# adolfogonzalez3/maddpg

Measured on AMD Instinct MI355X. Metric: env-steps/sec (end-to-end at the reference update cadence), simple_spread N=3, batch 1024, higher is better.
Workload: dtype fp32

## Files before the change

include/maddpg_hip.h:

```cpp
#ifndef MADDPG_HIP_H
#define MADDPG_HIP_H

#include <stddef.h>
#include <stdint.h>

#ifdef __cplusplus
extern "C" {
#endif

#define MDP_MAX_AGENTS 8
#define MDP_ACT_DIM 5
#define MDP_MAX_UNITS 256
#define MDP_ABI_VERSION 5

enum mdp_scenario {
    MDP_SCN_NONE = 0,
    MDP_SCN_SIMPLE = 1,
    MDP_SCN_SPREAD = 2,
    MDP_SCN_ADVERSARY = 3,
    MDP_SCN_TAG = 4,
    MDP_SCN_SPEAKER_LISTENER = 5
};

enum mdp_which {
    MDP_ACTOR = 0, MDP_CRITIC = 1, MDP_TGT_ACTOR = 2, MDP_TGT_CRITIC = 3,
    MDP_M_ACTOR = 4, MDP_V_ACTOR = 5, MDP_M_CRITIC = 6, MDP_V_CRITIC = 7,
    MDP_G_ACTOR = 8, MDP_G_CRITIC = 9
};

enum mdp_region_id {
    MDP_R_THETA = 0, MDP_R_TARGET = 1, MDP_R_ADAM_M = 2, MDP_R_ADAM_V = 3,
    MDP_R_GRAD = 4, MDP_R_REPLAY = 5, MDP_R_INDEX = 6, MDP_R_STATS = 7,
    MDP_R_ENV = 8, MDP_R_EPLOG = 9, MDP_R_BETA = 10, MDP_R_SLAB = 11,
    MDP_R_CTL = 12, MDP_R_COUNT = 13
};

typedef struct mdp_config {
    int32_t n_agents;
    int32_t obs_dim[MDP_MAX_AGENTS];
    int32_t local_q[MDP_MAX_AGENTS];
    int32_t act_dim;
    int32_t num_units;
    int32_t batch_size;
    int32_t max_episode_len;
    int64_t capacity;
    int32_t num_envs;
    int32_t scenario;
    int32_t num_adversaries;
    int32_t world_size, rank;
    float lr;
    float tau;
    float grad_clip;
    float actor_reg;
    float adam_b1, adam_b2, adam_eps;
    double gamma;
    uint64_t seed;
    int32_t episode_log_rows;
    int32_t reserved;
} mdp_config;

typedef struct mdp_tensor_info {
    int64_t offset;
    int32_t rows, cols;
    int32_t dev_rows, dev_cols;
} mdp_tensor_info;

typedef struct mdp_handle mdp_handle;

int32_t mdp_abi_version(void);
int64_t mdp_arena_bytes(const mdp_config* cfg, int64_t* param_floats);
int mdp_create(const mdp_config* cfg, void* arena_dev, int64_t arena_bytes,
               void* hip_stream, mdp_handle** out);
int mdp_destroy(mdp_handle* h);
const char* mdp_last_error(const mdp_handle* h);
void* mdp_stream(mdp_handle* h);
int mdp_synchronize(mdp_handle* h);
int mdp_region(const mdp_handle* h, int32_t region, int64_t* offset, int64_t* bytes);
int mdp_tensor(const mdp_handle* h, int32_t agent, int32_t net, int32_t t, mdp_tensor_info* out);
int mdp_row_layout(const mdp_handle* h, int32_t agent, int32_t out6[6]);
int mdp_set_act_dims(mdp_handle* h, const int32_t dims[MDP_MAX_AGENTS]);
int mdp_get_act_dims(const mdp_handle* h, int32_t dims[MDP_MAX_AGENTS]);

int mdp_set_params(mdp_handle* h, int32_t agent, int32_t which, const float* src_host, int64_t n);
int mdp_get_params(mdp_handle* h, int32_t agent, int32_t which, float* dst_host, int64_t n);
int mdp_get_beta_powers(mdp_handle* h, int32_t agent, int32_t net, float out2[2]);
int mdp_set_beta_powers(mdp_handle* h, int32_t agent, int32_t net, const float in2[2]);

int64_t mdp_buffer_len(mdp_handle* h);
int mdp_buffer_add_rows(mdp_handle* h, const float* rows_dev, int64_t rows);
int mdp_buffer_put_agent(mdp_handle* h, int32_t agent, const int64_t* pos_dev,
                         const float* cols_dev, int64_t rows);
int mdp_buffer_set_len(mdp_handle* h, int64_t len, int64_t next_idx);
int mdp_buffer_set_ring(mdp_handle* h, int64_t len, int64_t next_idx, int64_t rows_total);
int mdp_seed_py_random(mdp_handle* h, uint64_t seed);
int mdp_set_rng_state(mdp_handle* h, const uint32_t* state625_host);
int mdp_get_rng_state(mdp_handle* h, uint32_t* state625_host);
int mdp_make_index(mdp_handle* h, int32_t count, int32_t* idx_dev);
int mdp_sample_rows(mdp_handle* h, const int32_t* idx_dev, int32_t count, float* out_dev);

int mdp_act(mdp_handle* h, int32_t agent, int32_t target, const float* obs_dev,
            float* act_dev, int32_t rows, const float* u_dev);
int mdp_actor_logits(mdp_handle* h, int32_t agent, int32_t target, const float* obs_dev,
                     float* logits_dev, int32_t rows);
int mdp_q_values(mdp_handle* h, int32_t agent, int32_t target, const float* x_dev,
                 float* q_dev, int32_t rows);

int mdp_update(mdp_handle* h, int32_t agent, const int32_t* idx_dev,
               const float* u_tgt_dev, const float* u_act_dev);
int mdp_update_gate(mdp_handle* h, int64_t t);
int mdp_agent_update(mdp_handle* h, int32_t agent, int64_t t, const int32_t* idx_dev, const float* u_dev,
                     double stats_out[6]);
int mdp_update_round(mdp_handle* h);
int mdp_set_graphs(mdp_handle* h, int32_t on);
int mdp_train_step(mdp_handle* h, int32_t rounds);
int mdp_train_steps(mdp_handle* h, int32_t n, const int32_t* rounds, int32_t launch);

int mdp_dp_unique_id(uint8_t* out128);
int mdp_dp_init(mdp_handle* h, const uint8_t* id128, int32_t world, int32_t rank);

#define MDP_XGMI_HANDLE_BYTES 64
int mdp_dp_xgmi_open(mdp_handle* h, int32_t world, int32_t rank, uint8_t* handle_out);
int mdp_dp_xgmi_connect(mdp_handle* h, const uint8_t* handles);
int mdp_dp_xgmi_probe(mdp_handle* h, int32_t* mismatches);
int mdp_dp_xgmi_enable(mdp_handle* h);
int mdp_dp_xgmi_close(mdp_handle* h);
int mdp_dp_info(mdp_handle* h, int32_t out4[4]);
int mdp_dp_exchange_stats(mdp_handle* h, double out4[4], int32_t reset);
int mdp_dp_exchange_stats_enable(mdp_handle* h, int32_t on);
int mdp_ra_plan(const mdp_config* cfg, int32_t cus, int32_t per_cu, int32_t* out);
int mdp_critic_grad(mdp_handle* h, int32_t agent, const int32_t* idx_dev, const float* u_tgt_dev);
int mdp_actor_grad(mdp_handle* h, int32_t agent, const int32_t* idx_dev, const float* u_act_dev);
int mdp_reduce_grad(mdp_handle* h, int32_t agent, int32_t net);
int mdp_apply_grad(mdp_handle* h, int32_t agent, int32_t net, float scale);
int mdp_get_stats(mdp_handle* h, int32_t agent, double out6[6]);
int mdp_check_finite(mdp_handle* h, int64_t* nonfinite_out);

int mdp_set_update_mode(mdp_handle* h, int32_t mode);
int mdp_update_all(mdp_handle* h, const int32_t* idx_dev, const float* u_tgt_dev, const float* u_act_dev);

int mdp_env_reset(mdp_handle* h);
int mdp_env_step(mdp_handle* h, const float* act_in_dev, const float* u_dev);
int mdp_env_get_state(mdp_handle* h, float* pos_host, float* vel_host, int32_t* goal_host, int32_t* ep_step_host);
int mdp_env_set_state(mdp_handle* h, const float* pos_host, const float* vel_host, const int32_t* goal_host, const int32_t* ep_step_host);
int mdp_env_get_comm(mdp_handle* h, float* comm_host);
int mdp_env_set_comm(mdp_handle* h, const float* comm_host);
int mdp_env_obs(mdp_handle* h, float* obs_dev);
#define MDP_BENCH_W 8
int mdp_env_step_bench(mdp_handle* h, float* info_dev);
int mdp_env_step_bench_u(mdp_handle* h, float* info_dev, const float* u_dev);

enum { MDP_EVAL_SAMPLE = 0, MDP_EVAL_MEAN = 1 };
int mdp_evaluate(mdp_handle* h, int64_t first_episode, int32_t episodes, int32_t mode,
                 const float* u_dev, float* ret_dev, float* bench_dev);
int mdp_eval_initial_state(mdp_handle* h, int64_t first_episode, int32_t episodes,
                           float* pos_host, float* vel_host, int32_t* goal_host);

int64_t mdp_actor_set_floats(const mdp_handle* h);
int mdp_actor_set_write(mdp_handle* h, float* set_dev, int32_t agent, const float* src_host, int64_t n);
int mdp_actor_set_snapshot(mdp_handle* h, float* set_dev);
int mdp_evaluate_matchups(mdp_handle* h, const float* bank_dev, int32_t n_sets,
                          const int32_t* table_host, int32_t matchups,
                          int64_t first_episode, int32_t episodes, int32_t mode,
                          const float* u_dev, float* ret_dev, float* bench_dev);
int64_t mdp_episode_count(mdp_handle* h);
int mdp_episode_log(mdp_handle* h, int64_t first, int64_t n, float* out_host);

int64_t mdp_per_bytes(const mdp_config* cfg);
int mdp_per_enable(mdp_handle* h, void* buf_dev, int64_t bytes, float alpha, float beta0, float beta_inc,
                   float eps, float abs_err_upper);
int mdp_per_sample(mdp_handle* h, int32_t agent, int32_t count, const float* u_dev, int32_t* idx_out_dev,
                   float* w_out_dev);
int mdp_per_set_priorities(mdp_handle* h, int32_t agent, const int32_t* pos_dev, const float* p_dev, int32_t count);
int mdp_per_update_errors(mdp_handle* h, int32_t agent, const int32_t* pos_dev, const float* abs_err_dev,
                          int32_t count);
int mdp_per_slots(mdp_handle* h, int32_t agent, int64_t out3[3]);
int64_t mdp_per_tree_nodes(const mdp_handle* h);
int mdp_per_get_tree(mdp_handle* h, int32_t agent, float* nodes_host);
int mdp_per_info(mdp_handle* h, int32_t agent, double out5[5]);

enum mdp_kernel_kind {
    MDP_K_INDEX = 0, MDP_K_GATHER = 1, MDP_K_CRITIC_GRAD = 2, MDP_K_ACTOR_GRAD = 3,
    MDP_K_APPLY = 4, MDP_K_ROLLOUT = 5, MDP_K_REDUCE = 6, MDP_K_REDUCE_APPLY = 7,
    MDP_K_ALLREDUCE = 8,
    MDP_K_PER_SYNC = 9, MDP_K_PER_SAMPLE = 10, MDP_K_PER_UPDATE = 11,
    MDP_K_EVAL = 12,
    MDP_K_COUNT = 13
};
int mdp_prof_enable(mdp_handle* h, int32_t kind, int32_t on);
int mdp_grad_variant(mdp_handle* h, int32_t agent);
int mdp_prof_read(mdp_handle* h, int32_t kind, double* total_ms, int64_t* launches);

#ifdef __cplusplus
}
#endif
#endif
```

maddpg_amd/_lib.py:

```python
import ctypes
import os
import re

import torch

HERE = os.path.dirname(os.path.abspath(__file__))
LIB_PATH = os.environ.get("MDP_LIB") or os.path.join(HERE, "libmaddpg_hip.so")
HEADER = os.path.join(os.path.dirname(HERE), "include", "maddpg_hip.h")

MAX_AGENTS = 8
ACT_DIM = 5
BENCH_W = 8
MAX_UNITS = 256
ABI_VERSION = 5

SCN = {"none": 0, "simple": 1, "simple_spread": 2, "simple_adversary": 3, "simple_tag": 4,
       "simple_speaker_listener": 5}
WHICH = {"actor": 0, "critic": 1, "tgt_actor": 2, "tgt_critic": 3, "m_actor": 4, "v_actor": 5,
         "m_critic": 6, "v_critic": 7, "g_actor": 8, "g_critic": 9}
REGION = {"theta": 0, "target": 1, "adam_m": 2, "adam_v": 3, "grad": 4, "replay": 5, "index": 6,
          "stats": 7, "env": 8, "eplog": 9, "beta": 10, "slab": 11, "ctl": 12}
KERNEL = {"index": 0, "gather": 1, "critic_grad": 2, "actor_grad": 3, "apply": 4, "rollout": 5,
          "reduce": 6, "reduce_apply": 7, "allreduce": 8}
KERNEL_PER = {"per_sync": 9, "per_sample": 10, "per_update": 11}
KERNEL_EVAL = {"eval": 12}
EVAL_MODE = {"sample": 0, "mean": 1}
EVAL_MAX_EPISODES = 1 << 20
EVAL_MAX_SETS = 4096
EVAL_MAX_MATCHUP_EPISODES = 1 << 22


class MdpConfig(ctypes.Structure):
    _fields_ = [
        ("n_agents", ctypes.c_int32),
        ("obs_dim", ctypes.c_int32 * MAX_AGENTS),
        ("local_q", ctypes.c_int32 * MAX_AGENTS),
        ("act_dim", ctypes.c_int32),
        ("num_units", ctypes.c_int32),
        ("batch_size", ctypes.c_int32),
        ("max_episode_len", ctypes.c_int32),
        ("capacity", ctypes.c_int64),
        ("num_envs", ctypes.c_int32),
        ("scenario", ctypes.c_int32),
        ("num_adversaries", ctypes.c_int32),
        ("world_size", ctypes.c_int32),
        ("rank", ctypes.c_int32),
        ("lr", ctypes.c_float),
        ("tau", ctypes.c_float),
        ("grad_clip", ctypes.c_float),
        ("actor_reg", ctypes.c_float),
        ("adam_b1", ctypes.c_float),
        ("adam_b2", ctypes.c_float),
        ("adam_eps", ctypes.c_float),
        ("gamma", ctypes.c_double),
        ("seed", ctypes.c_uint64),
        ("episode_log_rows", ctypes.c_int32),
        ("reserved", ctypes.c_int32),
    ]


class MdpTensorInfo(ctypes.Structure):
    _fields_ = [("offset", ctypes.c_int64), ("rows", ctypes.c_int32), ("cols", ctypes.c_int32),
                ("dev_rows", ctypes.c_int32), ("dev_cols", ctypes.c_int32)]


_P = ctypes.c_void_p
_I32 = ctypes.c_int32
_I64 = ctypes.c_int64
_F32P = ctypes.POINTER(ctypes.c_float)
_F64P = ctypes.POINTER(ctypes.c_double)
_U32P = ctypes.POINTER(ctypes.c_uint32)
_I32P = ctypes.POINTER(ctypes.c_int32)

SIGNATURES = {
    "mdp_abi_version": (_I32, []),
    "mdp_arena_bytes": (_I64, [ctypes.POINTER(MdpConfig), ctypes.POINTER(_I64)]),
    "mdp_create": (ctypes.c_int, [ctypes.POINTER(MdpConfig), _P, _I64, _P, ctypes.POINTER(_P)]),
    "mdp_destroy": (ctypes.c_int, [_P]),
    "mdp_last_error": (ctypes.c_char_p, [_P]),
    "mdp_stream": (_P, [_P]),
    "mdp_synchronize": (ctypes.c_int, [_P]),
    "mdp_region": (ctypes.c_int, [_P, _I32, ctypes.POINTER(_I64), ctypes.POINTER(_I64)]),
    "mdp_tensor": (ctypes.c_int, [_P, _I32, _I32, _I32, ctypes.POINTER(MdpTensorInfo)]),
    "mdp_row_layout": (ctypes.c_int, [_P, _I32, _I32P]),
    "mdp_set_act_dims": (ctypes.c_int, [_P, _I32P]),
    "mdp_get_act_dims": (ctypes.c_int, [_P, _I32P]),
    "mdp_set_params": (ctypes.c_int, [_P, _I32, _I32, _F32P, _I64]),
    "mdp_get_params": (ctypes.c_int, [_P, _I32, _I32, _F32P, _I64]),
    "mdp_get_beta_powers": (ctypes.c_int, [_P, _I32, _I32, _F32P]),
    "mdp_set_beta_powers": (ctypes.c_int, [_P, _I32, _I32, _F32P]),
    "mdp_buffer_len": (_I64, [_P]),
    "mdp_buffer_add_rows": (ctypes.c_int, [_P, _P, _I64]),
    "mdp_buffer_put_agent": (ctypes.c_int, [_P, _I32, _P, _P, _I64]),
    "mdp_buffer_set_len": (ctypes.c_int, [_P, _I64, _I64]),
    "mdp_buffer_set_ring": (ctypes.c_int, [_P, _I64, _I64, _I64]),
    "mdp_seed_py_random": (ctypes.c_int, [_P, ctypes.c_uint64]),
    "mdp_set_rng_state": (ctypes.c_int, [_P, _U32P]),
    "mdp_get_rng_state": (ctypes.c_int, [_P, _U32P]),
    "mdp_make_index": (ctypes.c_int, [_P, _I32, _P]),
    "mdp_sample_rows": (ctypes.c_int, [_P, _P, _I32, _P]),
    "mdp_act": (ctypes.c_int, [_P, _I32, _I32, _P, _P, _I32, _P]),
    "mdp_actor_logits": (ctypes.c_int, [_P, _I32, _I32, _P, _P, _I32]),
    "mdp_q_values": (ctypes.c_int, [_P, _I32, _I32, _P, _P, _I32]),
    "mdp_update": (ctypes.c_int, [_P, _I32, _P, _P, _P]),
    "mdp_update_gate": (ctypes.c_int, [_P, _I64]),
    "mdp_update_round": (ctypes.c_int, [_P]),
    "mdp_set_graphs": (ctypes.c_int, [_P, _I32]),
    "mdp_train_step": (ctypes.c_int, [_P, _I32]),
    "mdp_dp_unique_id": (ctypes.c_int, [ctypes.c_char_p]),
    "mdp_grad_variant": (ctypes.c_int, [_P, _I32]),
    "mdp_dp_init": (ctypes.c_int, [_P, ctypes.c_char_p, _I32, _I32]),
    "mdp_dp_xgmi_open": (ctypes.c_int, [_P, _I32, _I32, ctypes.c_char_p]),
    "mdp_dp_xgmi_connect": (ctypes.c_int, [_P, ctypes.c_char_p]),
    "mdp_dp_xgmi_probe": (ctypes.c_int, [_P, _I32P]),
    "mdp_dp_xgmi_enable": (ctypes.c_int, [_P]),
    "mdp_dp_xgmi_close": (ctypes.c_int, [_P]),
    "mdp_dp_info": (ctypes.c_int, [_P, _I32P]),
    "mdp_dp_exchange_stats": (ctypes.c_int, [_P, ctypes.POINTER(ctypes.c_double), _I32]),
    "mdp_dp_exchange_stats_enable": (ctypes.c_int, [_P, _I32]),
    "mdp_train_steps": (ctypes.c_int, [_P, _I32, ctypes.POINTER(ctypes.c_int32), _I32]),
    "mdp_agent_update": (ctypes.c_int, [_P, _I32, ctypes.c_int64, _P, _P, ctypes.POINTER(ctypes.c_double)]),
    "mdp_ra_plan": (ctypes.c_int, [ctypes.POINTER(MdpConfig), _I32, _I32, _I32P]),
    "mdp_critic_grad": (ctypes.c_int, [_P, _I32, _P, _P]),
    "mdp_actor_grad": (ctypes.c_int, [_P, _I32, _P, _P]),
    "mdp_reduce_grad": (ctypes.c_int, [_P, _I32, _I32]),
    "mdp_apply_grad": (ctypes.c_int, [_P, _I32, _I32, ctypes.c_float]),
    "mdp_get_stats": (ctypes.c_int, [_P, _I32, _F64P]),
    "mdp_check_finite": (ctypes.c_int, [_P, ctypes.POINTER(_I64)]),
    "mdp_env_reset": (ctypes.c_int, [_P]),
    "mdp_env_step": (ctypes.c_int, [_P, _P, _P]),
    "mdp_env_get_state": (ctypes.c_int, [_P, _F32P, _F32P, _I32P, _I32P]),
    "mdp_env_set_state": (ctypes.c_int, [_P, _F32P, _F32P, _I32P, _I32P]),
    "mdp_env_get_comm": (ctypes.c_int, [_P, _F32P]),
    "mdp_env_set_comm": (ctypes.c_int, [_P, _F32P]),
    "mdp_env_obs": (ctypes.c_int, [_P, _P]),
    "mdp_env_step_bench": (ctypes.c_int, [_P, _P]),
    "mdp_env_step_bench_u": (ctypes.c_int, [_P, _P, _P]),
    "mdp_evaluate": (ctypes.c_int, [_P, _I64, _I32, _I32, _P, _P, _P]),
    "mdp_eval_initial_state": (ctypes.c_int, [_P, _I64, _I32, _F32P, _F32P, _I32P]),
    "mdp_actor_set_floats": (_I64, [_P]),
    "mdp_actor_set_write": (ctypes.c_int, [_P, _P, _I32, _F32P, _I64]),
    "mdp_actor_set_snapshot": (ctypes.c_int, [_P, _P]),
    "mdp_evaluate_matchups": (ctypes.c_int, [_P, _P, _I32, _I32P, _I32, _I64, _I32, _I32, _P, _P, _P]),
    "mdp_set_update_mode": (ctypes.c_int, [_P, _I32]),
    "mdp_update_all": (ctypes.c_int, [_P, _P, _P, _P]),
    "mdp_episode_count": (_I64, [_P]),
    "mdp_episode_log": (ctypes.c_int, [_P, _I64, _I64, _F32P]),
    "mdp_per_bytes": (_I64, [ctypes.POINTER(MdpConfig)]),
    "mdp_per_enable": (ctypes.c_int, [_P, _P, _I64, ctypes.c_float, ctypes.c_float, ctypes.c_float,
                                      ctypes.c_float, ctypes.c_float]),
    "mdp_per_sample": (ctypes.c_int, [_P, _I32, _I32, _P, _P, _P]),
    "mdp_per_set_priorities": (ctypes.c_int, [_P, _I32, _P, _P, _I32]),
    "mdp_per_update_errors": (ctypes.c_int, [_P, _I32, _P, _P, _I32]),
    "mdp_per_slots": (ctypes.c_int, [_P, _I32, ctypes.POINTER(_I64)]),
    "mdp_per_tree_nodes": (_I64, [_P]),
    "mdp_per_get_tree": (ctypes.c_int, [_P, _I32, _F32P]),
    "mdp_per_info": (ctypes.c_int, [_P, _I32, _F64P]),
    "mdp_prof_enable": (ctypes.c_int, [_P, _I32, _I32]),
    "mdp_prof_read": (ctypes.c_int, [_P, _I32, _F64P, ctypes.POINTER(_I64)]),
}


def header_symbols(path=HEADER):
    text = open(path).read()
    return sorted(set(re.findall(r"\b(mdp_[a-z0-9_]+)\s*\(", text)))


_lib = None


def load():
    global _lib
    if _lib is not None:
        return _lib
    if not os.path.exists(LIB_PATH):
        raise ImportError(
            f"{LIB_PATH} is missing: build it with `make -C maddpg_amd/csrc` "
            "(or __graft_entry__.build()); maddpg_amd has no CPU fallback")
    lib = ctypes.CDLL(LIB_PATH)
    for name, (res, args) in SIGNATURES.items():
        if os.environ.get("MDP_LIB") and not hasattr(lib, name):
            continue
        fn = getattr(lib, name)
        fn.restype = res
        fn.argtypes = args
    if lib.mdp_abi_version() != ABI_VERSION:
        raise ImportError("libmaddpg_hip.so ABI version mismatch")
    _lib = lib
    return lib


class MdpError(RuntimeError):
    pass


def check(lib, handle, rc, what=""):
    if rc < 0:
        msg = lib.mdp_last_error(handle)
        raise MdpError(f"{what}: {msg.decode() if msg else 'error'}")
    return rc


def fptr(a):
    return a.ctypes.data_as(_F32P)
```

maddpg_amd/csrc/mdp_api.cpp:

```cpp
#include <hip/hip_runtime.h>

#include <algorithm>
#include <cmath>
#include <cstdio>
#include <cstdlib>
#include <cstring>
#include <string>
#include <dlfcn.h>
#include <rccl/rccl.h>

#include <map>
#include <vector>

#include "mdp_kernels.h"

namespace {

inline int64_t r4(int64_t n) { return (n + 3) & ~int64_t(3); }
inline int64_t a256(int64_t n) { return (n + 255) & ~int64_t(255); }

NDesc make_net(int64_t& off, int in, int H, int out) {
  NDesc d;
  d.off = (int)off;
  d.in = in;
// ... 155 lines not shown
  }
  const int E = c->num_envs;
  std::vector<int> dims, widths;
  if (c->scenario != MDP_SCN_NONE) {
    if (!make_env(*c, L.env, dims, widths, err)) return false;
    for (int i = 0; i < n; ++i) topo_set_act_w(T, i, widths[i]);
    for (int i = 0; i < n; ++i)
      if (dims[i] != c->obs_dim[i]) {
        char b[160];
        std::snprintf(b, sizeof(b), "obs_dim[%d]=%d does not match scenario (%d)", i, c->obs_dim[i], dims[i]);
        err = b;
        return false;
      }
    if ((int64_t)E > c->capacity) { err = "num_envs exceeds replay capacity"; return false; }
  } else {
    std::memset(&L.env, 0, sizeof(L.env));
  }
  L.n_ent = n + L.env.n_landmarks;
  {
    int need = std::max(lds_critic_bytes(T, 1), lds_actor_bytes(T));
    need = std::max(need, lds_eval_bytes(std::max(cin_max, obs_max), H));
    if (c->scenario != MDP_SCN_NONE) need = std::max(need, lds_rollout_bytes(T));
    if (need > MDP_LDS_BUDGET) {
      char b[200];
      std::snprintf(b, sizeof(b),
                    "configuration outside the kernels' LDS envelope: a 16-row tile needs %d bytes, a CU has %d "
                    "(sum of obs dims %d, %d units)", need, MDP_LDS_BUDGET, sum_obs, c->num_units);
      err = b;
      return false;
    }
  }
  if (c->episode_log_rows < 0) { err = "episode_log_rows < 0"; return false; }
  if (c->episode_log_rows > 0 && (int64_t)c->episode_log_rows < 2 * (int64_t)E) {
    err = "episode_log_rows must be 0 (default) or at least 2 * num_envs";
    return false;
  }
  L.eplog_rows = c->episode_log_rows > 0 ? c->episode_log_rows : std::max(4096, 4 * E);
  int64_t sz[MDP_R_COUNT];
  sz[MDP_R_THETA] = sz[MDP_R_TARGET] = sz[MDP_R_ADAM_M] = sz[MDP_R_ADAM_V] = sz[MDP_R_GRAD] = 4 * L.PT;
  sz[MDP_R_REPLAY] = 4 * c->capacity * T.row_stride;
  sz[MDP_R_INDEX] = 2 * 4 * (int64_t)n * c->batch_size;
  sz[MDP_R_STATS] = 8 * 8 * (int64_t)n;
  sz[MDP_R_ENV] = (int64_t)E * (4 * 4 * L.n_ent + 4 + 4 + 4 * n) + 64 +
                  (env_dim_c(c->scenario) > 0 ? 4 * (int64_t)E * n * MDP_ACT_DIM : 0);
  sz[MDP_R_EPLOG] = 4 * (int64_t)L.eplog_rows * (1 + n);
  sz[MDP_R_BETA] = 4 * 8 * (int64_t)n;
  sz[MDP_R_SLAB] = (int64_t)n * (4 * (int64_t)L.nwg * (L.slab_c + L.slab_a) + 2 * 8 * 8 * (int64_t)L.nwg +
                                  8 * (int64_t)c->batch_size) + 256 + 256 + mdp_ra_sync_bytes() +
                   4 * (int64_t)L.nwg * 16 * (MDP_APRE_W + MDP_CPRE_W + 2 * T.row_stride) +
                   512;
  sz[MDP_R_CTL] = sizeof(Ctl);
  int64_t o = 0;
  for (int r = 0; r < MDP_R_COUNT; ++r) {
    L.off[r] = o;
    L.bytes[r] = sz[r];
    o += a256(sz[r]);
  }
  L.total = o;
  return true;
}

void py_seed_state(uint64_t seed, uint32_t* mt, int32_t* pos) {
  std::vector<uint32_t> key;
  uint64_t s = seed;
  while (s) {
    key.push_back((uint32_t)(s & 0xffffffffu));
    s >>= 32;
  }
  if (key.empty()) key.push_back(0);
  mt[0] = 19650218u;
  for (int i = 1; i < 624; ++i) mt[i] = 1812433253u * (mt[i - 1] ^ (mt[i - 1] >> 30)) + (uint32_t)i;
  int i = 1, j = 0;
  const int kl = (int)key.size();
  for (int k = std::max(624, kl); k; --k) {
    mt[i] = (mt[i] ^ ((mt[i - 1] ^ (mt[i - 1] >> 30)) * 1664525u)) + key[j] + (uint32_t)j;
    ++i;
    ++j;
    if (i >= 624) {
      mt[0] = mt[623];
      i = 1;
    }
    if (j >= kl) j = 0;
  }
  for (int k = 623; k; --k) {
    mt[i] = (mt[i] ^ ((mt[i - 1] ^ (mt[i - 1] >> 30)) * 1566083941u)) - (uint32_t)i;
    ++i;
    if (i >= 624) {
      mt[0] = mt[623];
      i = 1;
    }
  }
  mt[0] = 0x80000000u;
  *pos = 624;
}

}

struct mdp_handle {
  mdp_config cfg;
  Layout L;
  int device = 0;
  hipStream_t stream = nullptr;
  bool own_stream = false;
  char* arena = nullptr;
  float *theta, *target, *m, *v, *grad, *replay, *beta, *slab_c, *slab_a, *eplog;
  float *pos, *vel, *ep_rew;
  float* env_comm = nullptr;
  int32_t *index, *goal, *ep_step;
  double *stats, *stat_c, *stat_a, *y;
  Ctl* ctl;
  int64_t len = 0, next = 0;
  uint32_t act_ctr = 0, reset_ctr = 0;
  bool env_lockstep = true;
  std::string err;
  bool ready = false;
  bool prof_on[MDP_K_COUNT] = {};
  std::vector<hipEvent_t> ev[MDP_K_COUNT];
  size_t ev_used[MDP_K_COUNT] = {};
  double prof_ms[MDP_K_COUNT] = {};
  int64_t prof_n[MDP_K_COUNT] = {};
  bool graphs = true;
  bool capturing = false;
  int eager_rounds = 0;
  bool general_grads = false;
  bool fused_apply = true;
  uint32_t* ra_ctr = nullptr;
  uint64_t* ra_part = nullptr;
  float* apre = nullptr;
  bool actor_pre = true;
  float* cpre = nullptr;
  bool critic_pre = true;
  float* apre_rows = nullptr;
  float* cpre_rows = nullptr;
  hipGraph_t round_graph = nullptr;
  hipGraphExec_t round_exec = nullptr;
  std::map<int, hipGraphExec_t> step_exec;
  std::map<std::vector<int>, hipGraphExec_t> multi_exec;
  int eager_steps = 0;
  ncclComm_t comm = nullptr;
  int dp_world = 1;
  bool dp_graphs = false;
  int update_mode = 0;
  FusedApplyArgs* tp_list = nullptr;
  RaBatch tp_batch;
  RaBatch tp_reduce, tp_step;
  int ra_cap = 0, ra_batch_cap = 0;
  bool tp_fits[4] = {true, true, true, true};
  std::vector<FusedApplyArgs> tp_host[4];
  RaBatch tp_xchg;
  RaBatch tp_pair[3][MDP_MAX_AGENTS];
  bool tp_pair_fits[3][MDP_MAX_AGENTS] = {};
  FusedApplyArgs tp_pair_host[3][MDP_MAX_AGENTS][2];
  bool rollout_draw = true;
  bool draw_ahead = true;
  bool grad_pair = true;
  uint64_t* xbuf = nullptr;
  int x_world = 0, x_rank = 0;
  std::vector<void*> x_opened;
  XchgDesc* xd_dev = nullptr;
  uint32_t* x_probe = nullptr;
  uint32_t x_probe_ep = 0;
  bool p2p = false;
  bool xw_stats = false;
  bool per = false;
  bool trained = false;
  bool started = false;
  PerHdr* per_hdr = nullptr;
  PerState* per_st = nullptr;
  int32_t* per_idx = nullptr;
  float *per_w = nullptr, *per_td = nullptr;
  PerNode* per_trees = nullptr;
  int64_t per_P = 0;
  float per_alpha = 0.6f, per_beta0 = 0.4f, per_beta_inc = 0.001f, per_eps = 0.01f, per_upper = 1.0f;
  int64_t per_host_total = 0;
};

namespace {

int fail(mdp_handle* h, const char* what, hipError_t e = hipSuccess) {
  if (h) {
    h->err = what;
    if (e != hipSuccess) {
      h->err += ": ";
      h->err += hipGetErrorString(e);
    }
  }
  return -1;
}

#define HIPCHK(h, call)                        \
  do {                                         \
    hipError_t e__ = (call);                   \
    if (e__ != hipSuccess) return fail(h, #call, e__); \
  } while (0)

bool unusable(const mdp_handle* h) { return !h || !h->ready; }
#define MDP_NEED(h)               \
  do {                            \
    if (unusable(h)) return -1;   \
  } while (0)

int need_dev(mdp_handle* h, const void* p, int64_t bytes, const char* fn, const char* arg, bool null_ok = true) {
  auto refuse = [&](const char* why) {
    std::string m = std::string(fn) + ": " + arg + " " + why;
    return fail(h, m.c_str());
  };
  if (!p) return null_ok ? 0 : refuse("is null");
  hipPointerAttribute_t a;
  std::memset(&a, 0, sizeof(a));
  const hipError_t e = hipPointerGetAttributes(&a, p);
  if (e != hipSuccess) (void)hipGetLastError();
  const bool managed = a.isManaged || a.type == hipMemoryTypeManaged;
  if (e != hipSuccess || !(a.type == hipMemoryTypeDevice || managed)) {
    (void)hipGetLastError();
    return refuse("is not device memory (a host address would fault the GPU); pass a buffer of the handle's device");
  }
  if (!managed && a.device != h->device) return refuse("is memory of another device than the handle's");
  if (!managed && bytes > 0) {
    hipDeviceptr_t base = nullptr;
    size_t size = 0;
    if (hipMemGetAddressRange(&base, &size, (hipDeviceptr_t)p) == hipSuccess) {
      if ((const char*)p + bytes > (const char*)base + size)
        return refuse("ends before the bytes this call reads or writes (allocation too small)");
    } else {
      (void)hipGetLastError();
    }
  }
  return 0;
}
#define MDP_DEV(h, p, bytes, fn, null_ok)                                   \
  do {                                                                     \
    if (need_dev(h, p, (int64_t)(bytes), fn, #p, null_ok)) return -1;     \
  } while (0)

}

MdpLaunchEv& mdp_launch_ev() {
  static thread_local MdpLaunchEv e;
  return e;
}

namespace {

struct ProfScope {
  mdp_handle* h;
  int kind;
  bool packet;
  hipEvent_t stop = nullptr;
  ProfScope(mdp_handle* hh, int k, bool pk = true) : h(hh), kind(k), packet(pk) {
    if (!h->prof_on[kind] || h->capturing) return;
    auto& pool = h->ev[kind];
    size_t u = h->ev_used[kind];
    if (u + 2 > pool.size()) {
      for (int q = 0; q < 64; ++q) {
        hipEvent_t e;
        if (hipEventCreate(&e) != hipSuccess) return;
        pool.push_back(e);
      }
    }
    h->ev_used[kind] = u + 2;
    stop = pool[u + 1];
    if (packet) {
      mdp_launch_ev() = MdpLaunchEv{pool[u], pool[u + 1]};
    } else {
      (void)hipEventRecord(pool[u], h->stream);
    }
  }
  ~ProfScope() {
    if (!stop) return;
    if (!packet) {
      (void)hipEventRecord(stop, h->stream);
      return;
    }
    MdpLaunchEv& e = mdp_launch_ev();
    if (e.start) {
      e.start = e.stop = nullptr;
      h->ev_used[kind] -= 2;
    }
  }
};

void flush_prof(mdp_handle* h, int kind) {
  auto& pool = h->ev[kind];
  const size_t u = h->ev_used[kind];
  if (!u) return;
  (void)hipEventSynchronize(pool[u - 1]);
  for (size_t q = 0; q + 1 < u; q += 2) {
    float ms = 0.f;
    if (hipEventElapsedTime(&ms, pool[q], pool[q + 1]) == hipSuccess) {
      h->prof_ms[kind] += ms;
      h->prof_n[kind] += 1;
    }
  }
  h->ev_used[kind] = 0;
}

bool bad_agent(mdp_handle* h, int agent) {
  if (unusable(h)) return true;
  if (agent < 0 || agent >= h->cfg.n_agents) {
    fail(h, "agent index out of range");
    return true;
  }
  return false;
}

int region_for(int which, int* region, int* net) {
// ... 705 lines not shown
      const int rc = launch_tp_batch(h, 1);
      if (rc) return rc;
    }
    const int rc = dp_allreduce_all(h);
    if (rc) return rc;
    ProfScope p(h, MDP_K_APPLY, h->tp_fits[2]);
    return launch_tp_batch(h, 2);
  }
  ProfScope p(h, MDP_K_REDUCE_APPLY, h->tp_fits[0]);
  return launch_tp_batch(h, 0);
}

int set_ring(mdp_handle* h, int64_t len, int64_t next) {
  h->len = len;
  h->next = next;
  HIPCHK(h, mdp_launch_set_ring(h->ctl, len, next, h->stream));
  return 0;
}

struct PerLayout {
  int64_t P = 1, hdr = 0, st = 0, idx = 0, w = 0, td = 0, trees = 0, total = 0;
};
PerLayout per_layout(const mdp_config& c) {
  PerLayout p;
  while (p.P < c.capacity) p.P <<= 1;
  const int64_t nb = 4 * (int64_t)c.n_agents * c.batch_size;
  int64_t o = 0;
  p.hdr = o;
  o += a256(sizeof(PerHdr));
  p.st = o;
  o += a256(sizeof(PerState) * MDP_MAX_AGENTS);
  p.idx = o;
  o += a256(nb);
  p.w = o;
  o += a256(nb);
  p.td = o;
  o += a256(nb);
  p.trees = o;
  o += (int64_t)c.n_agents * 2 * p.P * (int64_t)sizeof(PerNode);
  p.total = o;
  return p;
}

int per_sync(mdp_handle* h, int64_t host_rows, bool reset) {
  PerSyncArgs a;
  a.ctl = h->ctl;
  a.hdr = h->per_hdr;
  a.trees = h->per_trees;
  a.tree_stride = 2 * h->per_P;
  a.P = h->per_P;
  a.cap = h->cfg.capacity;
  a.E = h->cfg.num_envs;
  a.host_rows = host_rows;
  a.reset = reset ? 1 : 0;
  a.upper = h->per_upper;
  a.alpha = h->per_alpha;
  ProfScope p(h, MDP_K_PER_SYNC);
  HIPCHK(h, mdp_launch_per_sync(a, h->cfg.n_agents, h->stream));
  return 0;
}

int per_sample(mdp_handle* h, int agent0, int agents, int count, const float* u, const int32_t* idx_in,
               int32_t* idx_out, float* w_out, int64_t stride) {
  PerSampleArgs a;
  a.trees = h->per_trees + (int64_t)agent0 * 2 * h->per_P;
  a.tree_stride = 2 * h->per_P;
  a.P = h->per_P;
  a.cap = h->cfg.capacity;
  a.st = h->per_st + agent0;
  a.agent0 = agent0;
  a.count = count;
  a.u = u;
  a.idx_in = idx_in;
  a.idx_out = idx_out;
  a.w_out = w_out;
  a.stride = stride;
  a.seed = h->cfg.seed;
  a.beta_inc = h->per_beta_inc;
  ProfScope p(h, MDP_K_PER_SAMPLE);
  HIPCHK(h, mdp_launch_per_sample(a, agents, h->stream));
  return 0;
}

int per_update(mdp_handle* h, int agent0, int agents, int count, const int32_t* pos, const float* val,
               int64_t stride, bool from_err) {
  PerUpdateArgs a;
  a.trees = h->per_trees + (int64_t)agent0 * 2 * h->per_P;
  a.tree_stride = 2 * h->per_P;
  a.P = h->per_P;
  a.cap = h->cfg.capacity;
  a.count = count;
  a.ctl = h->ctl;
  a.pos = pos;
  a.val = val;
  a.stride = stride;
  a.from_err = from_err ? 1 : 0;
  a.eps = h->per_eps;
  a.upper = h->per_upper;
  a.alpha = h->per_alpha;
  ProfScope p(h, MDP_K_PER_UPDATE);
  HIPCHK(h, mdp_launch_per_update(a, agents, h->stream));
  return 0;
}

const char* kPerNoDp = "prioritized replay runs on one GPU in strict mode: no data-parallel exchange";

}

extern "C" {

int32_t mdp_abi_version(void) { return MDP_ABI_VERSION; }

int64_t mdp_arena_bytes(const mdp_config* cfg, int64_t* param_floats) {
  Layout L;
  std::string err;
  if (!build_layout(cfg, L, err)) return -1;
  if (param_floats) *param_floats = L.PT;
  return L.total;
}

int mdp_ra_plan(const mdp_config* cfg, int32_t cus, int32_t per_cu, int32_t* out) {
  Layout L;
  std::string err;
  if (!build_layout(cfg, L, err) || cus < 0 || per_cu < 0) return -1;
  int fallback = 0;
  for (int i = 0; i < cfg->n_agents; ++i)
    for (int net = 0; net < 2; ++net) {
      const int g = mdp_ra_grid_of(L.topo, i, net);
      const bool ok = mdp_ra_fits(L.topo, i, net, cus * per_cu);
      if (out) out[2 * i + net] = ok ? g : -g;
      fallback += ok ? 0 : 1;
    }
  return fallback;
}

int mdp_create(const mdp_config* cfg, void* arena_dev, int64_t arena_bytes, void* hip_stream, mdp_handle** out) {
  if (!out) return -1;
  *out = nullptr;
  mdp_handle* h = new mdp_handle();
  std::string err;
  if (!build_layout(cfg, h->L, err)) {
    h->err = err;
    *out = h;
    return -1;
  }
  h->cfg = *cfg;
  {
    const char* g = getenv("MDP_GENERAL_GRADS");
    h->general_grads = g && g[0] == '1';
    const char* u = getenv("MDP_UNFUSED_APPLY");
    h->fused_apply = !(u && u[0] == '1');
    const char* rd = getenv("MDP_ROLLOUT_DRAW");
    h->rollout_draw = !(rd && rd[0] == '0');
    const char* da = getenv("MDP_DRAW_AHEAD");
    h->draw_ahead = !(da && da[0] == '0');
    const char* gp = getenv("MDP_GRAD_PAIR");
    h->grad_pair = !(gp && gp[0] == '0');
    const char* ap = getenv("MDP_ACTOR_PRE");
    h->actor_pre = !(ap && ap[0] == '0');
    const char* cp = getenv("MDP_CRITIC_PRE");
    h->critic_pre = !(cp && cp[0] == '0');
  }
  if (!arena_dev || arena_bytes < h->L.total) {
    h->err = "arena missing or too small";
    *out = h;
    return -1;
  }
  *out = h;
  HIPCHK(h, hipGetDevice(&h->device));
  if (need_dev(h, arena_dev, h->L.total, "mdp_create", "arena_dev", false)) return -1;
  {
    int cus = 0, per = 0, per_b = 0;
    HIPCHK(h, hipDeviceGetAttribute(&cus, hipDeviceAttributeMultiprocessorCount, h->device));
    HIPCHK(h, mdp_ra_occupancy(&per));
    HIPCHK(h, mdp_ra_batch_occupancy(&per_b));
    h->ra_cap = cus * per;
    h->ra_batch_cap = cus * per_b;
    int scratch = 0;
    HIPCHK(h, mdp_spin_kernels_scratch(&scratch));
    if (scratch > 0) h->ra_cap = h->ra_batch_cap = 0;
  }
  if (hip_stream) {
    h->stream = (hipStream_t)hip_stream;
  } else {
    HIPCHK(h, hipStreamCreateWithFlags(&h->stream, hipStreamNonBlocking));
    h->own_stream = true;
  }
  h->arena = (char*)arena_dev;
  auto R = [&](int r) { return (void*)(h->arena + h->L.off[r]); };
  h->theta = (float*)R(MDP_R_THETA);
  h->target = (float*)R(MDP_R_TARGET);
  h->m = (float*)R(MDP_R_ADAM_M);
  h->v = (float*)R(MDP_R_ADAM_V);
  h->grad = (float*)R(MDP_R_GRAD);
  h->replay = (float*)R(MDP_R_REPLAY);
  h->index = (int32_t*)R(MDP_R_INDEX);
  h->stats = (double*)R(MDP_R_STATS);
  h->eplog = (float*)R(MDP_R_EPLOG);
  h->beta = (float*)R(MDP_R_BETA);
  h->ctl = (Ctl*)R(MDP_R_CTL);
  {
    const int E = cfg->num_envs, ne = h->L.n_ent, n = cfg->n_agents;
    char* p = (char*)R(MDP_R_ENV);
    h->pos = (float*)p;
    p += 4 * (int64_t)E * ne * 2;
    h->vel = (float*)p;
    p += 4 * (int64_t)E * ne * 2;
    h->goal = (int32_t*)p;
    p += 4 * (int64_t)E;
    h->ep_step = (int32_t*)p;
    p += 4 * (int64_t)E;
    h->ep_rew = (float*)p;
    p += 4 * (int64_t)E * n;
    if (env_dim_c(cfg->scenario) > 0) h->env_comm = (float*)(p + 64);
  }
  {
    char* p = (char*)R(MDP_R_SLAB);
    const int64_t nwg = h->L.nwg, na = cfg->n_agents;
    h->slab_c = (float*)p;
    p += 4 * na * nwg * h->L.slab_c;
    h->slab_a = (float*)p;
    p += 4 * na * nwg * h->L.slab_a;
    p = (char*)(((uintptr_t)p + 7) & ~uintptr_t(7));
    h->stat_c = (double*)p;
    p += 8 * 8 * na * nwg;
    h->stat_a = (double*)p;
    p += 8 * 8 * na * nwg;
    h->y = (double*)p;
    p += 8 * na * (int64_t)cfg->batch_size + 256;
    p = (char*)(((uintptr_t)p + 255) & ~uintptr_t(255));
    h->ra_ctr = (uint32_t*)p;
    h->ra_part = (uint64_t*)(p + (int64_t)MDP_MAX_AGENTS * 2 * 8 * 128);
    h->apre = (float*)(p + mdp_ra_sync_bytes());
    h->cpre = h->apre + (int64_t)nwg * 16 * MDP_APRE_W;
    h->apre_rows = h->cpre + (int64_t)nwg * 16 * MDP_CPRE_W;
    h->cpre_rows = h->apre_rows + (int64_t)nwg * 16 * h->L.topo.row_stride;
  }
  HIPCHK(h, hipMemsetAsync(h->arena, 0, h->L.total, h->stream));
  std::vector<float> beta(8 * cfg->n_agents);
  for (int i = 0; i < cfg->n_agents * 2; ++i) {
    beta[4 * i] = beta[4 * i + 2] = cfg->adam_b1;
    beta[4 * i + 1] = beta[4 * i + 3] = cfg->adam_b2;
  }
  HIPCHK(h, hipMemcpyAsync(h->beta, beta.data(), 4 * beta.size(), hipMemcpyHostToDevice, h->stream));
  Ctl c;
  std::memset(&c, 0, sizeof(c));
  py_seed_state(0, c.mt, &c.mt_pos);
  HIPCHK(h, hipMemcpyAsync(h->ctl, &c, sizeof(c), hipMemcpyHostToDevice, h->stream));
  HIPCHK(h, hipStreamSynchronize(h->stream));
  h->err.clear();
  h->ready = true;
  return 0;
}

int mdp_destroy(mdp_handle* h) {
  if (!h) return 0;
  if (h->stream) (void)hipStreamSynchronize(h->stream);
  if (h->tp_list) (void)hipFree(h->tp_list);
  for (int k = 0; k < MDP_K_COUNT; ++k)
    for (auto e : h->ev[k]) (void)hipEventDestroy(e);
  if (h->round_exec) (void)hipGraphExecDestroy(h->round_exec);
  if (h->comm) (void)rccl().destroy(h->comm);
  xgmi_release(h);
  for (auto& kv : h->step_exec) (void)hipGraphExecDestroy(kv.second);
  for (auto& kv : h->multi_exec) (void)hipGraphExecDestroy(kv.second);
  if (h->round_graph) (void)hipGraphDestroy(h->round_graph);
  if (h->own_stream && h->stream) (void)hipStreamDestroy(h->stream);
  delete h;
  return 0;
}

const char* mdp_last_error(const mdp_handle* h) { return h ? h->err.c_str() : "null handle"; }
void* mdp_stream(mdp_handle* h) { return h ? (void*)h->stream : nullptr; }

int mdp_synchronize(mdp_handle* h) {
  MDP_NEED(h);
  HIPCHK(h, hipStreamSynchronize(h->stream));
  uint32_t fault = 0;
  HIPCHK(h, hipMemcpy(&fault, &h->ctl->fault, sizeof(fault), hipMemcpyDeviceToHost));
  if (fault == 1) return fail(h, "device fault: a tensor-norm handshake timed out (k_reduce_apply)");
  if (fault == 2) return fail(h, "device fault: a data-parallel peer did not reach the xGMI exchange within 30 s");
  if (fault) return fail(h, "device fault");
  return 0;
}

int mdp_region(const mdp_handle* h, int32_t region, int64_t* offset, int64_t* bytes) {
  if (unusable(h) || region < 0 || region >= MDP_R_COUNT) return -1;
  if (offset) *offset = h->L.off[region];
  if (bytes) *bytes = h->L.bytes[region];
  return 0;
}

int mdp_tensor(const mdp_handle* h, int32_t agent, int32_t net, int32_t t, mdp_tensor_info* out) {
  if (unusable(h) || agent < 0 || agent >= h->cfg.n_agents || t < 0 || t > 5 || !out) return -1;
  const NDesc& d = net ? h->L.topo.ag[agent].critic : h->L.topo.ag[agent].actor;
  out->offset = d.t[t].off;
  logical_shape(h, agent, net ? 1 : 0, t, &out->rows, &out->cols);
  out->dev_rows = d.t[t].rows;
  out->dev_cols = d.t[t].cols;
  return 0;
}

int mdp_set_act_dims(mdp_handle* h, const int32_t dims[MDP_MAX_AGENTS]) {
  MDP_NEED(h);
  if (!dims) return fail(h, "mdp_set_act_dims: dims is null");
  if (h->started || h->trained)
// ... 399 lines not shown
    if (e != hipSuccess) return fail(h, "hipStreamEndCapture", e);
    h->round_graph = g;
    HIPCHK(h, hipGraphInstantiate(&h->round_exec, g, nullptr, nullptr, 0));
  }
  HIPCHK(h, hipGraphLaunch(h->round_exec, h->stream));
  return 0;
}

int mdp_grad_variant(mdp_handle* h, int32_t agent) {
  if (unusable(h) || agent < 0 || agent >= h->cfg.n_agents) return -1;
  return (!h->general_grads && grads_r_ok(h->L.topo, agent)) ? 1 : 0;
}

int mdp_dp_unique_id(uint8_t* out128) {
  if (!out128 || !rccl().ok) return -1;
  ncclUniqueId id;
  if (rccl().get_id(&id) != ncclSuccess) return -1;
  std::memcpy(out128, &id, sizeof(id));
  return 0;
}

int mdp_dp_init(mdp_handle* h, const uint8_t* id128, int32_t world, int32_t rank) {
  if (unusable(h) || !id128) return -1;
  if (h->per) return fail(h, kPerNoDp);
  if (h->update_mode != 0) return fail(h, "join data parallelism before choosing the throughput mode");
  if (h->p2p || h->xbuf) return fail(h, "mdp_dp_init: the xGMI exchange is already set up");
  if (!rccl().ok) return fail(h, "librccl.so.1 could not be loaded");
  if (world < 1 || rank < 0 || rank >= world) return fail(h, "mdp_dp_init: bad world/rank");
  if (h->comm) return fail(h, "mdp_dp_init: already initialised");
  ncclUniqueId id;
  std::memcpy(&id, id128, sizeof(id));
  HIPCHK(h, hipSetDevice(h->device));
  const ncclResult_t r = rccl().init_rank(&h->comm, world, id, rank);
  if (r != ncclSuccess) {
    h->comm = nullptr;
    h->err = std::string("ncclCommInitRank: ") + rccl().err(r);
    return -1;
  }
  h->dp_world = world;
  const char* g = getenv("MDP_DP_GRAPHS");
  h->dp_graphs = g && g[0] == '1';
  for (auto& kv : h->step_exec) (void)hipGraphExecDestroy(kv.second);
  for (auto& kv : h->multi_exec) (void)hipGraphExecDestroy(kv.second);
  h->step_exec.clear();
  h->multi_exec.clear();
  if (h->round_exec) {
    (void)hipGraphExecDestroy(h->round_exec);
    h->round_exec = nullptr;
  }
  if (h->round_graph) {
    (void)hipGraphDestroy(h->round_graph);
    h->round_graph = nullptr;
  }
  return 0;
}

static void drop_graphs(mdp_handle* h);

int mdp_dp_xgmi_open(mdp_handle* h, int32_t world, int32_t rank, uint8_t* handle_out) {
  if (unusable(h) || !handle_out) return -1;
  if (h->per) return fail(h, kPerNoDp);
  if (h->update_mode != 0) return fail(h, "join data parallelism before choosing the throughput mode");
  if (h->comm) return fail(h, "mdp_dp_xgmi_open: an RCCL communicator is already set up");
  if (h->xbuf) return fail(h, "mdp_dp_xgmi_open: already open");
  if (world < 2 || world > MDP_XCH_MAXW || rank < 0 || rank >= world)
    return fail(h, "mdp_dp_xgmi_open: world must be 2..8 and 0 <= rank < world");
  if (h->general_grads || !h->fused_apply) return fail(h, "the xGMI exchange needs the fused optimizer kernel");
  for (int i = 0; i < h->cfg.n_agents; ++i)
    for (int net = 0; net < 2; ++net) {
      if (!reduce_apply_ok(h, i, net)) return fail(h, "the xGMI exchange needs the fused optimizer kernel");
    }
  HIPCHK(h, hipSetDevice(h->device));
  const int64_t bytes = mdp_xch_bytes(world, h->L.PT);
  void* p = nullptr;
  HIPCHK(h, hipExtMallocWithFlags(&p, (size_t)bytes, hipDeviceMallocUncached));
  h->xbuf = (uint64_t*)p;
  HIPCHK(h, hipMemset(p, 0, (size_t)bytes));
  HIPCHK(h, hipMalloc((void**)&h->x_probe, 2 * sizeof(uint32_t)));
  HIPCHK(h, hipDeviceSynchronize());
  hipIpcMemHandle_t mh;
  HIPCHK(h, hipIpcGetMemHandle(&mh, p));
  static_assert(sizeof(mh) == MDP_XGMI_HANDLE_BYTES, "IPC handle size");
  std::memcpy(handle_out, &mh, sizeof(mh));
  h->x_world = world;
  h->x_rank = rank;
  return 0;
}

int mdp_dp_xgmi_connect(mdp_handle* h, const uint8_t* handles) {
  if (unusable(h) || !handles) return -1;
  if (!h->xbuf) return fail(h, "mdp_dp_xgmi_connect: call mdp_dp_xgmi_open first");
  if (!h->x_opened.empty()) return fail(h, "mdp_dp_xgmi_connect: already connected");
  const int W = h->x_world, r = h->x_rank;
  XchgDesc xd;
  std::memset(&xd, 0, sizeof(xd));
  xd.world = W;
  xd.rank = r;
  xd.pt = h->L.PT + MDP_XCH_PROBE;
  h->x_opened.assign(W, nullptr);
  for (int q = 0; q < W; ++q) {
    void* base = h->xbuf;
    if (q != r) {
      hipIpcMemHandle_t mh;
      std::memcpy(&mh, handles + (int64_t)q * MDP_XGMI_HANDLE_BYTES, sizeof(mh));
      const hipError_t e = hipIpcOpenMemHandle(&base, mh, hipIpcMemLazyEnablePeerAccess);
      if (e != hipSuccess) return fail(h, "hipIpcOpenMemHandle", e);
      h->x_opened[q] = base;
    }
    xd.data[q] = (uint64_t*)base;
  }
  HIPCHK(h, hipMalloc((void**)&h->xd_dev, sizeof(XchgDesc)));
  HIPCHK(h, hipMemcpy(h->xd_dev, &xd, sizeof(XchgDesc), hipMemcpyHostToDevice));
  return 0;
}

int mdp_dp_xgmi_probe(mdp_handle* h, int32_t* mismatches) {
  if (unusable(h)) return -1;
  if (!h->xd_dev) return fail(h, "mdp_dp_xgmi_probe: not connected");
  const int nchunk = MDP_XCH_PROBE / 256;
  HIPCHK(h, hipMemsetAsync(h->x_probe, 0, 2 * sizeof(uint32_t), h->stream));
  for (int k = 0; k < 4; ++k)
    HIPCHK(h, mdp_launch_xchg_probe(h->xd_dev, ++h->x_probe_ep, nchunk, h->x_probe, h->x_probe + 1, h->stream));
  uint32_t res[2] = {0, 0};
  HIPCHK(h, hipMemcpyAsync(res, h->x_probe, sizeof(res), hipMemcpyDeviceToHost, h->stream));
  HIPCHK(h, hipStreamSynchronize(h->stream));
  if (mismatches) *mismatches = (int32_t)res[0];
  if (res[1]) return fail(h, "mdp_dp_xgmi_probe: a peer did not reach the exchange within 30 s");
  if (res[0]) return fail(h, "mdp_dp_xgmi_probe: exchanged values differ from the expected world sum");
  return 0;
}

int mdp_dp_xgmi_enable(mdp_handle* h) {
  if (unusable(h)) return -1;
  if (!h->xd_dev) return fail(h, "mdp_dp_xgmi_enable: not connected");
  if (h->per) return fail(h, kPerNoDp);
  if (h->update_mode != 0) return fail(h, "join data parallelism before choosing the throughput mode");
  HIPCHK(h, hipStreamSynchronize(h->stream));
  h->p2p = true;
  h->dp_world = h->x_world;
  drop_graphs(h);
  return 0;
}

int mdp_dp_xgmi_close(mdp_handle* h) {
  if (unusable(h)) return -1;
  (void)hipGetLastError();
  if (h->stream) HIPCHK(h, hipStreamSynchronize(h->stream));
  xgmi_release(h);
  if (!h->comm) h->dp_world = 1;
  drop_graphs(h);
  return 0;
}

int mdp_dp_info(mdp_handle* h, int32_t out4[4]) {
  if (unusable(h) || !out4) return -1;
  out4[0] = h->p2p ? 2 : (h->comm ? 1 : 0);
  out4[1] = 1;
  out4[2] = h->cfg.rank;
  out4[3] = 0;
  if (h->p2p) {
    out4[1] = h->x_world;
    out4[2] = h->x_rank;
    for (void* p : h->x_opened) out4[3] += p ? 1 : 0;
  } else if (h->comm) {
    int c = h->dp_world;
    if (rccl().count && rccl().count(h->comm, &c) != ncclSuccess) return fail(h, "ncclCommCount failed");
    out4[1] = c;
    out4[3] = c - 1;
  }
  return 0;
}

int mdp_dp_exchange_stats(mdp_handle* h, double out4[4], int32_t reset) {
  if (unusable(h) || !out4) return -1;
  HIPCHK(h, hipStreamSynchronize(h->stream));
  uint64_t w[3] = {0, 0, 0};
  HIPCHK(h, hipMemcpy(w, &h->ctl->xw_ticks, sizeof(w), hipMemcpyDeviceToHost));
  const double us_per_tick = 0.01;
  out4[0] = (double)w[1];
  out4[1] = w[1] ? (double)w[0] * us_per_tick / (double)w[1] : 0.0;
  out4[2] = (double)w[2] * us_per_tick;
  out4[3] = (double)w[0] * us_per_tick;
  if (reset) {
    HIPCHK(h, hipMemsetAsync(&h->ctl->xw_ticks, 0, sizeof(w), h->stream));
    HIPCHK(h, hipStreamSynchronize(h->stream));
  }
  return 0;
}

int mdp_dp_exchange_stats_enable(mdp_handle* h, int32_t on) {
  if (unusable(h)) return -1;
  h->xw_stats = on != 0;
  return 0;
}

int mdp_set_graphs(mdp_handle* h, int32_t on) {
  MDP_NEED(h);
  h->graphs = on != 0;
  return 0;
}

static void drop_graphs(mdp_handle* h) {
  for (auto& kv : h->step_exec) (void)hipGraphExecDestroy(kv.second);
  for (auto& kv : h->multi_exec) (void)hipGraphExecDestroy(kv.second);
  h->step_exec.clear();
  h->multi_exec.clear();
  h->eager_steps = 0;
  if (h->round_exec) {
    (void)hipGraphExecDestroy(h->round_exec);
    h->round_exec = nullptr;
  }
  if (h->round_graph) {
    (void)hipGraphDestroy(h->round_graph);
    h->round_graph = nullptr;
  }
  h->eager_rounds = 0;
}

int mdp_set_update_mode(mdp_handle* h, int32_t mode) {
  if (unusable(h)) return -1;
  if (mode != 0 && mode != 1) return fail(h, "update mode must be 0 (strict) or 1 (throughput)");
  if (mode == 1) {
    if (h->per) return fail(h, "prioritized replay needs the strict update mode (throughput mode is not supported)");
    if (!tp_ok(h)) return fail(h, "throughput mode needs the fused optimizer step for every net and <= 8 agents");
    HIPCHK(h, hipStreamSynchronize(h->stream));
    if (tp_setup(h)) return -1;
  }
  if (mode != h->update_mode) {
    HIPCHK(h, hipStreamSynchronize(h->stream));
    drop_graphs(h);
    h->update_mode = mode;
  }
  return 0;
}

int mdp_update_all(mdp_handle* h, const int32_t* idx_dev, const float* u_tgt_dev, const float* u_act_dev) {
  if (unusable(h)) return -1;
  if (h->update_mode != 1) return fail(h, "mdp_update_all: set throughput mode first");
  h->trained = true;
  if (h->len <= 0) return fail(h, "update on an empty replay buffer");
  {
    const int64_t B = h->cfg.batch_size, n = h->cfg.n_agents;
    MDP_DEV(h, idx_dev, 4 * n * B, "mdp_update_all", true);
    MDP_DEV(h, u_tgt_dev, 4 * n * n * B * MDP_ACT_DIM, "mdp_update_all", true);
    MDP_DEV(h, u_act_dev, 4 * n * B * MDP_ACT_DIM, "mdp_update_all", true);
  }
  const int32_t* idx = idx_dev;
  if (!idx) {
    const int rc = launch_make_index(h, h->cfg.n_agents * h->cfg.batch_size, h->index);
    if (rc) return rc;
    idx = h->index;
  }
  return do_round_tp(h, idx, u_tgt_dev, u_act_dev, nullptr);
}

int mdp_critic_grad(mdp_handle* h, int32_t agent, const int32_t* idx_dev, const float* u_tgt_dev) {
  if (bad_agent(h, agent)) return -1;
  if (!idx_dev) return fail(h, "critic_grad needs indices");
  if (h->per) return fail(h, "mdp_critic_grad: the phase entry points serve data parallelism; prioritized replay uses mdp_update");
  h->trained = true;
  MDP_DEV(h, idx_dev, 4 * (int64_t)h->cfg.batch_size, "mdp_critic_grad", false);
  MDP_DEV(h, u_tgt_dev, 4 * (int64_t)h->cfg.n_agents * h->cfg.batch_size * MDP_ACT_DIM, "mdp_critic_grad", true);
  return do_critic_grad(h, agent, idx_dev, u_tgt_dev);
}

int mdp_actor_grad(mdp_handle* h, int32_t agent, const int32_t* idx_dev, const float* u_act_dev) {
  if (bad_agent(h, agent)) return -1;
  if (!idx_dev) return fail(h, "actor_grad needs indices");
  h->started = true;
  MDP_DEV(h, idx_dev, 4 * (int64_t)h->cfg.batch_size, "mdp_actor_grad", false);
  MDP_DEV(h, u_act_dev, 4 * (int64_t)h->cfg.batch_size * MDP_ACT_DIM, "mdp_actor_grad", true);
  return do_actor_grad(h, agent, idx_dev, u_act_dev);
}

int mdp_reduce_grad(mdp_handle* h, int32_t agent, int32_t net) {
  if (bad_agent(h, agent)) return -1;
  return do_reduce(h, agent, net ? 1 : 0);
}

int mdp_apply_grad(mdp_handle* h, int32_t agent, int32_t net, float scale) {
  if (bad_agent(h, agent)) return -1;
  return do_apply(h, agent, net ? 1 : 0, false, scale);
}

int mdp_get_stats(mdp_handle* h, int32_t agent, double out6[6]) {
  if (bad_agent(h, agent)) return -1;
  double buf[8];
  HIPCHK(h, hipMemcpyAsync(buf, h->stats + agent * 8, sizeof(buf), hipMemcpyDeviceToHost, h->stream));
  HIPCHK(h, hipStreamSynchronize(h->stream));
  for (int i = 0; i < 6; ++i) out6[i] = buf[i];
  return 0;
}

static int need_env(mdp_handle* h) {
  MDP_NEED(h);
  if (h->cfg.scenario == MDP_SCN_NONE || h->cfg.num_envs <= 0) return fail(h, "handle has no device env");
  h->started = true;
  return 0;
}

int mdp_env_reset(mdp_handle* h) {
  if (need_env(h)) return -1;
  EnvResetArgs a;
  a.env = h->L.env;
  a.seed = h->cfg.seed;
  a.ctr = h->reset_ctr++;
  a.env_base = h->cfg.rank * h->cfg.num_envs;
  a.E = h->cfg.num_envs;
  a.pos = h->pos;
  a.vel = h->vel;
  a.goal = h->goal;
  a.ep_step = h->ep_step;
  a.ep_rew = h->ep_rew;
  a.comm = h->env_comm;
  HIPCHK(h, mdp_launch_env_reset(a, h->stream));
  h->env_lockstep = true;
  return 0;
}

static int env_step_launch(mdp_handle* h, const float* act_in_dev, const float* u_dev, float* bench = nullptr,
                           int32_t* pf_out = nullptr, int pf_count = 0, int nsteps = 1) {
  RolloutArgs a;
  a.pf_out = pf_out;
  a.pf_count = pf_out ? pf_count : 0;
  a.nsteps = nsteps;
  a.topo = h->L.topo;
  a.env = h->L.env;
  a.theta = h->theta;
  a.replay = h->replay;
  a.cap = h->cfg.capacity;
  a.pos = h->pos;
  a.vel = h->vel;
  a.goal = h->goal;
  a.ep_step = h->ep_step;
  a.ep_rew = h->ep_rew;
  a.comm = h->env_comm;
  a.eplog = h->eplog;
  a.eplog_cap = h->L.eplog_rows;
  a.eplog_by_env = h->env_lockstep ? 1 : 0;
  a.ctl = h->ctl;
  a.seed = h->cfg.seed;
  a.E = h->cfg.num_envs;
  a.env_base = h->cfg.rank * h->cfg.num_envs;
  a.act_in = act_in_dev;
  a.u_in = u_dev;
  a.ticket = &h->ctl->ticket[2];
  a.bench = bench;
  ProfScope p(h, MDP_K_ROLLOUT);
  HIPCHK(h, mdp_launch_rollout(a, h->L.topo.H, lds_rollout_bytes(h->L.topo), h->stream));
  return 0;
}

static bool rollout_multi_ok(const mdp_handle* h) { return h->cfg.num_envs <= 16; }

static void advance_ring_mirror(mdp_handle* h) {
  const int64_t cap = h->cfg.capacity, E = h->cfg.num_envs;
  h->len = std::min(cap, h->len + E);
  h->next = (h->next + E) % cap;
}

int mdp_env_step(mdp_handle* h, const float* act_in_dev, const float* u_dev) {
  if (need_env(h)) return -1;
  const int64_t en5 = 4 * (int64_t)h->cfg.num_envs * h->cfg.n_agents * MDP_ACT_DIM;
  MDP_DEV(h, act_in_dev, en5, "mdp_env_step", true);
  MDP_DEV(h, u_dev, en5, "mdp_env_step", true);
  const int rc = env_step_launch(h, act_in_dev, u_dev);
  if (rc) return rc;
  advance_ring_mirror(h);
  return 0;
}

int mdp_env_step_bench(mdp_handle* h, float* info_dev) {
  if (need_env(h)) return -1;
  if (!info_dev) return fail(h, "mdp_env_step_bench: info_dev is null");
  MDP_DEV(h, info_dev, 4 * (int64_t)h->cfg.num_envs * h->cfg.n_agents * MDP_BENCH_W, "mdp_env_step_bench", false);
  if (h->cfg.scenario == MDP_SCN_SIMPLE)
    return fail(h, "scenario 'simple' has no benchmark_data (MPE Scenario attribute missing)");
  if (h->cfg.scenario == MDP_SCN_SPEAKER_LISTENER)
    return fail(h, "scenario 'simple_speaker_listener': upstream's benchmark_data raises (it names an undefined "
                   "variable), so there is no record to return");
  const int rc = env_step_launch(h, nullptr, nullptr, info_dev);
  if (rc) return rc;
  advance_ring_mirror(h);
  return 0;
}

static const char* no_bench_reason(int scenario) {
  if (scenario == MDP_SCN_SIMPLE) return "scenario 'simple' has no benchmark_data (MPE Scenario attribute missing)";
  if (scenario == MDP_SCN_SPEAKER_LISTENER)
    return "scenario 'simple_speaker_listener': upstream's benchmark_data raises (it names an undefined "
           "variable), so there is no record to return";
  return nullptr;
}

int mdp_env_step_bench_u(mdp_handle* h, float* info_dev, const float* u_dev) {
  if (need_env(h)) return -1;
  if (!info_dev) return fail(h, "mdp_env_step_bench_u: info_dev is null");
  const int64_t en = 4 * (int64_t)h->cfg.num_envs * h->cfg.n_agents;
  MDP_DEV(h, info_dev, en * MDP_BENCH_W, "mdp_env_step_bench_u", false);
  MDP_DEV(h, u_dev, en * MDP_ACT_DIM, "mdp_env_step_bench_u", true);
  if (const char* why = no_bench_reason(h->cfg.scenario)) return fail(h, why);
  const int rc = env_step_launch(h, nullptr, u_dev, info_dev);
  if (rc) return rc;
  advance_ring_mirror(h);
  return 0;
}

#define MDP_EVAL_MAX_EPISODES (1 << 20)
static int eval_range_ok(mdp_handle* h, const char* fn, int64_t first, int32_t episodes) {
  std::string m = std::string(fn) + ": ";
  if (episodes < 1 || episodes > MDP_EVAL_MAX_EPISODES) return fail(h, (m + "1 <= episodes <= 2^20").c_str());
  if (first < 0 || first + episodes > ((int64_t)1 << 32))
    return fail(h, (m + "episode ids [first_episode, first_episode + episodes) must lie inside uint32").c_str());
  return 0;
}

int mdp_evaluate(mdp_handle* h, int64_t first_episode, int32_t episodes, int32_t mode, const float* u_dev,
                 float* ret_dev, float* bench_dev) {
  if (need_env(h)) return -1;
  if (mode != MDP_EVAL_SAMPLE && mode != MDP_EVAL_MEAN)
    return fail(h, "mdp_evaluate: mode must be MDP_EVAL_SAMPLE (0) or MDP_EVAL_MEAN (1)");
  if (eval_range_ok(h, "mdp_evaluate", first_episode, episodes)) return -1;
  if (u_dev && mode == MDP_EVAL_MEAN) return fail(h, "mdp_evaluate: u_dev is given but MDP_EVAL_MEAN draws no noise");
  if (!ret_dev) return fail(h, "mdp_evaluate: ret_dev is null");
  hipStreamCaptureStatus cs = hipStreamCaptureStatusNone;
  if (h->capturing || (hipStreamIsCapturing(h->stream, &cs) == hipSuccess && cs != hipStreamCaptureStatusNone))
    return fail(h, "mdp_evaluate: the handle's stream is capturing a graph (evaluation is not captured)");
  (void)hipGetLastError();
  const int64_t en = 4 * (int64_t)episodes * h->cfg.n_agents;
  MDP_DEV(h, u_dev, en * h->cfg.max_episode_len * MDP_ACT_DIM, "mdp_evaluate", true);
  MDP_DEV(h, ret_dev, en, "mdp_evaluate", false);
  MDP_DEV(h, bench_dev, en * MDP_BENCH_W, "mdp_evaluate", true);
  if (bench_dev)
    if (const char* why = no_bench_reason(h->cfg.scenario)) return fail(h, why);
  EvalEpArgs a;
  a.topo = h->L.topo;
  a.env = h->L.env;
  a.theta = h->theta;
  a.seed = h->cfg.seed;
  a.first = (uint32_t)first_episode;
  a.episodes = episodes;
  a.mode = mode;
  a.u_in = u_dev;
  a.ret = ret_dev;
  a.bench = bench_dev;
  ProfScope p(h, MDP_K_EVAL);
  HIPCHK(h, mdp_launch_eval_episodes(a, h->L.topo.H, lds_rollout_bytes(h->L.topo), h->stream));
  return 0;
}

int mdp_eval_initial_state(mdp_handle* h, int64_t first_episode, int32_t episodes, float* pos_host, float* vel_host,
                           int32_t* goal_host) {
  if (need_env(h)) return -1;
  if (eval_range_ok(h, "mdp_eval_initial_state", first_episode, episodes)) return -1;
  if (!pos_host || !vel_host || !goal_host) return fail(h, "mdp_eval_initial_state: null output");
  hipStreamCaptureStatus cs = hipStreamCaptureStatusNone;
  if (h->capturing || (hipStreamIsCapturing(h->stream, &cs) == hipSuccess && cs != hipStreamCaptureStatusNone))
    return fail(h, "mdp_eval_initial_state: the handle's stream is capturing a graph");
  (void)hipGetLastError();
  const int64_t ne2 = 2 * (int64_t)(h->L.env.n_agents + h->L.env.n_landmarks);
  const int chunk = std::min<int64_t>(episodes, 1 << 16);
  float* tmp = nullptr;
  HIPCHK(h, hipMalloc((void**)&tmp, (size_t)chunk * (2 * ne2 + 1) * 4));
  float* dpos = tmp;
  float* dvel = tmp + chunk * ne2;
  int32_t* dgoal = reinterpret_cast<int32_t*>(tmp + 2 * chunk * ne2);
  hipError_t e = hipSuccess;
  for (int64_t done = 0; done < episodes && e == hipSuccess; done += chunk) {
    const int c = (int)std::min<int64_t>(chunk, episodes - done);
    e = mdp_launch_eval_reset(h->L.env, h->cfg.seed, (uint32_t)(first_episode + done), c, dpos, dvel, dgoal, h->stream);
    if (e == hipSuccess) e = hipMemcpyAsync(pos_host + done * ne2, dpos, (size_t)c * ne2 * 4, hipMemcpyDeviceToHost, h->stream);
    if (e == hipSuccess) e = hipMemcpyAsync(vel_host + done * ne2, dvel, (size_t)c * ne2 * 4, hipMemcpyDeviceToHost, h->stream);
    if (e == hipSuccess) e = hipMemcpyAsync(goal_host + done, dgoal, (size_t)c * 4, hipMemcpyDeviceToHost, h->stream);
    if (e == hipSuccess) e = hipStreamSynchronize(h->stream);
  }
  (void)hipFree(tmp);
  if (e != hipSuccess) return fail(h, "mdp_eval_initial_state", e);
  return 0;
}

#define MDP_EVAL_MAX_SETS 4096
#define MDP_EVAL_MAX_MATCHUPS 4096
#define MDP_EVAL_MAX_MATCHUP_EPISODES ((int64_t)1 << 22)
static int64_t actor_set_floats(const mdp_handle* h) { return (h->L.PT + 3) & ~(int64_t)3; }
static bool stream_captures(mdp_handle* h) {
  hipStreamCaptureStatus cs = hipStreamCaptureStatusNone;
  const bool c = h->capturing || (hipStreamIsCapturing(h->stream, &cs) == hipSuccess && cs != hipStreamCaptureStatusNone);
  (void)hipGetLastError();
  return c;
}

int64_t mdp_actor_set_floats(const mdp_handle* h) { return unusable(h) ? -1 : actor_set_floats(h); }

int mdp_actor_set_write(mdp_handle* h, float* set_dev, int32_t agent, const float* src_host, int64_t n) {
  MDP_NEED(h);
  if (agent < 0 || agent >= h->cfg.n_agents) return fail(h, "mdp_actor_set_write: agent index out of range");
  if (!src_host) return fail(h, "mdp_actor_set_write: src_host is null");
  if (n != net_floats(h, agent, 0)) return fail(h, "mdp_actor_set_write: n: param count mismatch");
  if (stream_captures(h)) return fail(h, "mdp_actor_set_write: the handle's stream is capturing a graph");
  MDP_DEV(h, set_dev, 4 * actor_set_floats(h), "mdp_actor_set_write", false);
  const NDesc& d = h->L.topo.ag[agent].actor;
  const std::vector<float> buf = scatter_net(h, agent, 0, src_host);
  HIPCHK(h, hipMemcpyAsync(set_dev + d.off, buf.data(), 4 * buf.size(), hipMemcpyHostToDevice, h->stream));
  HIPCHK(h, hipStreamSynchronize(h->stream));
  return 0;
}

int mdp_actor_set_snapshot(mdp_handle* h, float* set_dev) {
  MDP_NEED(h);
  if (stream_captures(h)) return fail(h, "mdp_actor_set_snapshot: the handle's stream is capturing a graph");
  MDP_DEV(h, set_dev, 4 * actor_set_floats(h), "mdp_actor_set_snapshot", false);
  for (int j = 0; j < h->cfg.n_agents; ++j) {
    const NDesc& d = h->L.topo.ag[j].actor;
    HIPCHK(h, hipMemcpyAsync(set_dev + d.off, h->theta + d.off, 4 * (size_t)d.size, hipMemcpyDeviceToDevice, h->stream));
  }
  return 0;
}

int mdp_evaluate_matchups(mdp_handle* h, const float* bank_dev, int32_t n_sets, const int32_t* table_host,
                          int32_t matchups, int64_t first_episode, int32_t episodes, int32_t mode, const float* u_dev,
                          float* ret_dev, float* bench_dev) {
  MDP_NEED(h);
  const char* fn = "mdp_evaluate_matchups";
  if (h->cfg.scenario == MDP_SCN_NONE || h->cfg.num_envs <= 0)
    return fail(h, "mdp_evaluate_matchups: the handle has no device env");
  if (mode != MDP_EVAL_SAMPLE && mode != MDP_EVAL_MEAN)
    return fail(h, "mdp_evaluate_matchups: mode must be MDP_EVAL_SAMPLE (0) or MDP_EVAL_MEAN (1)");
  if (n_sets < 1 || n_sets > MDP_EVAL_MAX_SETS) return fail(h, "mdp_evaluate_matchups: 1 <= n_sets <= 4096");
  if (matchups < 1 || matchups > MDP_EVAL_MAX_MATCHUPS) return fail(h, "mdp_evaluate_matchups: 1 <= matchups <= 4096");
  if (eval_range_ok(h, fn, first_episode, episodes)) return -1;
  if ((int64_t)matchups * episodes > MDP_EVAL_MAX_MATCHUP_EPISODES)
    return fail(h, "mdp_evaluate_matchups: matchups * episodes <= 2^22");
  if (u_dev && mode == MDP_EVAL_MEAN)
    return fail(h, "mdp_evaluate_matchups: u_dev is given but MDP_EVAL_MEAN draws no noise");
  if (!bank_dev) return fail(h, "mdp_evaluate_matchups: bank_dev is null");
  if (!table_host) return fail(h, "mdp_evaluate_matchups: table_host is null");
  if (!ret_dev) return fail(h, "mdp_evaluate_matchups: ret_dev is null");
  if (((uintptr_t)bank_dev & 15) != 0) return fail(h, "mdp_evaluate_matchups: bank_dev must be 16-byte aligned");
  const int n = h->cfg.n_agents;
  for (int m = 0; m < matchups; ++m)
    for (int j = 0; j < n; ++j) {
      const int32_t v = table_host[(int64_t)m * n + j];
      if (v < 0 || v >= n_sets) {
        char b[200];
        std::snprintf(b, sizeof(b), "mdp_evaluate_matchups: table_host[matchup %d][agent %d] = %d is outside [0, n_sets = %d)",
                      m, j, (int)v, (int)n_sets);
        return fail(h, b);
      }
    }
  if (stream_captures(h))
    return fail(h, "mdp_evaluate_matchups: the handle's stream is capturing a graph (evaluation is not captured)");
  const int64_t stride = actor_set_floats(h);
  const int64_t en = 4 * (int64_t)episodes * n;
  MDP_DEV(h, bank_dev, 4 * (int64_t)n_sets * stride, fn, false);
  MDP_DEV(h, u_dev, en * h->cfg.max_episode_len * MDP_ACT_DIM, fn, true);
  MDP_DEV(h, ret_dev, (int64_t)matchups * en, fn, false);
  MDP_DEV(h, bench_dev, (int64_t)matchups * en * MDP_BENCH_W, fn, true);
  if (bench_dev)
    if (const char* why = no_bench_reason(h->cfg.scenario))
      return fail(h, (std::string("mdp_evaluate_matchups: bench_dev: ") + why).c_str());
  const int lds = lds_eval_matchups_bytes(h->L.topo);
  if (lds > MDP_LDS_BUDGET) return fail(h, "mdp_evaluate_matchups: the configuration leaves no LDS for the table row");
  int32_t* table_dev = nullptr;
  const size_t tbytes = 4 * (size_t)matchups * n;
  HIPCHK(h, hipMalloc((void**)&table_dev, tbytes));
  hipError_t e = hipMemcpyAsync(table_dev, table_host, tbytes, hipMemcpyHostToDevice, h->stream);
  if (e == hipSuccess) {
    EvalMuArgs a;
    a.topo = h->L.topo;
    a.env = h->L.env;
    a.theta = nullptr;
    a.seed = h->cfg.seed;
    a.first = (uint32_t)first_episode;
    a.episodes = episodes;
    a.mode = mode;
    a.u_in = u_dev;
    a.ret = ret_dev;
    a.bench = bench_dev;
    a.bank = bank_dev;
    a.table = table_dev;
    a.set_stride = stride;
    a.matchups = matchups;
    ProfScope p(h, MDP_K_EVAL);
    e = mdp_launch_eval_matchups(a, h->L.topo.H, lds, h->stream);
  }
  const hipError_t es = hipStreamSynchronize(h->stream);
  (void)hipFree(table_dev);
  if (e != hipSuccess) return fail(h, "mdp_evaluate_matchups: launch", e);
  if (es != hipSuccess) return fail(h, "mdp_evaluate_matchups: hipStreamSynchronize", es);
  return 0;
}

static int step_launches(mdp_handle* h, int rounds) {
  const int nb = h->cfg.n_agents * h->cfg.batch_size;
  if (h->per) {
    int rc = env_step_launch(h, nullptr, nullptr);
    for (int r = 0; r < rounds && !rc; ++r) rc = per_round_launches(h, r == 0);
    return rc;
  }
  int32_t* slot[2] = {h->index, h->index + nb};
  const bool pf = prefetch_ok(h) && (h->update_mode == 0 || tp_fast(h));
  const bool ra_draw = !pf && (h->update_mode == 0 ? draw_in_ra_ok(h) : !tp_fast(h));
  bool fast_all = !h->general_grads;
  for (int i = 0; i < h->cfg.n_agents && fast_all; ++i) fast_all = grads_r_ok(h->L.topo, i);
  const int ahead = !h->draw_ahead || h->update_mode != 0 ? 0 : (pf && fast_all) ? 1 : ra_draw ? 2 : 0;
  const int first = ahead ? h->cfg.batch_size : nb;
  const bool in_rollout = rounds > 0 && h->rollout_draw;
  int rc = env_step_launch(h, nullptr, nullptr, nullptr, in_rollout ? slot[0] : nullptr, first);
  if (rc || rounds == 0) return rc;
  if (!in_rollout && (rc = launch_make_index(h, first, slot[0]))) return rc;
  bool carry = false;
  for (int r = 0; r < rounds && !rc; ++r) {
    const bool more = r + 1 < rounds;
    int32_t* next = (more && pf) ? slot[(r + 1) & 1] : nullptr;
    rc = round_updates(h, slot[r & 1], next, carry, next, &carry, (more && ra_draw) ? slot[(r + 1) & 1] : nullptr,
                       ahead);
    if (!rc && more && !pf && !ra_draw) rc = launch_make_index(h, nb, slot[(r + 1) & 1]);
  }
  return rc;
}

static int train_step_body(mdp_handle* h, int rounds) {
  const bool no_graph = h->comm && !h->dp_graphs;
  if (!h->graphs || no_graph || any_prof(h) || h->eager_steps < 1 || rounds == 0) {
    if (rounds > 0) ++h->eager_steps;
    return step_launches(h, rounds);
  }
  auto it = h->step_exec.find(rounds);
  if (it == h->step_exec.end()) {
    HIPCHK(h, hipStreamBeginCapture(h->stream, hipStreamCaptureModeThreadLocal));
    h->capturing = true;
    const int rc = step_launches(h, rounds);
    h->capturing = false;
    hipGraph_t g = nullptr;
    const hipError_t e = hipStreamEndCapture(h->stream, &g);
    if (rc) {
      if (g) (void)hipGraphDestroy(g);
      return rc;
    }
    if (e != hipSuccess) return fail(h, "hipStreamEndCapture", e);
    hipGraphExec_t x = nullptr;
    const hipError_t ei = hipGraphInstantiate(&x, g, nullptr, nullptr, 0);
    (void)hipGraphDestroy(g);
    if (ei != hipSuccess) return fail(h, "hipGraphInstantiate", ei);
    it = h->step_exec.emplace(rounds, x).first;
  }
  HIPCHK(h, hipGraphLaunch(it->second, h->stream));
  return 0;
}

static int multi_graph(mdp_handle* h, const std::vector<int>& ks, hipGraphExec_t* out) {
  auto it = h->multi_exec.find(ks);
  if (it != h->multi_exec.end()) {
    *out = it->second;
    return 0;
  }
  HIPCHK(h, hipStreamBeginCapture(h->stream, hipStreamCaptureModeThreadLocal));
  h->capturing = true;
  int rc = 0;
  for (size_t i = 0; i < ks.size() && !rc;) {
    size_t j = i;
    while (j < ks.size() && ks[j] == 0 && (int)(j - i) < 64) ++j;
    if (j - i > 1 && rollout_multi_ok(h)) {
      rc = env_step_launch(h, nullptr, nullptr, nullptr, nullptr, 0, (int)(j - i));
      i = j;
    } else {
      rc = step_launches(h, ks[i]);
      ++i;
    }
  }
  h->capturing = false;
  hipGraph_t g = nullptr;
  const hipError_t e = hipStreamEndCapture(h->stream, &g);
  if (rc) {
    if (g) (void)hipGraphDestroy(g);
    return rc;
  }
  if (e != hipSuccess) return fail(h, "hipStreamEndCapture", e);
  hipGraphExec_t x = nullptr;
  const hipError_t ei = hipGraphInstantiate(&x, g, nullptr, nullptr, 0);
  (void)hipGraphDestroy(g);
  if (ei != hipSuccess) return fail(h, "hipGraphInstantiate", ei);
  h->multi_exec.emplace(ks, x);
  *out = x;
  return 0;
}

int mdp_train_steps(mdp_handle* h, int32_t n, const int32_t* rounds, int32_t launch) {
  if (need_env(h)) return -1;
  if (n < 1 || n > 64 || !rounds) return fail(h, "mdp_train_steps: 1 <= n <= 64 steps");
  std::vector<int> ks(rounds, rounds + n);
  for (int k : ks)
    if (k < 0 || k > 64) return fail(h, "mdp_train_steps: rounds must be in [0, 64]");
  h->trained = true;
  const bool no_graph = h->comm && !h->dp_graphs;
  const bool graphable = h->graphs && !no_graph && !any_prof(h) && h->eager_steps >= 1;
  if (!launch) {
    hipGraphExec_t x = nullptr;
    return graphable ? multi_graph(h, ks, &x) : 0;
  }
  if (!graphable) {
    for (int k : ks) {
      const int rc = mdp_train_step(h, k);
      if (rc) return rc;
    }
    return 0;
  }
  const int64_t len0 = h->len, next0 = h->next;
  for (int i = 0; i < n; ++i) advance_ring_mirror(h);
  hipGraphExec_t x = nullptr;
  int rc = multi_graph(h, ks, &x);
  if (!rc) {
    const hipError_t e = hipGraphLaunch(x, h->stream);
    if (e != hipSuccess) rc = fail(h, "hipGraphLaunch", e);
  }
  if (rc) {
    h->len = len0;
    h->next = next0;
  }
  return rc;
}

int mdp_train_step(mdp_handle* h, int32_t rounds) {
  if (need_env(h)) return -1;
  if (rounds < 0 || rounds > 64) return fail(h, "mdp_train_step: rounds must be in [0, 64]");
  if (rounds > 0 && h->len + h->cfg.num_envs <= 0) return fail(h, "update round on an empty replay buffer");
  h->trained = true;
  const int64_t len0 = h->len, next0 = h->next;
  advance_ring_mirror(h);
  const int rc = train_step_body(h, rounds);
  if (rc) {
    h->len = len0;
    h->next = next0;
  }
  return rc;
}

// ... 275 lines not shown
```

maddpg_amd/csrc/mdp_device.h:

```cpp
#pragma once
#include <hip/hip_runtime.h>
#include <stdint.h>

#include "mdp_topo.h"

#define MDP_NT 256
#define MDP_NW 4
#define MDP_R 16

typedef float f32x4 __attribute__((ext_vector_type(4)));

#define MDP_MFMA(a, b, c) __builtin_amdgcn_mfma_f32_16x16x4f32((a), (b), (c), 0, 0, 0)

#ifdef MDP_STAMPS
__device__ unsigned long long g_mdp_stamps[64];
#define MDP_STAMP(i)                                                                     \
  do {                                                                                   \
    if (blockIdx.x == 0 && threadIdx.x == 0) g_mdp_stamps[i] = __builtin_amdgcn_s_memrealtime(); \
  } while (0)
#define MDP_CLK(i)                                                                      \
  do {                                                                                  \
    if (blockIdx.x == 0 && (threadIdx.x & 63) == 0) g_mdp_stamps[i] = __builtin_amdgcn_s_memtime(); \
  } while (0)
#define MDP_STAMPW(i)                                                                              \
// ... 631 lines not shown
}

__device__ __forceinline__ void gather_rows16(const float* __restrict__ replay, int stride, const int32_t* __restrict__ idx,
                                     int r0, int nvalid, float* rowbuf, int ldr) {
  const int v4 = stride >> 2;
  for (int e = threadIdx.x; e < MDP_R * v4; e += blockDim.x) {
    const int r = e / v4, c4 = e - r * v4;
    float4 v = make_float4(0.f, 0.f, 0.f, 0.f);
    if (r < nvalid) v = *reinterpret_cast<const float4*>(replay + (int64_t)idx[r0 + r] * stride + c4 * 4);
    float* d = rowbuf + r * ldr + c4 * 4;
    d[0] = v.x;
    d[1] = v.y;
    d[2] = v.z;
    d[3] = v.w;
  }
}

__device__ __forceinline__ void gather_rows16_part(const float* __restrict__ replay, int stride,
                                                   const int32_t* __restrict__ idx, int r0, int nvalid, float* rowbuf,
                                                   int ldr, int t0, int nt) {
  const int v4 = stride >> 2;
  for (int e = (int)threadIdx.x - t0; e < MDP_R * v4; e += nt) {
    const int r = e / v4, c4 = e - r * v4;
    float4 v = make_float4(0.f, 0.f, 0.f, 0.f);
    if (r < nvalid) v = *reinterpret_cast<const float4*>(replay + (int64_t)idx[r0 + r] * stride + c4 * 4);
    float* d = rowbuf + r * ldr + c4 * 4;
    d[0] = v.x;
    d[1] = v.y;
    d[2] = v.z;
    d[3] = v.w;
  }
}

__device__ __forceinline__ void load_rows16_part(const float* __restrict__ block, int stride, float* rowbuf, int ldr,
                                                 int t0, int nt) {
  const int v4 = stride >> 2;
  for (int e = (int)threadIdx.x - t0; e < MDP_R * v4; e += nt) {
    const int r = e / v4, c4 = e - r * v4;
    const float4 v = *reinterpret_cast<const float4*>(block + (int64_t)r * stride + c4 * 4);
    float* d = rowbuf + r * ldr + c4 * 4;
    d[0] = v.x;
    d[1] = v.y;
    d[2] = v.z;
    d[3] = v.w;
  }
}
__device__ __forceinline__ void handoff_st4(float* p, f32x4 v) {
#ifdef MDP_WT_HANDOFF
  asm volatile("global_store_dwordx4 %0, %1, off sc1" ::"v"(p), "v"(v) : "memory");
#else
  *reinterpret_cast<f32x4*>(p) = v;
#endif
}

__device__ __forceinline__ void store_rows16(const float* rowbuf, int ldr, int stride, float* __restrict__ block) {
  const int v4 = stride >> 2;
  for (int e = threadIdx.x; e < MDP_R * v4; e += blockDim.x) {
    const int r = e / v4, c4 = e - r * v4;
    const float* sp = rowbuf + r * ldr + c4 * 4;
    handoff_st4(block + (int64_t)r * stride + c4 * 4, f32x4{sp[0], sp[1], sp[2], sp[3]});
  }
}

__device__ __forceinline__ void copy_cols16(const float* src, int lds_src, int src_off, float* dst, int lds_dst, int dst_off,
                                   int ncols) {
  for (int e = threadIdx.x; e < MDP_R * ncols; e += blockDim.x) {
    const int r = e / ncols, c = e - r * ncols;
    dst[r * lds_dst + dst_off + c] = src[r * lds_src + src_off + c];
  }
}

__device__ __forceinline__ void colsum16(const float* X, int ldx, int ncols, float* __restrict__ out) {
  for (int c = threadIdx.x; c < ncols; c += blockDim.x) {
    float s = 0.f;
#pragma unroll
    for (int r = 0; r < MDP_R; ++r) s += X[r * ldx + c];
    out[c] = s;
  }
}

struct LdsCarve {
  float* base;
  int off;
  __device__ LdsCarve(float* p) : base(p), off(0) {}
  __device__ float* take(int n) {
    float* p = base + off;
    off += (n + 3) & ~3;
    return p;
  }
};

#define MDP_RH 64
#define MDP_RLH 68
#define MDP_RLD 65

__device__ __forceinline__ f32x4 ld4(const float* __restrict__ p) { return *reinterpret_cast<const f32x4*>(p); }

template <int KS>
__device__ __forceinline__ void rf_load(f32x4 (&w)[KS], const float* __restrict__ W, int K) {
  const int lane = threadIdx.x & 63, r = lane & 15;
  const int kq = lane >> 4;
#pragma unroll
  for (int s = 0; s < KS; ++s) w[s] = ld4(W + min(4 * s + kq, K - 1) * MDP_RH + 4 * r);
}

template <int KS>
__device__ __forceinline__ void rf_acc(f32x4 (&acc)[4], const float* X, int ldx, int K, const f32x4 (&w)[KS],
                                       int mlo = 0, int mhi = 0) {
  const int lane = threadIdx.x & 63, r = lane & 15, kq = lane >> 4;
  const float* xr = X + r * ldx;
  float x[KS];
#pragma unroll
  for (int s = 0; s < KS; ++s) {
    const int k = 4 * s + kq;
    const float v = xr[min(k, K - 1)];
    x[s] = (k < K && (k < mlo || k >= mhi)) ? v : 0.f;
  }
  __builtin_amdgcn_sched_barrier(0);
#pragma unroll
  for (int s = 0; s < KS; ++s) {
    if (4 * s < K) {
#pragma unroll
      for (int t = 0; t < 4; ++t) acc[t] = MDP_MFMA(x[s], w[s][t], acc[t]);
    }
  }
}

__device__ __forceinline__ void rf_zero(f32x4 (&acc)[4]) {
#pragma unroll
  for (int t = 0; t < 4; ++t) acc[t] = f32x4{0.f, 0.f, 0.f, 0.f};
}

template <bool RELU>
__device__ __forceinline__ void rf_store(const f32x4 (&acc)[4], f32x4 b, float* Y, int ldy) {
  const int lane = threadIdx.x & 63, r = lane & 15, kq = lane >> 4;
#pragma unroll
  for (int i = 0; i < 4; ++i) {
    f32x4 v;
#pragma unroll
    for (int t = 0; t < 4; ++t) v[t] = RELU ? fmaxf(acc[t][i] + b[t], 0.f) : acc[t][i] + b[t];
    *reinterpret_cast<f32x4*>(Y + (kq * 4 + i) * ldy + 4 * r) = v;
  }
}

__device__ __forceinline__ void rh_load(float (&w)[16], const float* __restrict__ W, int nout) {
  const int lane = threadIdx.x & 63, r = lane & 15, kq = lane >> 4;
  const int c = min(r, nout - 1);
#pragma unroll
  for (int s = 0; s < 16; ++s) {
    const float v = W[(4 * s + kq) * nout + c];
    w[s] = r < nout ? v : 0.f;
  }
}
__device__ __forceinline__ f32x4 rh_acc(const float* X, int ldx, const float (&w)[16]) {
  const int lane = threadIdx.x & 63, r = lane & 15, kq = lane >> 4;
  float x[16];
#pragma unroll
  for (int s = 0; s < 16; ++s) x[s] = X[r * ldx + 4 * s + kq];
  __builtin_amdgcn_sched_barrier(0);
  f32x4 acc = {0.f, 0.f, 0.f, 0.f};
#pragma unroll
  for (int s = 0; s < 16; ++s) acc = MDP_MFMA(x[s], w[s], acc);
  return acc;
}

__device__ __forceinline__ void rq_load(float (&w)[16], const float* __restrict__ W) {
  const int q = threadIdx.x & 3;
#pragma unroll
  for (int j = 0; j < 16; ++j) w[j] = W[4 * j + q];
}
__device__ __forceinline__ float rq_head(const float* X, int ldx, const float (&w)[16]) {
  const int lane = threadIdx.x & 63, row = lane >> 2, q = lane & 3;
  float s = 0.f;
#pragma unroll
  for (int j = 0; j < 16; ++j) s = fmaf(X[row * ldx + 4 * j + q], w[j], s);
  return quad_sum(s);
}

template <int KS>
__device__ __forceinline__ void rt_load(float (&w)[KS], const float* __restrict__ W, int ldw, int col, int K) {
  const int kq = (threadIdx.x & 63) >> 4;
#pragma unroll
  for (int s = 0; s < KS; ++s) w[s] = W[min(4 * s + kq, K - 1) * ldw + col];
}
template <int KS>
__device__ __forceinline__ void rt_load_k(float (&w)[KS], const float* __restrict__ W, int ldw, int col, int K) {
  const int kq = (threadIdx.x & 63) >> 4;
#pragma unroll
  for (int s = 0; s < KS; ++s) {
    w[s] = 0.f;
    if (4 * s < K) w[s] = W[min(4 * s + kq, K - 1) * ldw + col];
  }
}
template <int KS>
__device__ __forceinline__ void rt_acc(f32x4& acc, const float* X, int ldx, int K, const float (&w)[KS]) {
  const int lane = threadIdx.x & 63, r = lane & 15, kq = lane >> 4;
  const float* xr = X + r * ldx;
  float x[KS];
#pragma unroll
  for (int s = 0; s < KS; ++s) {
    const int k = 4 * s + kq;
    const float v = xr[min(k, K - 1)];
    x[s] = k < K ? v : 0.f;
  }
  __builtin_amdgcn_sched_barrier(0);
#pragma unroll
  for (int s = 0; s < KS; ++s)
    if (4 * s < K) acc = MDP_MFMA(x[s], w[s], acc);
}

__device__ __forceinline__ void rdg_load(f32x4 (&w)[4], const float* __restrict__ W, int kk, bool ok) {
  const int kq = (threadIdx.x & 63) >> 4;
#pragma unroll
  for (int m = 0; m < 4; ++m) {
    const f32x4 v = ld4(W + kk * MDP_RH + 16 * kq + 4 * m);
    w[m] = ok ? v : f32x4{0.f, 0.f, 0.f, 0.f};
  }
}
__device__ __forceinline__ f32x4 rdg_acc(const float* dY, int ldy, const f32x4 (&w)[4]) {
  const int lane = threadIdx.x & 63, r = lane & 15, kq = lane >> 4;
  const float* yr = dY + r * ldy + 16 * kq;
  float x[16];
#pragma unroll
  for (int s = 0; s < 16; ++s) x[s] = yr[s];
  __builtin_amdgcn_sched_barrier(0);
  f32x4 acc = {0.f, 0.f, 0.f, 0.f};
#pragma unroll
  for (int s = 0; s < 16; ++s) acc = MDP_MFMA(x[s], w[s >> 2][s & 3], acc);
  return acc;
}

__device__ __forceinline__ void lds_signal(int* flag) {
  asm volatile("s_waitcnt lgkmcnt(0)" ::: "memory");
  if ((threadIdx.x & 63) == 0) __hip_atomic_fetch_add(flag, 1, __ATOMIC_RELAXED, __HIP_MEMORY_SCOPE_WORKGROUP);
}
__device__ __forceinline__ void lds_wait(int* flag, int n) {
  while (__hip_atomic_load(flag, __ATOMIC_RELAXED, __HIP_MEMORY_SCOPE_WORKGROUP) < n) __builtin_amdgcn_s_sleep(1);
  asm volatile("" ::: "memory");
}

__device__ __forceinline__ double sum16(double v) {
  const int lane = threadIdx.x & 63;
  v = lane < MDP_R ? v : 0.0;
  v += dpp_d<0xB1, 0xf>(v);
  v += dpp_d<0x4E, 0xf>(v);
  v += dpp_d<0x141, 0xf>(v);
  v += dpp_d<0x140, 0xf>(v);
  return v;
}

#ifndef MDP_NT_SLAB
#define MDP_NT_SLAB 0
#endif
__device__ __forceinline__ void slab_st(float* p, float v) {
#if MDP_NT_SLAB == 3
  asm volatile("global_store_dword %0, %1, off sc1" ::"v"(p), "v"(v) : "memory");
#elif MDP_NT_SLAB == 2
  __hip_atomic_store(p, v, __ATOMIC_RELAXED, __HIP_MEMORY_SCOPE_AGENT);
#elif MDP_NT_SLAB
  __builtin_nontemporal_store(v, p);
#else
  *p = v;
#endif
}
__device__ __forceinline__ void slab_st4(float* p, f32x4 v) {
#if MDP_NT_SLAB == 3
  asm volatile("global_store_dwordx4 %0, %1, off sc1" ::"v"(p), "v"(v) : "memory");
#elif MDP_NT_SLAB == 2
#pragma unroll
  for (int j = 0; j < 4; ++j) __hip_atomic_store(p + j, v[j], __ATOMIC_RELAXED, __HIP_MEMORY_SCOPE_AGENT);
#elif MDP_NT_SLAB
  __builtin_nontemporal_store(v, reinterpret_cast<f32x4*>(p));
#else
  *reinterpret_cast<f32x4*>(p) = v;
#endif
}
struct WgJob {
  const float* X;
  const float* dY;
  float* dW;
  int ldx, K, ldy, N;
};
template <int T>
__device__ __forceinline__ void wgrad_multi(const WgJob& j0, const WgJob& j1, const WgJob& j2, int w0, int wn) {
  const int lane = threadIdx.x & 63, wave = __builtin_amdgcn_readfirstlane(threadIdx.x >> 6);
  if (wave < w0 || wave >= w0 + wn) return;
  const int r = lane & 15, kq = lane >> 4;
  const int n0 = ((j0.K + 15) >> 4) * (j0.N >> 4);
  const int n1 = j1.K > 0 ? ((j1.K + 15) >> 4) * (j1.N >> 4) : 0;
  const int n2 = j2.K > 0 ? ((j2.K + 15) >> 4) * (j2.N >> 4) : 0;
  const int total = n0 + n1 + n2;
  for (int base = wave - w0; base < total; base += T * wn) {
    float a[T][4], g[T][4];
    float* dst[T];
    bool krem[T];
#pragma unroll
    for (int s = 0; s < T; ++s) {
      const int tv = base + s * wn;
      const int t = min(tv, total - 1);
      const bool in0 = t < n0, in1 = !in0 && t < n0 + n1;
      const float* X = in0 ? j0.X : (in1 ? j1.X : j2.X);
      const float* dY = in0 ? j0.dY : (in1 ? j1.dY : j2.dY);
      float* dW = in0 ? j0.dW : (in1 ? j1.dW : j2.dW);
      const int ldx = in0 ? j0.ldx : (in1 ? j1.ldx : j2.ldx);
      const int K = in0 ? j0.K : (in1 ? j1.K : j2.K);
      const int ldy = in0 ? j0.ldy : (in1 ? j1.ldy : j2.ldy);
// ... 51 lines not shown
```

maddpg_amd/csrc/mdp_kernels.h:

```cpp
#pragma once
#include <hip/hip_runtime.h>
#include <hip/hip_ext.h>
#include <stdint.h>

#include "mdp_topo.h"

struct CriticArgs {
  int agent, B;
  const float* theta;
  const float* target;
  const float* replay;
  const int32_t* idx;
  const float* u_tgt;
  uint64_t seed;
  const Ctl* ctl;
  double gamma;
  float inv_b;
  float* slab;
  int slab_stride;
  double* slab_stat;
  double* y_out;
  int group;
  Ctl* pf_ctl;
  int32_t* pf_out;
// ... 182 lines not shown
  float* replay;
  int64_t cap;
  float* pos;
  float* vel;
  int32_t* goal;
  int32_t* ep_step;
  float* ep_rew;
  float* eplog;
  int64_t eplog_cap;
  int eplog_by_env;
  Ctl* ctl;
  uint64_t seed;
  int E, env_base;
  const float* act_in;
  const float* u_in;
  uint32_t* ticket;
  float* bench;
  int pf_count;
  int32_t* pf_out;
  int nsteps;
  float* comm;
};

struct EnvResetArgs {
  EnvDesc env;
  uint64_t seed;
  uint32_t ctr;
  int env_base, E;
  float* pos;
  float* vel;
  int32_t* goal;
  int32_t* ep_step;
  float* ep_rew;
  float* comm;
};

struct EnvObsArgs {
  Topo topo;
  EnvDesc env;
  int E;
  const float* pos;
  const float* vel;
  const int32_t* goal;
  const float* comm;
  float* obs;
};

struct EvalEpArgs {
  Topo topo;
  EnvDesc env;
  const float* theta;
  uint64_t seed;
  uint32_t first;
  int episodes;
  int mode;
  const float* u_in;
  float* ret;
  float* bench;
};

struct EvalMuArgs : EvalEpArgs {
  const float* bank;
  const int32_t* table;
  int64_t set_stride;
  int matchups;
};

struct EvalArgs {
  const float* P;
  NDesc net;
  int in, rows;
  const float* x;
  float* out;
  int gumbel;
  const float* u;
  uint64_t seed;
  uint32_t stream, ctr;
  int act_w;
};

inline int mdp_device_units(int u) { return u <= 64 ? 64 : (u <= 128 ? 128 : 256); }

inline int mdp_r4(int n) { return (n + 3) & ~3; }
inline int mdp_ld(int c) { return c | 1; }
inline int lds_critic_bytes(const Topo& t, int G) {
  const int R = 16, ldr = mdp_ld(t.row_stride), ldc = mdp_ld(t.cin_max), S = R * (t.H + 1);
  return 4 * (mdp_r4(R * ldr) + 2 * mdp_r4(R * ldc) + 2 * mdp_r4((G + 1) * S) + mdp_r4((G + 1) * R * 8) +
              mdp_r4(R) + mdp_r4(MDP_MAX_AGENTS + 4));
}
inline int lds_actor_bytes(const Topo& t) {
  const int R = 16, ldr = mdp_ld(t.row_stride), ldc = mdp_ld(t.cin_max), S = R * (t.H + 1);
  return 4 * (mdp_r4(R * ldr) + mdp_r4(R * ldc) + 6 * mdp_r4(S) + 5 * mdp_r4(R * 8) + mdp_r4(5 * t.H));
}
#define MDP_LDS_BUDGET (160 * 1024)
inline int lds_critic_r_bytes(const Topo& t, int agent) {
  const int R = 16, ldr = mdp_ld(t.row_stride), LH = 68, LD = 65;
  const int na = t.ag[agent].local_q ? 1 : t.n, ldA = mdp_ld(5 * na);
  return 4 * (mdp_r4(R * ldr) + mdp_r4(R * ldA) + 3 * R * 8 + 6 * R * LH + 4 * R * LH + 3 * R + 2 * mdp_r4(R * LD));
}
inline int lds_actor_r_bytes(const Topo& t) {
  const int R = 16, ldr = mdp_ld(t.row_stride), LH = 68, LD = 65;
  return 4 * (mdp_r4(R * ldr) + 4 * R * 8 + R + 3 * R * LH + 4 * mdp_r4(R * LD) + 2 * 64 * 16 + 4 * R + 4 * 5 * 64);
}
inline int lds_critic_pre_bytes(const Topo& t) {
  const int R = 16, ldr = mdp_ld(t.row_stride), LH = 68, ldA = mdp_ld(5 * t.n);
  return 4 * (mdp_r4(R * ldr) + mdp_r4(R * ldA) + 3 * R * 8 + 6 * R * LH + 3 * R * LH + 4 * R + 16 * R);
}
inline bool grads_r_ok(const Topo& t, int agent) {
  if (t.H != 64) return false;
  const ADesc& ag = t.ag[agent];
  const int na = ag.local_q ? 1 : t.n;
  if (na > 3) return false;
  for (int j = 0; j < t.n; ++j)
    if (t.ag[j].obs_dim > 64) return false;
  if (ag.cin > 80) return false;
  if ((ag.local_q ? ag.obs_dim : t.sum_obs) > 64) return false;
  return 5 * na <= 20;
}
inline int lds_rollout_bytes(const Topo& t) {
  const int R = 16, ldr = mdp_ld(t.row_stride), ldh = t.H + 1;
  const int par = t.H == 64 ? 4 * (2 * R * 68 + R * 8) : 0;
  return 4 * (mdp_r4(R * ldr) + 2 * mdp_r4(R * ldh) + mdp_r4(R * 8) + par + 2 * mdp_r4(R * 2 * MDP_MAX_ENT) +
              mdp_r4(R * 3 * MDP_MAX_ENT) + mdp_r4(R * MDP_MAX_AGENTS) + mdp_r4(R));
}
inline int lds_eval_matchups_bytes(const Topo& t) { return lds_rollout_bytes(t) + 4 * mdp_r4(MDP_MAX_AGENTS); }
inline int lds_eval_bytes(int in, int H) {
  const int R = 16, ldx = mdp_ld(in), ldh = H + 1;
  return 4 * (mdp_r4(R * ldx) + 2 * mdp_r4(R * ldh) + mdp_r4(R * 8));
}

struct MdpLaunchEv {
  hipEvent_t start = nullptr, stop = nullptr;
};
MdpLaunchEv& mdp_launch_ev();
template <typename F, typename... Args>
inline void mdp_launch(F kernel, const dim3& grid, const dim3& block, uint32_t lds, hipStream_t s, Args... args) {
  MdpLaunchEv& e = mdp_launch_ev();
  if (e.start) {
    const hipEvent_t a = e.start, z = e.stop;
    e.start = e.stop = nullptr;
    hipExtLaunchKernelGGL(kernel, grid, block, lds, s, a, z, 0u, args...);
  } else {
    hipLaunchKernelGGL(kernel, grid, block, lds, s, args...);
  }
}

hipError_t mdp_launch_critic_grad(const CriticArgs& a, int H, int lds_bytes, hipStream_t s);
hipError_t mdp_launch_actor_grad(const ActorArgs& a, int H, int lds_bytes, hipStream_t s);
hipError_t mdp_launch_grad_pair(const GradPairArgs& a, int H, int lds_bytes, hipStream_t s);
hipError_t mdp_launch_critic_grad_r(const CriticArgs& a, int lds_bytes, hipStream_t s);
hipError_t mdp_launch_critic_grad_per(const CriticArgsPer& a, int H, int lds_bytes, hipStream_t s);
hipError_t mdp_launch_critic_grad_r_per(const CriticArgsPer& a, int lds_bytes, hipStream_t s);
hipError_t mdp_launch_actor_grad_r(const ActorArgs& a, int lds_bytes, hipStream_t s);
hipError_t mdp_launch_rollout(const RolloutArgs& a, int H, int lds_bytes, hipStream_t s);
hipError_t mdp_launch_eval(const EvalArgs& a, int H, int lds_bytes, hipStream_t s);
hipError_t mdp_launch_eval_episodes(const EvalEpArgs& a, int H, int lds_bytes, hipStream_t s);
hipError_t mdp_launch_eval_matchups(const EvalMuArgs& a, int H, int lds_bytes, hipStream_t s);
hipError_t mdp_launch_eval_reset(const EnvDesc& env, uint64_t seed, uint32_t first, int count, float* pos, float* vel,
                                 int32_t* goal, hipStream_t s);
hipError_t mdp_launch_apply(const ApplyArgs& a, hipStream_t s);
hipError_t mdp_launch_reduce(const ReduceArgs& a, hipStream_t s);
hipError_t mdp_launch_reduce_apply(const FusedApplyArgs& f, hipStream_t s);
#define MDP_RA_BATCH_MAX (2 * MDP_MAX_AGENTS)
struct RaBatch {
  const FusedApplyArgs* list = nullptr;
  int count = 0;
  int narrow = 0;
  int wg_start[MDP_RA_BATCH_MAX + 1] = {};
  int pf_count = 0;
  int32_t* pf_out = nullptr;
  Ctl* pf_ctl = nullptr;
};
int mdp_ra_grid(const FusedApplyArgs& f);
hipError_t mdp_ra_occupancy(int* per_cu);
hipError_t mdp_spin_kernels_scratch(int* bytes);
inline int mdp_ra_grid_of(const Topo& t, int agent, int net) {
  const NDesc& d = net ? t.ag[agent].critic : t.ag[agent].actor;
  const NDesc& o = net ? t.ag[agent].actor : t.ag[agent].critic;
  int g = 2;
  for (int k = 0; k < 6; ++k) {
    g += (d.t[k].rows * d.t[k].cols + MDP_RA_CHUNK - 1) / MDP_RA_CHUNK;
    if (!net) g += (o.t[k].rows * o.t[k].cols + MDP_APPLY_CHUNK - 1) / MDP_APPLY_CHUNK;
  }
  return g;
}
inline bool mdp_ra_fits(const Topo& t, int agent, int net, int capacity) {
  const NDesc& d = net ? t.ag[agent].critic : t.ag[agent].actor;
  for (int k = 0; k < 6; ++k)
    if ((d.t[k].rows * d.t[k].cols + MDP_RA_CHUNK - 1) / MDP_RA_CHUNK > MDP_RA_MAXCH) return false;
  return mdp_ra_grid_of(t, agent, net) <= capacity;
}
hipError_t mdp_launch_reduce_apply_batch(const RaBatch& b, hipStream_t s);
hipError_t mdp_ra_batch_occupancy(int* per_cu);
hipError_t mdp_launch_xchg_probe(const XchgDesc* xd, uint32_t ep, int nchunk, uint32_t* bad, uint32_t* fault,
                                 hipStream_t s);
hipError_t mdp_launch_make_index(Ctl* ctl, int count, int32_t* out, hipStream_t s);
hipError_t mdp_launch_polyak(float* target, const float* theta, int64_t n, float pa, float pb, const Ctl* ctl,
                             hipStream_t s);
hipError_t mdp_launch_gather(const float* replay, int stride, const int32_t* idx, int count, float* out,
                             hipStream_t s);
hipError_t mdp_launch_count_nonfinite(const float* p, int64_t n, uint32_t* cnt, hipStream_t s);
hipError_t mdp_launch_put_rows(float* replay, int stride, int64_t cap, int64_t next, const float* src, int64_t rows,
                               hipStream_t s);
hipError_t mdp_launch_put_agent(float* replay, int stride, const ADesc& ag, const int64_t* pos, const float* cols,
                                int64_t rows, hipStream_t s);
hipError_t mdp_launch_env_reset(const EnvResetArgs& a, hipStream_t s);
hipError_t mdp_launch_env_obs(const EnvObsArgs& a, hipStream_t s);
hipError_t mdp_launch_set_ring(Ctl* ctl, int64_t len, int64_t next, hipStream_t s);
```

maddpg_amd/csrc/mdp_kernels.hip:

```cpp
#include <type_traits>

#include "mdp_device.h"
#include "mdp_kernels.h"
#include "mdp_mt.h"

__global__ __launch_bounds__(1024) void k_make_index(Ctl* ctl, int count, int32_t* __restrict__ out) {
  make_index_block<1024>(ctl, count, out);
}

__device__ __forceinline__ void st_nt4(float* o, float4 v) {
  __builtin_nontemporal_store(v.x, o);
  __builtin_nontemporal_store(v.y, o + 1);
  __builtin_nontemporal_store(v.z, o + 2);
  __builtin_nontemporal_store(v.w, o + 3);
}

__global__ __launch_bounds__(256) void k_gather_rows(const float* __restrict__ replay, int stride,
                                                     const int32_t* __restrict__ idx, int count,
                                                     float* __restrict__ out) {
  const uint32_t v4 = (uint32_t)stride >> 2;
  const uint32_t total = (uint32_t)count * v4;
  const uint32_t step = gridDim.x * blockDim.x;
  uint32_t e = blockIdx.x * blockDim.x + threadIdx.x;
  for (; e + 3u * step < total; e += 4u * step) {
// ... 170 lines not shown
    a.beta[2] = p1;
    a.beta[3] = p2;
    a.beta[0] = p1 * a.b1;
    a.beta[1] = p2 * a.b2;
    if (a.bump_ctr) a.ctl->upd_ctr += 1u;
  }
  const int64_t el = e >> 3;
  const int q = (int)(e & 7);
  float s = 0.f;
  if (el < a.size) {
    const float* p = a.slab + el;
    float v[8], t[24];
#pragma unroll
    for (int k = 0; k < 8; ++k) {
      const int w = q + 8 * k;
      v[k] = w < a.nwg ? p[(int64_t)w * a.slab_stride] : 0.f;
    }
#pragma unroll
    for (int k = 0; k < 24; ++k) {
      const int w = q + 64 + 8 * k;
      t[k] = w < a.nwg ? p[(int64_t)w * a.slab_stride] : 0.f;
    }
#pragma unroll
    for (int k = 0; k < 24; ++k)
      if (q + 64 + 8 * k < a.nwg) s += t[k];
    for (int w = q + 256; w < a.nwg; w += 8) s += p[(int64_t)w * a.slab_stride];
#pragma unroll
    for (int k = 0; k < 8; ++k) s += v[k];
  }
  s = half_row_sum(s);
  if (el < a.size && q == 0) a.grad[a.off + el] = s;
}

__global__ __launch_bounds__(256) void k_apply(ApplyArgs a) {
  __shared__ double red[4];
  const int b = blockIdx.x;
  const int tid = threadIdx.x;
  const float b1p = a.beta[2], b2p = a.beta[3];
  if (b < a.blk[6]) {
    int t = 0;
    while (b >= a.blk[t + 1]) ++t;
    const TDesc td = a.net.t[t];
    const int n = td.rows * td.cols;
    const float* g = a.grad + td.off;
    constexpr int PT = MDP_APPLY_CHUNK / 256;
    const int e0 = (b - a.blk[t]) * MDP_APPLY_CHUNK;
    const int e1 = min(n, e0 + MDP_APPLY_CHUNK);
    float cg[PT], cm[PT], cv[PT], cth[PT], ctg[PT];
#pragma unroll
    for (int q = 0; q < PT; ++q) {
      const int e = min(e0 + tid + q * 256, e1 - 1);
      const int64_t i = td.off + e;
      cg[q] = g[e];
      cm[q] = a.m[i];
      cv[q] = a.v[i];
      cth[q] = a.theta[i];
      ctg[q] = a.polyak ? a.target[i] : 0.f;
    }
    double ss = 0.0;
    for (int f0 = tid; f0 < n; f0 += 8 * blockDim.x) {
      float v[8];
#pragma unroll
      for (int q = 0; q < 8; ++q) {
        const int e = f0 + q * blockDim.x;
        v[q] = e < n ? g[min(e, n - 1)] * a.scale : 0.f;
      }
#pragma unroll
      for (int q = 0; q < 8; ++q) ss += (double)v[q] * (double)v[q];
    }
    ss = block_sum_d(ss, red);
    const float norm = (float)sqrt(ss);
    const float clip = a.clip;
    const float denom = fmaxf(norm, clip);
    const float one = 1.0f;
    const float alpha = a.lr * sqrtf(one - b2p) / (one - b1p);
    const float c1 = one - a.b1, c2 = one - a.b2;
#pragma unroll
    for (int q = 0; q < PT; ++q) {
      const int e = e0 + tid + q * 256;
      if (e < e1) {
        const int64_t i = td.off + e;
        const float gc = ((cg[q] * a.scale) * clip) / denom;
        const float m = cm[q] + (gc - cm[q]) * c1;
        const float v = cv[q] + (gc * gc - cv[q]) * c2;
        const float th = cth[q] - (m * alpha) / (sqrtf(v) + a.eps);
        a.m[i] = m;
        a.v[i] = v;
        a.theta[i] = th;
        if (a.polyak) a.target[i] = a.pa * ctg[q] + a.pb * th;
      }
    }
  } else if (a.polyak && b < a.blk[6] + a.oblk[6]) {
    const int bb = b - a.blk[6];
    int t = 0;
    while (bb >= a.oblk[t + 1]) ++t;
    const TDesc td = a.other.t[t];
    const int n = td.rows * td.cols;
    const int e0 = (bb - a.oblk[t]) * MDP_APPLY_CHUNK;
    const int e1 = min(n, e0 + MDP_APPLY_CHUNK);
    for (int e = e0 + tid; e < e1; e += blockDim.x) {
      const int64_t i = td.off + e;
      a.target[i] = a.pa * a.target[i] + a.pb * a.theta[i];
    }
  } else if (a.stats_mode) {
    if (tid < 64) {
      double s0 = 0.0, s1 = 0.0, s2 = 0.0, s3 = 0.0;
      for (int w = tid; w < a.nwg; w += 64) {
        const double* st = a.slab_stat + (int64_t)w * 8;
        s0 += st[0];
        s1 += st[1];
        s2 += st[2];
        s3 += st[3];
      }
      s0 = wave_sum_d(s0);
      s1 = wave_sum_d(s1);
      if (a.stats_mode == 1) {
        s2 = wave_sum_d(s2);
        s3 = wave_sum_d(s3);
        const double mean_y = s1 / a.B;
        double dv = 0.0;
        for (int i = tid; i < a.B; i += 64) {
          const double d = a.y[i] - mean_y;
          dv += d * d;
        }
        dv = wave_sum_d(dv);
        if (tid == 0) {
          a.stats_out[0] = s0 / a.B;
          a.stats_out[2] = mean_y;
          a.stats_out[3] = s2 / a.B;
          a.stats_out[4] = s3 / a.B;
          a.stats_out[5] = sqrt(dv / a.B);
        }
      } else if (tid == 0) {
        a.stats_out[1] = -s0 / a.B + (double)a.reg * (s1 / ((double)a.B * (a.stats_mode - 1)));
      }
    }
  }
}

namespace {

struct EnvTile {
  float* pos;
  float* vel;
};

__device__ inline float softplus_f(float x) { return fmaxf(x, 0.f) + log1pf(expf(-fabsf(x))); }

__device__ inline float dist2(const float* p, int a, int b) {
  const float dx = p[2 * a] - p[2 * b], dy = p[2 * a + 1] - p[2 * b + 1];
  return sqrtf(dx * dx + dy * dy);
}

__device__ inline void env_obs(const EnvDesc& E, const float* p, const float* v, int goal, int i, float* o) {
  const int n = E.n_agents, L = E.n_landmarks;
  int c = 0;
  switch (E.scenario) {
    case MDP_SCN_SIMPLE:
      o[c++] = v[2 * i];
      o[c++] = v[2 * i + 1];
      for (int l = 0; l < L; ++l) {
        o[c++] = p[2 * (n + l)] - p[2 * i];
        o[c++] = p[2 * (n + l) + 1] - p[2 * i + 1];
      }
      break;
    case MDP_SCN_SPREAD:
      o[c++] = v[2 * i];
      o[c++] = v[2 * i + 1];
      o[c++] = p[2 * i];
      o[c++] = p[2 * i + 1];
      for (int l = 0; l < L; ++l) {
        o[c++] = p[2 * (n + l)] - p[2 * i];
        o[c++] = p[2 * (n + l) + 1] - p[2 * i + 1];
      }
      for (int j = 0; j < n; ++j) {
        if (j == i) continue;
        o[c++] = p[2 * j] - p[2 * i];
        o[c++] = p[2 * j + 1] - p[2 * i + 1];
      }
      for (int j = 0; j < n; ++j) {
        if (j == i) continue;
        o[c++] = 0.f;
        o[c++] = 0.f;
      }
      break;
    case MDP_SCN_ADVERSARY:
      if (!E.adversary[i]) {
        o[c++] = p[2 * (n + goal)] - p[2 * i];
        o[c++] = p[2 * (n + goal) + 1] - p[2 * i + 1];
      }
      for (int l = 0; l < L; ++l) {
        o[c++] = p[2 * (n + l)] - p[2 * i];
        o[c++] = p[2 * (n + l) + 1] - p[2 * i + 1];
      }
      for (int j = 0; j < n; ++j) {
        if (j == i) continue;
        o[c++] = p[2 * j] - p[2 * i];
        o[c++] = p[2 * j + 1] - p[2 * i + 1];
      }
      break;
    case MDP_SCN_TAG:
      o[c++] = v[2 * i];
      o[c++] = v[2 * i + 1];
      o[c++] = p[2 * i];
      o[c++] = p[2 * i + 1];
      for (int l = 0; l < L; ++l) {
        o[c++] = p[2 * (n + l)] - p[2 * i];
        o[c++] = p[2 * (n + l) + 1] - p[2 * i + 1];
      }
      for (int j = 0; j < n; ++j) {
        if (j == i) continue;
        o[c++] = p[2 * j] - p[2 * i];
        o[c++] = p[2 * j + 1] - p[2 * i + 1];
      }
      for (int j = 0; j < n; ++j) {
        if (j == i || E.adversary[j]) continue;
        o[c++] = v[2 * j];
        o[c++] = v[2 * j + 1];
      }
      break;
    default:
      break;
  }
}

__device__ inline void env_obs_comm(const EnvDesc& E, const float* p, const float* v, int goal, int i, float* o,
                                    const float* comm) {
  const int n = E.n_agents, L = E.n_landmarks;
  int c = 0;
  if (E.scenario != MDP_SCN_SPEAKER_LISTENER) return;
  if (i == 0) {
    for (int l = 0; l < L; ++l) o[c++] = l == goal ? 0.65f : 0.15f;
  } else {
    o[c++] = v[2 * i];
    o[c++] = v[2 * i + 1];
    for (int l = 0; l < L; ++l) {
      o[c++] = p[2 * (n + l)] - p[2 * i];
      o[c++] = p[2 * (n + l) + 1] - p[2 * i + 1];
    }
    for (int k = 0; k < env_dim_c(E.scenario); ++k) o[c++] = comm ? comm[k] : 0.f;
  }
}

__device__ inline void env_reward(const EnvDesc& E, const float* p, int goal, float* rew) {
  const int n = E.n_agents, L = E.n_landmarks;
  switch (E.scenario) {
    case MDP_SCN_SIMPLE: {
      const float dx = p[0] - p[2 * n], dy = p[1] - p[2 * n + 1];
      rew[0] = -(dx * dx + dy * dy);
      break;
    }
    case MDP_SCN_SPEAKER_LISTENER: {
      const int g = n + goal;
      const float dx = p[2] - p[2 * g], dy = p[3] - p[2 * g + 1];
      const float r = -(dx * dx + dy * dy);
      rew[0] = rew[1] = r + r;
      break;
    }
    case MDP_SCN_SPREAD: {
      float base = 0.f;
      for (int l = 0; l < L; ++l) {
        float m = INFINITY;
        for (int a = 0; a < n; ++a) m = fminf(m, dist2(p, a, n + l));
        base -= m;
      }
      float tot = 0.f;
      for (int i = 0; i < n; ++i) {
        float r = base;
        for (int a = 0; a < n; ++a)
          if (dist2(p, a, i) < E.size[a] + E.size[i]) r -= 1.f;
        tot += r;
      }
      for (int i = 0; i < n; ++i) rew[i] = tot;
      break;
    }
    case MDP_SCN_ADVERSARY: {
      const int g = n + goal;
      float adv = 0.f, mg = INFINITY;
      for (int a = 0; a < n; ++a) {
        if (E.adversary[a]) adv += dist2(p, a, g);
        else mg = fminf(mg, dist2(p, a, g));
      }
      for (int i = 0; i < n; ++i) {
        if (E.adversary[i]) {
          const float dx = p[2 * i] - p[2 * g], dy = p[2 * i + 1] - p[2 * g + 1];
          rew[i] = -(dx * dx + dy * dy);
        } else {
          rew[i] = -mg + adv;
        }
      }
      break;
    }
    case MDP_SCN_TAG: {
      float caught = 0.f;
      for (int g = 0; g < n; ++g) {
        if (E.adversary[g]) continue;
        for (int a = 0; a < n; ++a)
          if (E.adversary[a] && dist2(p, g, a) < E.size[g] + E.size[a]) caught += 1.f;
      }
      for (int i = 0; i < n; ++i) {
        if (E.adversary[i]) {
          rew[i] = 10.f * caught;
        } else {
          float r = 0.f;
          for (int a = 0; a < n; ++a)
            if (E.adversary[a] && dist2(p, a, i) < E.size[a] + E.size[i]) r -= 10.f;
          for (int d = 0; d < 2; ++d) {
            const float x = fabsf(p[2 * i + d]);
            float bnd = 0.f;
            if (x < 0.9f) bnd = 0.f;
            else if (x < 1.0f) bnd = (x - 0.9f) * 10.f;
            else bnd = fminf(expf(2.f * x - 2.f), 10.f);
            r -= bnd;
          }
          rew[i] = r;
        }
      }
      break;
    }
    default:
      break;
  }
}

__device__ inline void env_bench(const EnvDesc& E, const float* p, int goal, float* out) {
  const int n = E.n_agents, L = E.n_landmarks;
  for (int q = 0; q < n * MDP_BENCH_W; ++q) out[q] = 0.f;
  switch (E.scenario) {
    case MDP_SCN_SPREAD: {
      float min_dists = 0.f, occupied = 0.f;
      for (int l = 0; l < L; ++l) {
        float m = INFINITY;
        for (int a = 0; a < n; ++a) m = fminf(m, dist2(p, a, n + l));
        min_dists += m;
        if (m < 0.1f) occupied += 1.f;
      }
      for (int i = 0; i < n; ++i) {
        float coll = 0.f;
        for (int a = 0; a < n; ++a)
          if (dist2(p, a, i) < E.size[a] + E.size[i]) coll += 1.f;
        float* o = out + i * MDP_BENCH_W;
        o[0] = -min_dists - coll;
        o[1] = coll;
        o[2] = min_dists;
        o[3] = occupied;
      }
      break;
    }
    case MDP_SCN_ADVERSARY: {
      const int g = n + goal;
      for (int i = 0; i < n; ++i) {
        float* o = out + i * MDP_BENCH_W;
        auto sq = [&](int b) {
          const float dx = p[2 * i] - p[2 * b], dy = p[2 * i + 1] - p[2 * b + 1];
          return dx * dx + dy * dy;
        };
        if (E.adversary[i]) {
          o[0] = sq(g);
        } else {
          for (int l = 0; l < L; ++l) o[l] = sq(n + l);
          o[L] = sq(g);
        }
      }
      break;
    }
    case MDP_SCN_TAG: {
      for (int i = 0; i < n; ++i) {
        if (!E.adversary[i]) continue;
        float c = 0.f;
        for (int a = 0; a < n; ++a)
          if (!E.adversary[a] && dist2(p, a, i) < E.size[a] + E.size[i]) c += 1.f;
        out[i * MDP_BENCH_W] = c;
      }
      break;
    }
    default:
      break;
  }
}

__device__ inline void env_physics_tile(const EnvDesc& E, float* sp, float* sv, const float* act, int ldr, float* f,
                                        int nvalid) {
  const int n = E.n_agents, ne = E.n_agents + E.n_landmarks;
  const float k = 1e-3f;
  for (int q = threadIdx.x; q < nvalid * ne; q += MDP_NT) {
    const int r = q / ne, e = q - r * ne;
    const float* p = sp + r * 2 * MDP_MAX_ENT;
    float fx = 0.f, fy = 0.f, has = 0.f;
    if (e < n) {
      const float* a = act + r * ldr + e * MDP_ACT_DIM;
      fx = (a[1] - a[2]) * E.accel[e];
      fy = (a[3] - a[4]) * E.accel[e];
      has = 1.f;
    }
    if (E.collide[e] && E.movable[e]) {
      for (int o = 0; o < ne; ++o) {
        if (o == e || !E.collide[o]) continue;
        const int a = min(o, e), b = max(o, e);
        const float dx = p[2 * a] - p[2 * b], dy = p[2 * a + 1] - p[2 * b + 1];
        const float dist = sqrtf(dx * dx + dy * dy);
        const float dmin = E.size[a] + E.size[b];
        const float pen = softplus_f(-(dist - dmin) / k) * k;
        const float sx = 1e2f * dx / dist * pen, sy = 1e2f * dy / dist * pen;
        if (e == a) {
          fx = sx + fx;
          fy = sy + fy;
        } else {
          fx = -sx + fx;
          fy = -sy + fy;
        }
        has = 1.f;
      }
    }
    float* fr = f + r * 3 * MDP_MAX_ENT;
    fr[e] = fx;
    fr[MDP_MAX_ENT + e] = fy;
    fr[2 * MDP_MAX_ENT + e] = has;
  }
  __syncthreads();
  for (int q = threadIdx.x; q < nvalid * ne; q += MDP_NT) {
    const int r = q / ne, e = q - r * ne;
    if (!E.movable[e]) continue;
    float* p = sp + r * 2 * MDP_MAX_ENT;
    float* v = sv + r * 2 * MDP_MAX_ENT;
    const float* fr = f + r * 3 * MDP_MAX_ENT;
    float vx = v[2 * e] * (1.f - 0.25f), vy = v[2 * e + 1] * (1.f - 0.25f);
    if (fr[2 * MDP_MAX_ENT + e] != 0.f) {
      vx += (fr[e] / 1.f) * 0.1f;
      vy += (fr[MDP_MAX_ENT + e] / 1.f) * 0.1f;
    }
    const float ms = E.max_speed[e];
    if (ms >= 0.f) {
      const float spd = sqrtf(vx * vx + vy * vy);
      if (spd > ms) {
        const float s = sqrtf(vx * vx + vy * vy);
        vx = vx / s * ms;
        vy = vy / s * ms;
      }
    }
    v[2 * e] = vx;
    v[2 * e + 1] = vy;
    p[2 * e] += vx * 0.1f;
    p[2 * e + 1] += vy * 0.1f;
  }
  __syncthreads();
}

__device__ inline void env_reset_one(const EnvDesc& E, uint64_t seed, uint32_t stream, uint32_t ctr, uint32_t env,
                                     float* p, float* v, int32_t* goal) {
  const int n = E.n_agents, ne = E.n_agents + E.n_landmarks;
  const uint2 key = make_uint2((uint32_t)seed, (uint32_t)(seed >> 32));
  uint4 blk = make_uint4(0u, 0u, 0u, 0u);
  int c = 0;
  auto next_u = [&]() -> float {
    const int w = c & 3;
    if (w == 0) blk = Philox::gen(make_uint4(env, ctr, stream, (uint32_t)(c >> 2)), key);
    ++c;
    return u01(w == 0 ? blk.x : w == 1 ? blk.y : w == 2 ? blk.z : blk.w);
  };
  for (int e = 0; e < ne; ++e) {
    float lo = -1.f, hi = 1.f, sc = 1.f;
    if (e >= n) {
      if (E.scenario == MDP_SCN_SPREAD || E.scenario == MDP_SCN_ADVERSARY) sc = 0.8f;
      if (E.scenario == MDP_SCN_TAG) {
        lo = -0.9f;
        hi = 0.9f;
      }
    }
    const float ux = next_u();
    const float uy = next_u();
    p[2 * e] = sc * (lo + (hi - lo) * ux);
    p[2 * e + 1] = sc * (lo + (hi - lo) * uy);
    v[2 * e] = 0.f;
    v[2 * e + 1] = 0.f;
  }
  if (E.scenario == MDP_SCN_ADVERSARY || E.scenario == MDP_SCN_SPEAKER_LISTENER) {
    int g = (int)(next_u() * E.n_landmarks);
    *goal = g < E.n_landmarks ? g : E.n_landmarks - 1;
  } else {
    *goal = 0;
  }
}

}

__global__ __launch_bounds__(256) void k_env_reset(EnvResetArgs a) {
  const int e = blockIdx.x * blockDim.x + threadIdx.x;
  if (e >= a.E) return;
  const int ne = a.env.n_agents + a.env.n_landmarks;
  float p[2 * MDP_MAX_ENT], v[2 * MDP_MAX_ENT];
  int32_t g;
  env_reset_one(a.env, a.seed, 0x30000u, a.ctr, (uint32_t)(a.env_base + e), p, v, &g);
  for (int q = 0; q < 2 * ne; ++q) {
    a.pos[(int64_t)e * 2 * ne + q] = p[q];
    a.vel[(int64_t)e * 2 * ne + q] = v[q];
  }
  a.goal[e] = g;
  a.ep_step[e] = 0;
  for (int j = 0; j < a.env.n_agents; ++j) a.ep_rew[(int64_t)e * a.env.n_agents + j] = 0.f;
  if (a.comm)
    for (int q = 0; q < a.env.n_agents * MDP_ACT_DIM; ++q) a.comm[(int64_t)e * a.env.n_agents * MDP_ACT_DIM + q] = 0.f;
}

__global__ __launch_bounds__(256) void k_env_obs(EnvObsArgs a) {
  const int e = blockIdx.x * blockDim.x + threadIdx.x;
  if (e >= a.E) return;
  const int ne = a.env.n_agents + a.env.n_landmarks;
  const float* p = a.pos + (int64_t)e * 2 * ne;
  const float* v = a.vel + (int64_t)e * 2 * ne;
  float* o = a.obs + (int64_t)e * a.topo.sum_obs;
  for (int j = 0; j < a.env.n_agents; ++j) {
    if (a.comm) env_obs_comm(a.env, p, v, a.goal[e], j, o + a.topo.ag[j].obs_off, a.comm + (int64_t)e * a.env.n_agents * MDP_ACT_DIM);
    else env_obs(a.env, p, v, a.goal[e], j, o + a.topo.ag[j].obs_off);
  }
}

__device__ __forceinline__ void rollout_finish(const RolloutArgs& a, int64_t next, int64_t len) {
  if (last_block(a.ticket) && threadIdx.x == 0) {
    const int64_t moved = (int64_t)a.nsteps * a.E;
    a.ctl->next = (next + moved) % a.cap;
    a.ctl->len = len + moved < a.cap ? len + moved : a.cap;
    a.ctl->env_steps += (uint64_t)a.nsteps;
    a.ctl->episodes += atomicExch(&a.ctl->ep_pending, 0u);
    *a.ticket = 0u;
  }
}

template <int H, bool MULTI>
__global__ __launch_bounds__(MDP_NT) void k_rollout(RolloutArgs a) {
  extern __shared__ __attribute__((aligned(16))) float lds[];
  MDP_TL_ROLLOUT();
  const Topo& T = a.topo;
  const EnvDesc& E = a.env;
  const int n = E.n_agents, ne = E.n_agents + E.n_landmarks;
  const int ldr = lds_ld(T.row_stride), ldh = H + 1;
  LdsCarve cv(lds);
  float* rowt = cv.take(MDP_R * ldr);
  float* h1 = cv.take(MDP_R * ldh);
  float* h2 = cv.take(MDP_R * ldh);
  float* lg = cv.take(MDP_R * 8);
  constexpr int PAR_W = H == 64 ? MDP_NW * (2 * MDP_R * MDP_RLH + MDP_R * 8) : 0;
  float* hpar = cv.take(PAR_W);
  float* sp = cv.take(MDP_R * 2 * MDP_MAX_ENT);
  float* sv = cv.take(MDP_R * 2 * MDP_MAX_ENT);
  float* sfo = cv.take(MDP_R * 3 * MDP_MAX_ENT);
  float* epr = cv.take(MDP_R * MDP_MAX_AGENTS);
  int* sgoal = reinterpret_cast<int*>(cv.take(MDP_R));

  const int tid = threadIdx.x;
  const int e0 = ((int)blockIdx.x - (a.pf_count > 0 ? 1 : 0)) * MDP_R;
  const int nvalid = min(MDP_R, a.E - e0);
  const Ctl* ctlv = a.ctl;
  asm volatile("" : "+v"(ctlv));
  typedef __attribute__((address_space(1))) const Ctl gCtl;
  const gCtl* gc = (const gCtl*)ctlv;
  if (a.pf_count > 0 && blockIdx.x == 0) {
    const int64_t next = gc->next, len = gc->len;
    MDP_STAMP(48);
    make_index_block<MDP_NT>(a.ctl, a.pf_count, a.pf_out, (uint32_t)(len + a.E < a.cap ? len + a.E : a.cap));
    MDP_STAMP(49);
    rollout_finish(a, next, len);
    return;
  }

  MDP_STAMP(40);
  int goal = 0, ep_st = 0;
  if (tid < MDP_R && tid < nvalid) {
    goal = a.goal[e0 + tid];
    ep_st = a.ep_step[e0 + tid];
  }
  static_assert(MDP_R * 2 * MDP_MAX_ENT <= 2 * MDP_NT && MDP_R * MDP_MAX_AGENTS <= MDP_NT, "rollout prologue");
  float pv[2] = {0.f, 0.f}, vv[2] = {0.f, 0.f}, er = 0.f;
  const int er_r = tid / n, er_j = tid - er_r * n;
  if (tid < MDP_R * n && er_r < nvalid) er = a.ep_rew[(int64_t)(e0 + er_r) * n + er_j];
#pragma unroll
  for (int u = 0; u < 2; ++u) {
    const int q = tid + u * MDP_NT, r = q / (2 * ne), c = q - r * 2 * ne;
    if (q < MDP_R * 2 * ne && r < nvalid) {
      pv[u] = a.pos[(int64_t)(e0 + r) * 2 * ne + c];
      vv[u] = a.vel[(int64_t)(e0 + r) * 2 * ne + c];
    }
  }
  const int64_t next_raw = gc->next, len_raw = gc->len;
  const uint32_t step_raw = (uint32_t)gc->env_steps;
  const int64_t ep_base_raw = gc->episodes;
  if (tid < MDP_R * n) epr[er_r * MDP_MAX_AGENTS + er_j] = er;
#pragma unroll
  for (int u = 0; u < 2; ++u) {
    const int q = tid + u * MDP_NT, r = q / (2 * ne), c = q - r * 2 * ne;
    if (q < MDP_R * 2 * ne) {
      sp[r * 2 * MDP_MAX_ENT + c] = pv[u];
      sv[r * 2 * MDP_MAX_ENT + c] = vv[u];
    }
  }
  if (tid < MDP_R) sgoal[tid] = (int)ctr_use((uint32_t)goal);
  __shared__ int s_nterm;
  int ep_done = 0;
  const int nsteps = MULTI ? a.nsteps : 1;
  for (int sidx = 0; sidx < nsteps; ++sidx) {
  if (MULTI && sidx > 0) __syncthreads();
  auto step_s = [&]() { return ctr_use(step_raw) + (uint32_t)sidx; };
  const int64_t next_s = next_raw + (int64_t)sidx * a.E;
  for (int q = tid; q < MDP_R * ldr; q += MDP_NT) rowt[q] = 0.f;
  if (MULTI && tid == 0) s_nterm = 0;
  __syncthreads();
  static_assert(MDP_R * MDP_MAX_AGENTS <= MDP_NT, "rollout obs: one pass");
  if (tid < MDP_R * n) {
    const int r = tid / n, j = tid - r * n;
    if (__builtin_expect(a.comm != nullptr, 0))
      env_obs_comm(E, sp + r * 2 * MDP_MAX_ENT, sv + r * 2 * MDP_MAX_ENT, sgoal[r], j, rowt + r * ldr + T.ag[j].obs_off,
                   r < nvalid ? a.comm + (int64_t)(e0 + r) * n * MDP_ACT_DIM : nullptr);
    else
      env_obs(E, sp + r * 2 * MDP_MAX_ENT, sv + r * 2 * MDP_MAX_ENT, sgoal[r], j, rowt + r * ldr + T.ag[j].obs_off);
  }
  __syncthreads();

  MDP_STAMP(41);
  bool par = false;
  if constexpr (H == 64) {
    par = !a.act_in && n <= MDP_NW;
    for (int j = 0; j < n; ++j) par = par && T.ag[j].obs_dim <= 64;
  }
  if (par) {
    if constexpr (H == 64) {
      const int wave = __builtin_amdgcn_readfirstlane(tid >> 6), lane = tid & 63, r = lane & 15, kq = lane >> 4;
      if (wave < n) {
        const int j = wave;
        const ADesc& aj = T.ag[j];
        const NDesc& an = aj.actor;
        const float* P = a.theta;
        f32x4 w1[16], w2[16];
        float w3[16];
        rf_load<16>(w1, P + an.t[0].off, aj.obs_dim);
        rf_load<16>(w2, P + an.t[2].off, MDP_RH);
        rh_load(w3, P + an.t[4].off, MDP_ACT_DIM);
        const f32x4 b1 = ld4(P + an.t[1].off + 4 * r), b2 = ld4(P + an.t[3].off + 4 * r);
        const float b3 = P[an.t[5].off + min(r, MDP_ACT_DIM - 1)];
        float u[MDP_ACT_DIM];
        if (lane < MDP_R) {
          if (a.u_in) {
            for (int k = 0; k < MDP_ACT_DIM; ++k)
              u[k] = lane < nvalid ? a.u_in[((int64_t)(e0 + lane) * n + j) * MDP_ACT_DIM + k] : 0.5f;
          } else {
            uniforms5(a.seed, 0x10000u | (uint32_t)j, step_s(), (uint32_t)(a.env_base + e0 + lane), u);
          }
        }
        float* h1j = hpar + j * (2 * MDP_R * MDP_RLH + MDP_R * 8);
        float* h2j = h1j + MDP_R * MDP_RLH;
        float* lgj = h2j + MDP_R * MDP_RLH;
        {
          f32x4 acc[4];
          rf_zero(acc);
          rf_acc<16>(acc, rowt + aj.obs_off, ldr, aj.obs_dim, w1);
          rf_store<true>(acc, b1, h1j, MDP_RLH);
        }
        wave_sync();
        {
          f32x4 acc[4];
          rf_zero(acc);
          rf_acc<16>(acc, h1j, MDP_RLH, MDP_RH, w2);
          rf_store<true>(acc, b2, h2j, MDP_RLH);
        }
        wave_sync();
        {
          const f32x4 acc = rh_acc(h2j, MDP_RLH, w3);
          if (r < MDP_ACT_DIM) {
#pragma unroll
            for (int i = 0; i < 4; ++i) lgj[(kq * 4 + i) * 8 + r] = acc[i] + b3;
          }
        }
        wave_sync();
        if (lane < MDP_R) gumbel_softmax(lgj + lane * 8, u, rowt + lane * ldr + aj.act_off, topo_act_w(T, j));
      }
      __syncthreads();
      MDP_STAMP(42);
    }
  }
  for (int j = 0; j < (par ? 0 : n); ++j) {
    const ADesc& aj = T.ag[j];
    if (!a.act_in) {
      bool pf = false;
      if constexpr (H == 64 && MDP_NW == 4) {
        if (aj.obs_dim <= 4 * MDP_KC) {
          mlp_fwd_tile_pf<H>(rowt + aj.obs_off, ldr, aj.obs_dim, a.theta, aj.actor, h1, h2, ldh, lg, 8);
          pf = true;
        }
      }
      if (!pf) mlp_fwd_tile<H>(rowt + aj.obs_off, ldr, aj.obs_dim, a.theta, aj.actor, h1, h2, ldh, lg, 8);
    }
    if (tid < MDP_R) {
      float* dst = rowt + tid * ldr + aj.act_off;
      if (a.act_in) {
        for (int k = 0; k < MDP_ACT_DIM; ++k)
          dst[k] = tid < nvalid ? a.act_in[((int64_t)(e0 + tid) * n + j) * MDP_ACT_DIM + k] : 0.f;
      } else {
        float u[MDP_ACT_DIM];
        if (a.u_in) {
          for (int k = 0; k < MDP_ACT_DIM; ++k)
            u[k] = tid < nvalid ? a.u_in[((int64_t)(e0 + tid) * n + j) * MDP_ACT_DIM + k] : 0.5f;
        } else {
          uniforms5(a.seed, 0x10000u | (uint32_t)j, step_s(), (uint32_t)(a.env_base + e0 + tid), u);
        }
        gumbel_softmax(lg + tid * 8, u, dst, topo_act_w(T, j));
      }
    }
    __syncthreads();
    if (j < 4) MDP_STAMP(42 + j);
  }

  env_physics_tile(E, sp, sv, rowt + T.ag[0].act_off, ldr, sfo, nvalid);
  bool term = false;
  if (tid < nvalid) {
    const float* p = sp + tid * 2 * MDP_MAX_ENT;
    float* row = rowt + tid * ldr;
    float* rew = row + T.ag[0].rew_off;
    env_reward(E, p, goal, rew);
    if (a.bench) env_bench(E, p, goal, a.bench + (int64_t)(e0 + tid) * n * MDP_BENCH_W);
    for (int j = 0; j < n; ++j) row[T.ag[j].done_off] = 0.f;
    const int e = e0 + tid;
    float tot = 0.f;
    for (int j = 0; j < n; ++j) {
      const float r = epr[tid * MDP_MAX_AGENTS + j] + rew[j];
      epr[tid * MDP_MAX_AGENTS + j] = r;
      a.ep_rew[(int64_t)e * n + j] = r;
      tot += r;
    }
    const int st = (int)ctr_use((uint32_t)ep_st) + 1;
    term = st >= E.max_ep_len;
    if (term) {
      const uint32_t q = atomicAdd(&a.ctl->ep_pending, 1u);
      const int64_t slot = ep_base_raw + (a.eplog_by_env ? (int64_t)(ep_done + e) : (int64_t)q);
      float* lgp = a.eplog + (slot % a.eplog_cap) * (1 + n);
      lgp[0] = tot;
      for (int j = 0; j < n; ++j) {
        lgp[1 + j] = epr[tid * MDP_MAX_AGENTS + j];
        a.ep_rew[(int64_t)e * n + j] = 0.f;
        if (MULTI) epr[tid * MDP_MAX_AGENTS + j] = 0.f;
      }
      if (MULTI) {
        atomicAdd(&s_nterm, 1);
        ep_st = 0;
      }
    } else {
      a.ep_step[e] = st;
      if (MULTI) ep_st = st;
    }
    if (__builtin_expect(a.comm != nullptr, 0)) {
      float* cm = a.comm + (int64_t)e * n * MDP_ACT_DIM;
      for (int j = 0; j < n; ++j)
        for (int k = 0; k < MDP_ACT_DIM; ++k)
          cm[j * MDP_ACT_DIM + k] = (term || env_silent(E.scenario, j)) ? 0.f : row[T.ag[j].act_off + k];
    }
  } else if (tid >= 64 && tid - 64 < nvalid * n) {
    const int q = tid - 64, r = q / n, j = q - r * n;
    if (__builtin_expect(a.comm != nullptr, 0))
      env_obs_comm(E, sp + r * 2 * MDP_MAX_ENT, sv + r * 2 * MDP_MAX_ENT, sgoal[r], j, rowt + r * ldr + T.ag[j].nobs_off,
                   rowt + r * ldr + T.ag[0].act_off);
    else
      env_obs(E, sp + r * 2 * MDP_MAX_ENT, sv + r * 2 * MDP_MAX_ENT, sgoal[r], j, rowt + r * ldr + T.ag[j].nobs_off);
  }
  static_assert(64 + MDP_R * MDP_MAX_AGENTS <= MDP_NT, "rollout obs': one pass on waves 1..");
  __syncthreads();
  if (MULTI) ep_done += s_nterm;
  if (term) {
    const int e = e0 + tid;
    int32_t g;
    env_reset_one(E, a.seed, 0x20000u, step_s(), (uint32_t)(a.env_base + e), sp + tid * 2 * MDP_MAX_ENT,
                  sv + tid * 2 * MDP_MAX_ENT, &g);
    a.goal[e] = g;
    a.ep_step[e] = 0;
    if (MULTI) {
      goal = g;
      sgoal[tid] = g;
    }
  }
  __syncthreads();
  MDP_STAMP(46);
  const int v4 = T.row_stride >> 2;
  for (int q = tid; q < nvalid * v4; q += MDP_NT) {
    const int r = q / v4, c4 = q - r * v4;
    const float* s = rowt + r * ldr + c4 * 4;
    const int64_t dst = (next_s + e0 + r) % a.cap;
    *reinterpret_cast<float4*>(a.replay + dst * T.row_stride + c4 * 4) = make_float4(s[0], s[1], s[2], s[3]);
  }
  }
  for (int q = tid; q < nvalid * 2 * ne; q += MDP_NT) {
    const int r = q / (2 * ne), c = q - r * 2 * ne;
    a.pos[(int64_t)(e0 + r) * 2 * ne + c] = sp[r * 2 * MDP_MAX_ENT + c];
    a.vel[(int64_t)(e0 + r) * 2 * ne + c] = sv[r * 2 * MDP_MAX_ENT + c];
  }
  MDP_STAMP(47);
  rollout_finish(a, next_raw, len_raw);
}

template <int H, class Args = EvalEpArgs>
__global__ __launch_bounds__(MDP_NT) void k_eval_episodes(Args a) {
  constexpr bool MU = std::is_same<Args, EvalMuArgs>::value;
  extern __shared__ __attribute__((aligned(16))) float lds[];
  const Topo& T = a.topo;
  const EnvDesc& E = a.env;
  const int n = E.n_agents;
  const int ldr = lds_ld(T.row_stride), ldh = H + 1;
  LdsCarve cv(lds);
  float* rowt = cv.take(MDP_R * ldr);
  float* h1 = cv.take(MDP_R * ldh);
  float* h2 = cv.take(MDP_R * ldh);
  float* lg = cv.take(MDP_R * 8);
  constexpr int PAR_W = H == 64 ? MDP_NW * (2 * MDP_R * MDP_RLH + MDP_R * 8) : 0;
  float* hpar = cv.take(PAR_W);
  float* sp = cv.take(MDP_R * 2 * MDP_MAX_ENT);
  float* sv = cv.take(MDP_R * 2 * MDP_MAX_ENT);
  float* sfo = cv.take(MDP_R * 3 * MDP_MAX_ENT);
  float* epr = cv.take(MDP_R * MDP_MAX_AGENTS);
  int* sgoal = reinterpret_cast<int*>(cv.take(MDP_R));
  int* stab = MU ? reinterpret_cast<int*>(cv.take(MDP_MAX_AGENTS)) : nullptr;
  static_assert(MDP_R * MDP_MAX_AGENTS * MDP_BENCH_W <= MDP_R * (H + 1), "record tile fits h1");
  float* rec = h1;

  const int tid = threadIdx.x;
  const int i0 = (int)blockIdx.x * MDP_R;
  const int nvalid = min(MDP_R, a.episodes - i0);
  const bool comm = env_dim_c(E.scenario) > 0;
  const bool mean = a.mode == MDP_EVAL_MEAN;

  for (int q = tid; q < MDP_R * ldr; q += MDP_NT) rowt[q] = 0.f;
  for (int q = tid; q < MDP_R * 2 * MDP_MAX_ENT; q += MDP_NT) sp[q] = sv[q] = 0.f;
  if (tid < MDP_R * MDP_MAX_AGENTS) epr[tid] = 0.f;
  if (tid < MDP_R) sgoal[tid] = 0;
  if constexpr (MU) {
    if (tid < n) stab[tid] = a.table[(int64_t)blockIdx.y * n + tid];
  }
  __syncthreads();
  if (tid < nvalid) {
    int32_t g;
    env_reset_one(E, a.seed, 0x60000u, 0u, a.first + (uint32_t)(i0 + tid), sp + tid * 2 * MDP_MAX_ENT,
                  sv + tid * 2 * MDP_MAX_ENT, &g);
    sgoal[tid] = g;
  }

  bool par = false;
  if constexpr (H == 64) {
    par = n <= MDP_NW;
    for (int j = 0; j < n; ++j) par = par && T.ag[j].obs_dim <= 64;
  }
  const int wave = __builtin_amdgcn_readfirstlane(tid >> 6), lane = tid & 63, r16 = lane & 15, kq = lane >> 4;
  f32x4 w1[16], w2[16], b1 = {0.f, 0.f, 0.f, 0.f}, b2 = {0.f, 0.f, 0.f, 0.f};
  float w3[16], b3 = 0.f;
  if constexpr (H == 64) {
    if (par && wave < n) {
      const ADesc& aj = T.ag[wave];
      const NDesc& an = aj.actor;
      const float* P = a.theta;
      if constexpr (MU) P = a.bank + (int64_t)a.table[(int64_t)blockIdx.y * n + wave] * a.set_stride;
      rf_load<16>(w1, P + an.t[0].off, aj.obs_dim);
      rf_load<16>(w2, P + an.t[2].off, MDP_RH);
      rh_load(w3, P + an.t[4].off, MDP_ACT_DIM);
      b1 = ld4(P + an.t[1].off + 4 * r16);
      b2 = ld4(P + an.t[3].off + 4 * r16);
      b3 = P[an.t[5].off + min(r16, MDP_ACT_DIM - 1)];
    }
  }
  float bsum[MDP_BENCH_W];
#pragma unroll
  for (int k = 0; k < MDP_BENCH_W; ++k) bsum[k] = 0.f;
  const int br = tid / n, bj = tid - br * n;
  __syncthreads();

  const int nst = E.max_ep_len;
  for (int t = 0; t < nst; ++t) {
    auto sample = [&](const float* logits, int row, int j, float* dst) {
      float gn[MDP_ACT_DIM];
      if (mean) {
#pragma unroll
        for (int k = 0; k < MDP_ACT_DIM; ++k) gn[k] = 0.f;
      } else {
        float u[MDP_ACT_DIM];
        if (a.u_in) {
          for (int k = 0; k < MDP_ACT_DIM; ++k)
            u[k] = row < nvalid ? a.u_in[(((int64_t)(i0 + row) * nst + t) * n + j) * MDP_ACT_DIM + k] : 0.5f;
        } else {
          uniforms5(a.seed, 0x70000u | (uint32_t)j, (uint32_t)t, a.first + (uint32_t)(i0 + row), u);
        }
        gumbel_noise5(u, gn);
      }
      gumbel_softmax_pre(logits, gn, dst, topo_act_w(T, j));
    };
    if (tid < MDP_R * n) {
      const int r = tid / n, j = tid - r * n;
      if (comm)
        env_obs_comm(E, sp + r * 2 * MDP_MAX_ENT, sv + r * 2 * MDP_MAX_ENT, sgoal[r], j, rowt + r * ldr + T.ag[j].obs_off,
                     t > 0 ? rowt + r * ldr + T.ag[0].act_off : nullptr);
      else
        env_obs(E, sp + r * 2 * MDP_MAX_ENT, sv + r * 2 * MDP_MAX_ENT, sgoal[r], j, rowt + r * ldr + T.ag[j].obs_off);
    }
    __syncthreads();
    if (par) {
      if constexpr (H == 64) {
        if (wave < n) {
          const int j = wave;
          const ADesc& aj = T.ag[j];
          float* h1j = hpar + j * (2 * MDP_R * MDP_RLH + MDP_R * 8);
          float* h2j = h1j + MDP_R * MDP_RLH;
          float* lgj = h2j + MDP_R * MDP_RLH;
          {
            f32x4 acc[4];
            rf_zero(acc);
            rf_acc<16>(acc, rowt + aj.obs_off, ldr, aj.obs_dim, w1);
            rf_store<true>(acc, b1, h1j, MDP_RLH);
          }
          wave_sync();
          {
            f32x4 acc[4];
            rf_zero(acc);
            rf_acc<16>(acc, h1j, MDP_RLH, MDP_RH, w2);
            rf_store<true>(acc, b2, h2j, MDP_RLH);
          }
          wave_sync();
          {
            const f32x4 acc = rh_acc(h2j, MDP_RLH, w3);
            if (r16 < MDP_ACT_DIM) {
#pragma unroll
              for (int i = 0; i < 4; ++i) lgj[(kq * 4 + i) * 8 + r16] = acc[i] + b3;
            }
          }
          wave_sync();
          if (lane < MDP_R) sample(lgj + lane * 8, lane, j, rowt + lane * ldr + aj.act_off);
        }
        __syncthreads();
      }
    }
    for (int j = 0; j < (par ? 0 : n); ++j) {
      const ADesc& aj = T.ag[j];
      const float* Pj = a.theta;
      if constexpr (MU) Pj = a.bank + (int64_t)stab[j] * a.set_stride;
      bool pf = false;
      if constexpr (H == 64 && MDP_NW == 4) {
        if (aj.obs_dim <= 4 * MDP_KC) {
          mlp_fwd_tile_pf<H>(rowt + aj.obs_off, ldr, aj.obs_dim, Pj, aj.actor, h1, h2, ldh, lg, 8);
          pf = true;
        }
      }
      if (!pf) mlp_fwd_tile<H>(rowt + aj.obs_off, ldr, aj.obs_dim, Pj, aj.actor, h1, h2, ldh, lg, 8);
      if (tid < MDP_R) sample(lg + tid * 8, tid, j, rowt + tid * ldr + aj.act_off);
      __syncthreads();
    }

    env_physics_tile(E, sp, sv, rowt + T.ag[0].act_off, ldr, sfo, nvalid);
    if (tid < nvalid) {
      const float* p = sp + tid * 2 * MDP_MAX_ENT;
      float* rew = rowt + tid * ldr + T.ag[0].rew_off;
      env_reward(E, p, sgoal[tid], rew);
      if (a.bench) env_bench(E, p, sgoal[tid], rec + tid * n * MDP_BENCH_W);
      for (int j = 0; j < n; ++j) epr[tid * MDP_MAX_AGENTS + j] = epr[tid * MDP_MAX_AGENTS + j] + rew[j];
    }
    if (a.bench) {
      __syncthreads();
      if (tid < MDP_R * n && br < nvalid) {
#pragma unroll
        for (int k = 0; k < MDP_BENCH_W; ++k) bsum[k] += rec[(br * n + bj) * MDP_BENCH_W + k];
      }
    }
    __syncthreads();
  }

  if (tid < MDP_R * n && br < nvalid) {
    int64_t o = (int64_t)(i0 + br) * n + bj;
    if constexpr (MU) o += (int64_t)blockIdx.y * a.episodes * n;
    a.ret[o] = epr[br * MDP_MAX_AGENTS + bj];
    if (a.bench) {
#pragma unroll
      for (int k = 0; k < MDP_BENCH_W; ++k) a.bench[o * MDP_BENCH_W + k] = bsum[k];
    }
  }
}

__global__ __launch_bounds__(256) void k_eval_reset(EnvDesc env, uint64_t seed, uint32_t first, int count, float* pos,
                                                    float* vel, int32_t* goal) {
  const int e = blockIdx.x * blockDim.x + threadIdx.x;
  if (e >= count) return;
  const int ne = env.n_agents + env.n_landmarks;
  float p[2 * MDP_MAX_ENT], v[2 * MDP_MAX_ENT];
  int32_t g;
  env_reset_one(env, seed, 0x60000u, 0u, first + (uint32_t)e, p, v, &g);
  for (int q = 0; q < 2 * ne; ++q) {
    pos[(int64_t)e * 2 * ne + q] = p[q];
    vel[(int64_t)e * 2 * ne + q] = v[q];
  }
  goal[e] = g;
}

template <int H>
__global__ __launch_bounds__(MDP_NT) void k_mlp_eval(EvalArgs a) {
  extern __shared__ __attribute__((aligned(16))) float lds[];
  const int ldx = lds_ld(a.in), ldh = H + 1;
  LdsCarve cv(lds);
  float* x = cv.take(MDP_R * ldx);
  float* h1 = cv.take(MDP_R * ldh);
  float* h2 = cv.take(MDP_R * ldh);
  float* lg = cv.take(MDP_R * 8);
  const int r0 = blockIdx.x * MDP_R;
  const int nvalid = min(MDP_R, a.rows - r0);
  for (int q = threadIdx.x; q < MDP_R * a.in; q += MDP_NT) {
    const int r = q / a.in, c = q - r * a.in;
    x[r * ldx + c] = r < nvalid ? a.x[(int64_t)(r0 + r) * a.in + c] : 0.f;
  }
  __syncthreads();
  mlp_fwd_tile<H>(x, ldx, a.in, a.P, a.net, h1, h2, ldh, lg, 8);
  const int tid = threadIdx.x;
  if (tid < nvalid) {
    const int row = r0 + tid;
    if (a.gumbel) {
      float u[MDP_ACT_DIM], act[MDP_ACT_DIM];
      if (a.u) {
        for (int k = 0; k < MDP_ACT_DIM; ++k) u[k] = a.u[(int64_t)row * MDP_ACT_DIM + k];
      } else {
        uniforms5(a.seed, a.stream, a.ctr, (uint32_t)row, u);
      }
      gumbel_softmax(lg + tid * 8, u, act, a.act_w);
      for (int k = 0; k < MDP_ACT_DIM; ++k) a.out[(int64_t)row * MDP_ACT_DIM + k] = act[k];
    } else {
      for (int k = 0; k < a.net.out; ++k) a.out[(int64_t)row * a.net.out + k] = lg[tid * 8 + k];
    }
  }
}

#define MDP_CHECK_LAUNCH() \
  do {                     \
    hipError_t e_ = hipGetLastError(); \
    if (e_ != hipSuccess) return e_;   \
  } while (0)

template <int H>
static hipError_t launch_rollout_t(const RolloutArgs& a, int lds_bytes, hipStream_t s) {
  const int grid = (a.E + MDP_R - 1) / MDP_R + (a.pf_count > 0 ? 1 : 0);
  if (a.nsteps > 1)
    mdp_launch(k_rollout<H, true>, dim3(grid), dim3(MDP_NT), lds_bytes, s, a);
  else
    mdp_launch(k_rollout<H, false>, dim3(grid), dim3(MDP_NT), lds_bytes, s, a);
  MDP_CHECK_LAUNCH();
  return hipSuccess;
}
template <int H>
static hipError_t launch_eval_t(const EvalArgs& a, int lds_bytes, hipStream_t s) {
  const int grid = (a.rows + MDP_R - 1) / MDP_R;
  hipLaunchKernelGGL(k_mlp_eval<H>, dim3(grid), dim3(MDP_NT), lds_bytes, s, a);
  MDP_CHECK_LAUNCH();
  return hipSuccess;
}

static int set_lds_limit_done = 0;
template <int H>
static void raise_lds_limits() {
  (void)hipFuncSetAttribute((const void*)k_rollout<H, false>, hipFuncAttributeMaxDynamicSharedMemorySize, 128 * 1024);
  (void)hipFuncSetAttribute((const void*)k_rollout<H, true>, hipFuncAttributeMaxDynamicSharedMemorySize, 128 * 1024);
  (void)hipFuncSetAttribute((const void*)k_mlp_eval<H>, hipFuncAttributeMaxDynamicSharedMemorySize, 128 * 1024);
  (void)hipFuncSetAttribute((const void*)k_eval_episodes<H>, hipFuncAttributeMaxDynamicSharedMemorySize, 128 * 1024);
  (void)hipFuncSetAttribute((const void*)k_eval_episodes<H, EvalMuArgs>, hipFuncAttributeMaxDynamicSharedMemorySize,
                            128 * 1024);
}
static void ensure_lds_limits() {
  if (!set_lds_limit_done) {
    raise_lds_limits<64>();
    raise_lds_limits<128>();
    raise_lds_limits<256>();
    (void)hipGetLastError();
    set_lds_limit_done = 1;
  }
}

hipError_t mdp_launch_rollout(const RolloutArgs& a, int H, int lds_bytes, hipStream_t s) {
  ensure_lds_limits();
  switch (H) {
    case 64: return launch_rollout_t<64>(a, lds_bytes, s);
    case 128: return launch_rollout_t<128>(a, lds_bytes, s);
    case 256: return launch_rollout_t<256>(a, lds_bytes, s);
    default: return hipErrorInvalidValue;
  }
}
hipError_t mdp_launch_eval(const EvalArgs& a, int H, int lds_bytes, hipStream_t s) {
  ensure_lds_limits();
  switch (H) {
    case 64: return launch_eval_t<64>(a, lds_bytes, s);
    case 128: return launch_eval_t<128>(a, lds_bytes, s);
    case 256: return launch_eval_t<256>(a, lds_bytes, s);
    default: return hipErrorInvalidValue;
  }
}
template <int H>
static hipError_t launch_eval_episodes_t(const EvalEpArgs& a, int lds_bytes, hipStream_t s) {
  mdp_launch(k_eval_episodes<H>, dim3((a.episodes + MDP_R - 1) / MDP_R), dim3(MDP_NT), lds_bytes, s, a);
  MDP_CHECK_LAUNCH();
  return hipSuccess;
}
hipError_t mdp_launch_eval_episodes(const EvalEpArgs& a, int H, int lds_bytes, hipStream_t s) {
  ensure_lds_limits();
  switch (H) {
    case 64: return launch_eval_episodes_t<64>(a, lds_bytes, s);
    case 128: return launch_eval_episodes_t<128>(a, lds_bytes, s);
    case 256: return launch_eval_episodes_t<256>(a, lds_bytes, s);
    default: return hipErrorInvalidValue;
  }
}
template <int H>
static hipError_t launch_eval_matchups_t(const EvalMuArgs& a, int lds_bytes, hipStream_t s) {
  const dim3 grid((a.episodes + MDP_R - 1) / MDP_R, a.matchups);
  mdp_launch(k_eval_episodes<H, EvalMuArgs>, grid, dim3(MDP_NT), lds_bytes, s, a);
  MDP_CHECK_LAUNCH();
  return hipSuccess;
}
hipError_t mdp_launch_eval_matchups(const EvalMuArgs& a, int H, int lds_bytes, hipStream_t s) {
  ensure_lds_limits();
  switch (H) {
    case 64: return launch_eval_matchups_t<64>(a, lds_bytes, s);
    case 128: return launch_eval_matchups_t<128>(a, lds_bytes, s);
    case 256: return launch_eval_matchups_t<256>(a, lds_bytes, s);
    default: return hipErrorInvalidValue;
  }
}
hipError_t mdp_launch_eval_reset(const EnvDesc& env, uint64_t seed, uint32_t first, int count, float* pos, float* vel,
                                 int32_t* goal, hipStream_t s) {
  hipLaunchKernelGGL(k_eval_reset, dim3((count + 255) / 256), dim3(256), 0, s, env, seed, first, count, pos, vel, goal);
  MDP_CHECK_LAUNCH();
  return hipSuccess;
}
hipError_t mdp_launch_apply(const ApplyArgs& a, hipStream_t s) {
  const int grid = a.blk[6] + (a.polyak ? a.oblk[6] : 0) + (a.stats_mode ? 1 : 0);
  mdp_launch(k_apply, dim3(grid), dim3(256), 0, s, a);
  MDP_CHECK_LAUNCH();
  return hipSuccess;
}
hipError_t mdp_launch_reduce(const ReduceArgs& a, hipStream_t s) {
  const int grid = (int)((a.size * 8 + 255) / 256);
  mdp_launch(k_reduce, dim3(grid), dim3(256), 0, s, a);
  MDP_CHECK_LAUNCH();
  return hipSuccess;
}
hipError_t mdp_launch_make_index(Ctl* ctl, int count, int32_t* out, hipStream_t s) {
  mdp_launch(k_make_index, dim3(1), dim3(1024), 0, s, ctl, count, out);
  MDP_CHECK_LAUNCH();
  return hipSuccess;
}
__global__ __launch_bounds__(256) void k_polyak(float* __restrict__ target, const float* __restrict__ theta,
                                                int64_t n4, float pa, float pb, const Ctl* ctl) {
  if (__hip_atomic_load(&ctl->fault, __ATOMIC_RELAXED, __HIP_MEMORY_SCOPE_AGENT) != 0u) return;
  for (int64_t i = (int64_t)blockIdx.x * 256 + threadIdx.x; i < n4; i += (int64_t)gridDim.x * 256) {
    const f32x4 tg = reinterpret_cast<const f32x4*>(target)[i];
    const f32x4 th = reinterpret_cast<const f32x4*>(theta)[i];
    f32x4 o;
#pragma unroll
    for (int j = 0; j < 4; ++j) o[j] = pa * tg[j] + pb * th[j];
    reinterpret_cast<f32x4*>(target)[i] = o;
  }
}
hipError_t mdp_launch_polyak(float* target, const float* theta, int64_t n, float pa, float pb, const Ctl* ctl,
                             hipStream_t s) {
  const int64_t n4 = n / 4;
  const int grid = (int)std::min<int64_t>(1024, (n4 + 255) / 256);
  mdp_launch(k_polyak, dim3(grid > 0 ? grid : 1), dim3(256), 0, s, target, theta, n4, pa, pb, ctl);
  MDP_CHECK_LAUNCH();
  return hipSuccess;
}
hipError_t mdp_launch_gather(const float* replay, int stride, const int32_t* idx, int count, float* out,
                             hipStream_t s) {
  const int v4 = stride >> 2;
  const int per = (int)((((int64_t)1 << 31) - 1) / v4);
  for (int b0 = 0; b0 < count; b0 += per) {
    const int n = count - b0 < per ? count - b0 : per;
    const int64_t total = (int64_t)n * v4;
    int grid = (int)((total + 255) / 256);
    if (grid > 4096) grid = 4096;
    if (grid < 1) grid = 1;
    hipLaunchKernelGGL(k_gather_rows, dim3(grid), dim3(256), 0, s, replay, stride, idx + b0, n,
                       out + (int64_t)b0 * stride);
    MDP_CHECK_LAUNCH();
  }
  return hipSuccess;
}
hipError_t mdp_launch_count_nonfinite(const float* p, int64_t n, uint32_t* cnt, hipStream_t s) {
  int grid = (int)((n + 255) / 256);
  if (grid > 2048) grid = 2048;
  if (grid < 1) grid = 1;
  hipLaunchKernelGGL(k_count_nonfinite, dim3(grid), dim3(256), 0, s, p, n, cnt);
  MDP_CHECK_LAUNCH();
  return hipSuccess;
}
hipError_t mdp_launch_put_rows(float* replay, int stride, int64_t cap, int64_t next, const float* src, int64_t rows,
                               hipStream_t s) {
  const int64_t total = rows * (stride >> 2);
  int grid = (int)((total + 255) / 256);
  if (grid > 4096) grid = 4096;
  if (grid < 1) grid = 1;
  hipLaunchKernelGGL(k_put_rows, dim3(grid), dim3(256), 0, s, replay, stride, cap, next, src, rows);
  MDP_CHECK_LAUNCH();
  return hipSuccess;
}
hipError_t mdp_launch_put_agent(float* replay, int stride, const ADesc& ag, const int64_t* pos, const float* cols,
                                int64_t rows, hipStream_t s) {
  const int64_t total = rows * (2 * ag.obs_dim + MDP_ACT_DIM + 2);
  int grid = (int)((total + 255) / 256);
  if (grid > 4096) grid = 4096;
  if (grid < 1) grid = 1;
  hipLaunchKernelGGL(k_put_agent, dim3(grid), dim3(256), 0, s, replay, stride, ag.obs_off, ag.act_off, ag.nobs_off,
                     ag.rew_off, ag.done_off, ag.obs_dim, pos, cols, rows);
  MDP_CHECK_LAUNCH();
  return hipSuccess;
}
hipError_t mdp_launch_env_reset(const EnvResetArgs& a, hipStream_t s) {
  hipLaunchKernelGGL(k_env_reset, dim3((a.E + 255) / 256), dim3(256), 0, s, a);
  MDP_CHECK_LAUNCH();
  return hipSuccess;
}
hipError_t mdp_launch_env_obs(const EnvObsArgs& a, hipStream_t s) {
  hipLaunchKernelGGL(k_env_obs, dim3((a.E + 255) / 256), dim3(256), 0, s, a);
  MDP_CHECK_LAUNCH();
  return hipSuccess;
}

__global__ void k_set_ring(Ctl* ctl, int64_t len, int64_t next) {
  ctl->len = len;
  ctl->next = next;
}
hipError_t mdp_launch_set_ring(Ctl* ctl, int64_t len, int64_t next, hipStream_t s) {
  hipLaunchKernelGGL(k_set_ring, dim3(1), dim3(1), 0, s, ctl, len, next);
  MDP_CHECK_LAUNCH();
  return hipSuccess;
}

#ifdef MDP_TIMELINE
extern "C" int mdp_debug_tl_roll(unsigned long long* out, int reset) {
  const size_t n = sizeof(unsigned long long) * MDP_TL_WG * 2;
  if (reset) {
    void* p = nullptr;
    if (hipGetSymbolAddress(&p, HIP_SYMBOL(g_mdp_tl_roll)) != hipSuccess) return -1;
    return hipMemset(p, 0, n) == hipSuccess && hipDeviceSynchronize() == hipSuccess ? 0 : -1;
  }
  return hipMemcpyFromSymbol(out, HIP_SYMBOL(g_mdp_tl_roll), n) == hipSuccess ? 0 : -1;
}
#endif

#ifdef MDP_STAMPS
extern "C" int mdp_debug_stamps_k(unsigned long long* out, int n) {
  return hipMemcpyFromSymbol(out, HIP_SYMBOL(g_mdp_stamps), sizeof(unsigned long long) * n) == hipSuccess ? 0 : -1;
}
#endif
```

maddpg_amd/csrc/mdp_topo.h:

```cpp
#pragma once
#include <stdint.h>

#include "../../include/maddpg_hip.h"

#define MDP_MAX_ENT 16

struct TDesc {
  int off, rows, cols;
};
struct NDesc {
  TDesc t[6];
  int off, size, in, out;
};
struct ADesc {
  NDesc actor, critic;
  int obs_dim, obs_off, act_off, nobs_off, rew_off, done_off;
  int local_q, cin, a_in_off;
};
struct Topo {
  int n, H, row_stride, sum_obs, cin_max, obs_max;
  ADesc ag[MDP_MAX_AGENTS];
  uint32_t act_w4;
  float reg_scale_w[MDP_ACT_DIM];
};
#if defined(__HIPCC__)
__host__ __device__
#endif
inline int topo_act_w(const Topo& t, int j) { return (int)((t.act_w4 >> (4 * j)) & 7u); }
inline void topo_set_act_w(Topo& t, int j, int w) {
  t.act_w4 = (t.act_w4 & ~(7u << (4 * j))) | ((uint32_t)w << (4 * j));
}

struct EnvDesc {
  int scenario, n_agents, n_landmarks, n_adv, max_ep_len;
  float size[MDP_MAX_ENT];
  float accel[MDP_MAX_AGENTS];
  float max_speed[MDP_MAX_ENT];
  int collide[MDP_MAX_ENT];
  int movable[MDP_MAX_ENT];
  int adversary[MDP_MAX_AGENTS];
};
#if defined(__HIPCC__)
__host__ __device__
#endif
inline int env_dim_c(int scenario) { return scenario == MDP_SCN_SPEAKER_LISTENER ? 3 : 0; }
#if defined(__HIPCC__)
__host__ __device__
#endif
inline bool env_silent(int scenario, int agent) { return !(scenario == MDP_SCN_SPEAKER_LISTENER && agent == 0); }

struct Ctl {
  uint32_t mt[624];
  int32_t mt_pos;
  int32_t pad0;
  int64_t len;
  int64_t next;
  int64_t env_steps;
  int64_t episodes;
  uint32_t ticket[8];
  uint32_t upd_ctr;
  uint32_t fault;
  uint32_t xstep[16];
  uint32_t ep_pending;
  uint32_t pad1;
  uint64_t xw_ticks;
  uint64_t xw_count;
  uint64_t xw_max;
  uint32_t nonfinite;
  uint32_t pad2;
};
```

maddpg_amd/engine.py:

```python
import ctypes
import os

import numpy as np
import torch

from . import _lib
from ._lib import MdpConfig, MdpTensorInfo

TENSOR_NAMES = ("W1", "b1", "W2", "b2", "W3", "b3")

UPDATE_STAT_DTYPES = (np.float32, np.float32, np.float64, np.float64, np.float32, np.float64)


def update_stats(vals):
    return [dt(v) for dt, v in zip(UPDATE_STAT_DTYPES, list(vals))]


def read_checkpoint(fname, path, n, sets):
    from .common import tf_checkpoint as tfc
    if tfc.is_bundle(fname) and os.path.isfile(path):
        t_npz, t_tf1 = os.stat(path).st_mtime_ns, os.stat(fname + ".index").st_mtime_ns
        if t_npz == t_tf1:
            import warnings
            warnings.warn(f"both {path} and the TF1 bundle {fname}.index exist with the same modification "
# ... 529 lines not shown
        self._c("mdp_dp_init", bytes(uid), int(world), int(rank))

    @staticmethod
    def dp_unique_id():
        buf = ctypes.create_string_buffer(128)
        if _lib.load().mdp_dp_unique_id(buf) != 0:
            raise _lib.MdpError("mdp_dp_unique_id failed (librccl.so.1 not loadable?)")
        return buf.raw

    def dp_init_from_dist(self, world, rank):
        import torch.distributed as dist
        obj = [None]
        if rank == 0:
            try:
                obj[0] = Engine.dp_unique_id()
            except Exception:
                obj[0] = None
        dist.broadcast_object_list(obj, src=0)
        if obj[0] is None:
            return False
        self.dp_init(world, rank, obj[0])
        return True

    def dp_xgmi_open(self, world, rank):
        buf = ctypes.create_string_buffer(64)
        self._c("mdp_dp_xgmi_open", int(world), int(rank), buf)
        return buf.raw

    def dp_xgmi_connect(self, handles):
        self._c("mdp_dp_xgmi_connect", b"".join(bytes(x) for x in handles))

    def dp_xgmi_probe(self):
        bad = ctypes.c_int32(0)
        self._c("mdp_dp_xgmi_probe", ctypes.byref(bad))
        return bad.value

    def dp_xgmi_init_from_dist(self, world, rank):
        from .parallel import xgmi_handshake
        eng = self

        class _Ops:
            device = eng.device
            open = staticmethod(eng.dp_xgmi_open)
            connect = staticmethod(eng.dp_xgmi_connect)
            probe = staticmethod(eng.dp_xgmi_probe)

            @staticmethod
            def enable():
                eng._c("mdp_dp_xgmi_enable")

            @staticmethod
            def close():
                eng._c("mdp_dp_xgmi_close")

        ok, err = xgmi_handshake(_Ops, world, rank)
        if not ok and err is not None:
            import sys
            print(f"[rank {rank}] xGMI exchange unavailable ({err}); using RCCL", file=sys.stderr)
        return ok

    DP_KINDS = {0: None, 1: "rccl", 2: "xgmi"}

    def dp_info(self):
        out = (ctypes.c_int32 * 4)()
        self._c("mdp_dp_info", out)
        return {"kind": self.DP_KINDS[out[0]], "ranks": out[1], "rank": out[2], "peers": out[3]}

    def dp_exchange_stats(self, reset=False):
        out = (ctypes.c_double * 4)()
        self._c("mdp_dp_exchange_stats", out, 1 if reset else 0)
        return {"chunk_exchanges": int(out[0]), "mean_us": out[1], "max_us": out[2], "total_us": out[3]}

    def dp_exchange_stats_enable(self, on=True):
        self._c("mdp_dp_exchange_stats_enable", 1 if on else 0)

    def param_checksum(self):
        out = []
        for name in ("theta", "target", "adam_m", "adam_v", "beta"):
            w = self.region(name, torch.int32).to(torch.int64)
            pos = torch.arange(1, w.numel() + 1, device=w.device, dtype=torch.int64)
            out += [int(w.sum().item()), int(((w & 0xFFFF) * pos).sum().item())]
        return out

    def set_graphs(self, on=True):
        self._c("mdp_set_graphs", 1 if on else 0)

    def critic_grad(self, agent, idx, u_tgt=None):
        B, n, A = self.batch_size, self.n, _lib.ACT_DIM
        self._sized("idx", idx, B)
        self._sized("u_tgt", u_tgt, n * B * A)
        idx = idx.to(self.device, torch.int32).contiguous()
        u_tgt = None if u_tgt is None else u_tgt.to(self.device, torch.float32).contiguous()
        self._c("mdp_critic_grad", agent, self._ptr(idx), self._ptr(u_tgt))
        self._keep = (idx, u_tgt)

    def actor_grad(self, agent, idx, u_act=None):
        B, A = self.batch_size, _lib.ACT_DIM
        self._sized("idx", idx, B)
        self._sized("u_act", u_act, B * A)
        idx = idx.to(self.device, torch.int32).contiguous()
        u_act = None if u_act is None else u_act.to(self.device, torch.float32).contiguous()
        self._c("mdp_actor_grad", agent, self._ptr(idx), self._ptr(u_act))
        self._keep = (idx, u_act)

    def reduce_grad(self, agent, net):
        self._c("mdp_reduce_grad", agent, net)

    def apply_grad(self, agent, net, scale=1.0):
        self._c("mdp_apply_grad", agent, net, float(scale))

    def index_slot(self, agent):
        return self.region("index", torch.int32)[agent * self.batch_size:(agent + 1) * self.batch_size]

    def stats(self, agent):
        out = (ctypes.c_double * 6)()
        self._c("mdp_get_stats", agent, out)
        return list(out)

    def check_finite(self):
        out = ctypes.c_int64()
        self._c("mdp_check_finite", ctypes.byref(out))
        return int(out.value)

    def stats_future(self, agent):
        src = self.region("stats", torch.float64)[agent * 8:agent * 8 + 6]
        dst = torch.empty(6, dtype=torch.float64, pin_memory=True)
        with torch.cuda.stream(self.stream):
            dst.copy_(src, non_blocking=True)
            ev = torch.cuda.Event()
            ev.record(self.stream)
        return dst, ev

    @property
    def n_entities(self):
        landmarks = {"simple": 1, "simple_spread": self.n, "simple_adversary": self.n - 1,
                     "simple_tag": 2, "simple_speaker_listener": 3}.get(self.scenario, 0)
        return self.n + landmarks

    def env_reset(self):
        self._c("mdp_env_reset")

    def env_step(self, act_in=None, u=None):
        a = None if act_in is None else act_in.to(self.device, torch.float32).contiguous()
        uu = None if u is None else u.to(self.device, torch.float32).contiguous()
        self._sized("act_in", a, self.num_envs * self.n * _lib.ACT_DIM)
        self._sized("u", uu, self.num_envs * self.n * _lib.ACT_DIM)
        if a is not None or uu is not None:
            self.sync_in()
        self._c("mdp_env_step", self._ptr(a), self._ptr(uu))
        if a is not None or uu is not None:
            self._keep = (a, uu)
            self.sync_out()

    def env_step_bench(self, out=None, u=None):
        if out is None:
            out = torch.empty((self.num_envs, self.n, _lib.BENCH_W), dtype=torch.float32, device=self.device)
        if u is None:
            self._c("mdp_env_step_bench", self._ptr(out))
        else:
            uu = u.to(self.device, torch.float32).contiguous()
            self._sized("u", uu, self.num_envs * self.n * _lib.ACT_DIM)
            self.sync_in()
            self._c("mdp_env_step_bench_u", self._ptr(out), self._ptr(uu))
            self._keep = (uu,)
        self.sync_out()
        return out

    def evaluate(self, episodes, first_episode=0, mode="sample", bench=False, u=None):
        if mode not in _lib.EVAL_MODE:
            raise ValueError(f"unknown evaluation mode {mode!r} (sample, mean)")
        episodes, first_episode = int(episodes), int(first_episode)
        uu = None if u is None else u.to(self.device, torch.float32).contiguous()
        self._sized("u", uu, episodes * self.max_episode_len * self.n * _lib.ACT_DIM)
        ret = torch.empty((max(episodes, 0), self.n), dtype=torch.float32, device=self.device)
        rec = None
        if bench:
            rec = torch.empty((max(episodes, 0), self.n, _lib.BENCH_W), dtype=torch.float32, device=self.device)
        self.sync_in()
        self._c("mdp_evaluate", first_episode, episodes, _lib.EVAL_MODE[mode], self._ptr(uu), self._ptr(ret),
                self._ptr(rec))
        self._keep = (uu,)
        self.sync_out()
        r64 = ret.double()
        summary = {"mean": r64.mean(0).tolist(), "std": r64.std(0, unbiased=False).tolist(),
                   "min": r64.min(0).values.tolist(), "max": r64.max(0).values.tolist()}
        return {"returns": ret, "bench": rec, "summary": summary}

    def eval_initial_state(self, episodes, first_episode=0):
        episodes, ne = int(episodes), self.n_entities
        pos = np.empty((max(episodes, 0), ne, 2), np.float32)
        vel = np.empty((max(episodes, 0), ne, 2), np.float32)
        goal = np.empty(max(episodes, 0), np.int32)
        self._c("mdp_eval_initial_state", int(first_episode), episodes, _lib.fptr(pos), _lib.fptr(vel),
                goal.ctypes.data_as(ctypes.POINTER(ctypes.c_int32)))
        return {"pos": pos, "vel": vel, "goal": goal}

    def actor_set_floats(self):
        v = int(self.lib.mdp_actor_set_floats(self.h))
        if v < 0:
            raise _lib.MdpError("mdp_actor_set_floats: unusable handle")
        return v

    def actor_bank(self, n_sets):
        n_sets = int(n_sets)
        if not 1 <= n_sets <= _lib.EVAL_MAX_SETS:
            raise ValueError(f"actor_bank: 1 <= n_sets <= {_lib.EVAL_MAX_SETS}, got {n_sets}")
        return torch.zeros((n_sets, self.actor_set_floats()), dtype=torch.float32, device=self.device)

    def _bank_slot(self, bank, k):
        sf = self.actor_set_floats()
        if (not isinstance(bank, torch.Tensor) or bank.dtype != torch.float32 or bank.device != self.device
                or not bank.is_contiguous()):
            raise ValueError("bank: a contiguous float32 tensor on the engine's device (actor_bank)")
        if bank.numel() == 0 or bank.numel() % sf:
            raise ValueError(f"bank: {bank.numel()} elements, a set has {sf}")
        k = int(k)
        if not 0 <= k < bank.numel() // sf:
            raise ValueError(f"bank slot {k} out of range for {bank.numel() // sf} sets")
        return bank.view(-1, sf)[k]

    def bank_snapshot(self, bank, k):
        slot = self._bank_slot(bank, k)
        self.sync_in()
        self._c("mdp_actor_set_snapshot", self._ptr(slot))
        self.sync_out()

    def bank_write(self, bank, k, source, agents=None):
        slot = self._bank_slot(bank, k)
        sd = source
        if not isinstance(source, dict):
            sd = read_checkpoint(source, self.checkpoint_path(source), self.n, self.SETS)[0]
        todo = range(self.n) if agents is None else sorted({int(a) for a in agents})
        flats = []
        for i in todo:
            if not 0 <= i < self.n:
                raise ValueError(f"agent {i} out of range for {self.n} agents")
            flats.append((i, self._flat_params(i, "actor", {t: sd[f"agent_{i}/actor/{t}"] for t in TENSOR_NAMES})))
        self.sync_in()
        for i, flat in flats:
            self._c("mdp_actor_set_write", self._ptr(slot), i, _lib.fptr(flat), flat.size)
        self.sync_out()

    def evaluate_matchups(self, bank, table, episodes, first_episode=0, mode="sample", bench=False, u=None):
        if mode not in _lib.EVAL_MODE:
            raise ValueError(f"unknown evaluation mode {mode!r} (sample, mean)")
        episodes, first_episode = int(episodes), int(first_episode)
        sf = self.actor_set_floats()
        if (not isinstance(bank, torch.Tensor) or bank.dtype != torch.float32 or bank.device != self.device
                or not bank.is_contiguous()):
            raise ValueError("bank: a contiguous float32 tensor on the engine's device (actor_bank)")
        n_sets = bank.numel() // sf
        self._sized("bank", bank, max(n_sets, 1) * sf)
        tab = table.cpu().numpy() if isinstance(table, torch.Tensor) else np.asarray(table)
        if tab.dtype != np.int32:
            raise ValueError(f"table: dtype {tab.dtype}, the call reads int32")
        if tab.ndim != 2 or tab.shape[1] != self.n or tab.shape[0] < 1:
            raise ValueError(f"table: shape {tab.shape}, expected [matchups, {self.n}]")
        tab = np.ascontiguousarray(tab)
        M = tab.shape[0]
        uu = None if u is None else u.to(self.device, torch.float32).contiguous()
        self._sized("u", uu, episodes * self.max_episode_len * self.n * _lib.ACT_DIM)
        ne = max(episodes, 0)
        ret = torch.empty((M, ne, self.n), dtype=torch.float32, device=self.device)
        rec = None
        if bench:
            rec = torch.empty((M, ne, self.n, _lib.BENCH_W), dtype=torch.float32, device=self.device)
        self.sync_in()
        self._c("mdp_evaluate_matchups", self._ptr(bank), n_sets, tab.ctypes.data_as(ctypes.POINTER(ctypes.c_int32)),
                M, first_episode, episodes, _lib.EVAL_MODE[mode], self._ptr(uu), self._ptr(ret), self._ptr(rec))
        self.sync_out()
        r64 = ret.double()
        std = r64.std(1, unbiased=False)
        summary = {"mean": r64.mean(1).tolist(), "std": std.tolist(), "sem": (std / ne ** 0.5).tolist()}
        return {"returns": ret, "bench": rec, "summary": summary}

    def cross_play(self, bank, team, episodes, first_episode=0, mode="sample", bench=False, u=None):
        K = bank.numel() // self.actor_set_floats()
        team = sorted({int(a) for a in team})
        if any(not 0 <= a < self.n for a in team):
            raise ValueError(f"team {team}: agents out of range for {self.n} agents")
        table = np.empty((K, K, self.n), np.int32)
        for j in range(self.n):
            table[:, :, j] = np.arange(K)[:, None] if j in team else np.arange(K)[None, :]
        table = table.reshape(K * K, self.n)
        r = self.evaluate_matchups(bank, table, episodes, first_episode, mode, bench, u)
        shape = (K, K, self.n)
        return {"mean": np.asarray(r["summary"]["mean"], np.float64).reshape(shape),
                "sem": np.asarray(r["summary"]["sem"], np.float64).reshape(shape), "table": table,
                "returns": r["returns"].view(K, K, -1, self.n),
                "bench": None if r["bench"] is None else r["bench"].view(K, K, -1, self.n, _lib.BENCH_W)}

    def env_state(self):
        E, ne = self.num_envs, self.n_entities
        pos = np.empty((E, ne, 2), np.float32)
        vel = np.empty((E, ne, 2), np.float32)
        goal = np.empty(E, np.int32)
        step = np.empty(E, np.int32)
        self._c("mdp_env_get_state", _lib.fptr(pos), _lib.fptr(vel),
                goal.ctypes.data_as(ctypes.POINTER(ctypes.c_int32)),
                step.ctypes.data_as(ctypes.POINTER(ctypes.c_int32)))
        comm = np.empty((E, self.n, _lib.ACT_DIM), np.float32)
        self._c("mdp_env_get_comm", _lib.fptr(comm))
        return {"pos": pos, "vel": vel, "goal": goal, "ep_step": step, "comm": comm}

    def set_env_state(self, pos, vel, goal=None, ep_step=None, comm=None):
        E = self.num_envs
# ... 49 lines not shown
```

Baseline: 1.126 million.

## Specialize rollout and eval kernels on compile-time scenario constants

Adds an EnvFixed template that encodes scenario, agent and landmark counts and per-entity constants at compile time. The H=64 rollout and eval kernels are instantiated per known spec and selected at create time when the runtime EnvDesc matches. In the fixed path the actor weights are preloaded into registers once per kernel instead of per-agent loop, and loops over agents can unroll. The change also adds an env_steps API and profiling stamps, and brings a risk of higher register pressure and more kernel variants to compile.

Result: no change. 1.130 million (median of 5 runs) (+0.4%).

```diff
diff --git a/include/maddpg_hip.h b/include/maddpg_hip.h
--- a/include/maddpg_hip.h
+++ b/include/maddpg_hip.h
@@ -140,6 +140,8 @@
 
 int mdp_env_reset(mdp_handle* h);
 int mdp_env_step(mdp_handle* h, const float* act_in_dev, const float* u_dev);
+int mdp_env_steps(mdp_handle* h, int32_t nsteps, const float* act_in_dev, const float* u_dev, float* info_dev);
+int mdp_rollout_kernel(mdp_handle* h);
 int mdp_env_get_state(mdp_handle* h, float* pos_host, float* vel_host, int32_t* goal_host, int32_t* ep_step_host);
 int mdp_env_set_state(mdp_handle* h, const float* pos_host, const float* vel_host, const int32_t* goal_host, const int32_t* ep_step_host);
 int mdp_env_get_comm(mdp_handle* h, float* comm_host);
diff --git a/maddpg_amd/_lib.py b/maddpg_amd/_lib.py
--- a/maddpg_amd/_lib.py
+++ b/maddpg_amd/_lib.py
@@ -129,6 +129,8 @@
     "mdp_check_finite": (ctypes.c_int, [_P, ctypes.POINTER(_I64)]),
     "mdp_env_reset": (ctypes.c_int, [_P]),
     "mdp_env_step": (ctypes.c_int, [_P, _P, _P]),
+    "mdp_env_steps": (ctypes.c_int, [_P, _I32, _P, _P, _P]),
+    "mdp_rollout_kernel": (ctypes.c_int, [_P]),
     "mdp_env_get_state": (ctypes.c_int, [_P, _F32P, _F32P, _I32P, _I32P]),
     "mdp_env_set_state": (ctypes.c_int, [_P, _F32P, _F32P, _I32P, _I32P]),
     "mdp_env_get_comm": (ctypes.c_int, [_P, _F32P]),
diff --git a/maddpg_amd/csrc/mdp_api.cpp b/maddpg_amd/csrc/mdp_api.cpp
--- a/maddpg_amd/csrc/mdp_api.cpp
+++ b/maddpg_amd/csrc/mdp_api.cpp
@@ -331,6 +331,7 @@
   bool tp_pair_fits[3][MDP_MAX_AGENTS] = {};
   FusedApplyArgs tp_pair_host[3][MDP_MAX_AGENTS][2];
   bool rollout_draw = true;
+  int rollout_spec = 0;
   bool draw_ahead = true;
   bool grad_pair = true;
   uint64_t* xbuf = nullptr;
@@ -1342,6 +1343,8 @@
     h->fused_apply = !(u && u[0] == '1');
     const char* rd = getenv("MDP_ROLLOUT_DRAW");
     h->rollout_draw = !(rd && rd[0] == '0');
+    const char* rg = getenv("MDP_ROLLOUT_GENERIC");
+    h->rollout_spec = (rg && rg[0] == '1') ? 0 : mdp_rollout_spec_of(h->L.topo, h->L.env);
     const char* da = getenv("MDP_DRAW_AHEAD");
     h->draw_ahead = !(da && da[0] == '0');
     const char* gp = getenv("MDP_GRAD_PAIR");
@@ -2047,6 +2050,8 @@
   return 0;
 }
 
+int mdp_rollout_kernel(mdp_handle* h) { return unusable(h) ? -1 : h->rollout_spec; }
+
 int mdp_dp_info(mdp_handle* h, int32_t out4[4]) {
   if (unusable(h) || !out4) return -1;
   out4[0] = h->p2p ? 2 : (h->comm ? 1 : 0);
@@ -2213,8 +2218,14 @@
   return 0;
 }
 
+static bool rollout_multi_ok(const mdp_handle* h) { return h->cfg.num_envs <= 16; }
+
 static int env_step_launch(mdp_handle* h, const float* act_in_dev, const float* u_dev, float* bench = nullptr,
                            int32_t* pf_out = nullptr, int pf_count = 0, int nsteps = 1) {
+  if (nsteps < 1) return fail(h, "env step: nsteps must be >= 1");
+  if (nsteps > 1 && (act_in_dev || u_dev || bench || pf_out || !rollout_multi_ok(h)))
+    return fail(h, "env step: several steps per launch need at most 16 env copies and no injected actions, "
+                   "injected uniforms, benchmark records or index draw");
   RolloutArgs a;
   a.pf_out = pf_out;
   a.pf_count = pf_out ? pf_count : 0;
@@ -2242,17 +2253,17 @@
   a.ticket = &h->ctl->ticket[2];
   a.bench = bench;
   ProfScope p(h, MDP_K_ROLLOUT);
-  HIPCHK(h, mdp_launch_rollout(a, h->L.topo.H, lds_rollout_bytes(h->L.topo), h->stream));
-  return 0;
-}
-
-static bool rollout_multi_ok(const mdp_handle* h) { return h->cfg.num_envs <= 16; }
+  HIPCHK(h, mdp_launch_rollout(a, h->L.topo.H, h->rollout_spec, lds_rollout_bytes(h->L.topo), h->stream));
+  return 0;
+}
 
 static void advance_ring_mirror(mdp_handle* h) {
   const int64_t cap = h->cfg.capacity, E = h->cfg.num_envs;
   h->len = std::min(cap, h->len + E);
   h->next = (h->next + E) % cap;
 }
+
+static const char* no_bench_reason(int scenario);
 
 int mdp_env_step(mdp_handle* h, const float* act_in_dev, const float* u_dev) {
   if (need_env(h)) return -1;
@@ -2262,6 +2273,20 @@
   const int rc = env_step_launch(h, act_in_dev, u_dev);
   if (rc) return rc;
   advance_ring_mirror(h);
+  return 0;
+}
+
+int mdp_env_steps(mdp_handle* h, int32_t nsteps, const float* act_in_dev, const float* u_dev, float* info_dev) {
+  if (need_env(h)) return -1;
+  const int64_t en = 4 * (int64_t)h->cfg.num_envs * h->cfg.n_agents;
+  MDP_DEV(h, act_in_dev, en * MDP_ACT_DIM, "mdp_env_steps", true);
+  MDP_DEV(h, u_dev, en * MDP_ACT_DIM, "mdp_env_steps", true);
+  MDP_DEV(h, info_dev, en * MDP_BENCH_W, "mdp_env_steps", true);
+  if (info_dev)
+    if (const char* why = no_bench_reason(h->cfg.scenario)) return fail(h, why);
+  const int rc = env_step_launch(h, act_in_dev, u_dev, info_dev, nullptr, 0, nsteps);
+  if (rc) return rc;
+  for (int s = 0; s < nsteps; ++s) advance_ring_mirror(h);
   return 0;
 }
 
@@ -2340,7 +2365,7 @@
   a.ret = ret_dev;
   a.bench = bench_dev;
   ProfScope p(h, MDP_K_EVAL);
-  HIPCHK(h, mdp_launch_eval_episodes(a, h->L.topo.H, lds_rollout_bytes(h->L.topo), h->stream));
+  HIPCHK(h, mdp_launch_eval_episodes(a, h->L.topo.H, h->rollout_spec, lds_rollout_bytes(h->L.topo), h->stream));
   return 0;
 }
 
@@ -2477,7 +2502,7 @@
     a.set_stride = stride;
     a.matchups = matchups;
     ProfScope p(h, MDP_K_EVAL);
-    e = mdp_launch_eval_matchups(a, h->L.topo.H, lds, h->stream);
+    e = mdp_launch_eval_matchups(a, h->L.topo.H, h->rollout_spec, lds, h->stream);
   }
   const hipError_t es = hipStreamSynchronize(h->stream);
   (void)hipFree(table_dev);
diff --git a/maddpg_amd/csrc/mdp_device.h b/maddpg_amd/csrc/mdp_device.h
--- a/maddpg_amd/csrc/mdp_device.h
+++ b/maddpg_amd/csrc/mdp_device.h
@@ -807,6 +807,17 @@
     w[s] = r < nout ? v : 0.f;
   }
 }
+__device__ __forceinline__ void rh_load_raw(float (&w)[16], const float* __restrict__ W, int nout) {
+  const int lane = threadIdx.x & 63, r = lane & 15, kq = lane >> 4;
+  const int c = min(r, nout - 1);
+#pragma unroll
+  for (int s = 0; s < 16; ++s) w[s] = W[(4 * s + kq) * nout + c];
+}
+__device__ __forceinline__ void rh_mask(float (&w)[16], int nout) {
+  const int r = threadIdx.x & 15;
+#pragma unroll
+  for (int s = 0; s < 16; ++s) w[s] = r < nout ? w[s] : 0.f;
+}
 __device__ __forceinline__ f32x4 rh_acc(const float* X, int ldx, const float (&w)[16]) {
   const int lane = threadIdx.x & 63, r = lane & 15, kq = lane >> 4;
   float x[16];
diff --git a/maddpg_amd/csrc/mdp_kernels.h b/maddpg_amd/csrc/mdp_kernels.h
--- a/maddpg_amd/csrc/mdp_kernels.h
+++ b/maddpg_amd/csrc/mdp_kernels.h
@@ -358,10 +358,11 @@
 hipError_t mdp_launch_critic_grad_per(const CriticArgsPer& a, int H, int lds_bytes, hipStream_t s);
 hipError_t mdp_launch_critic_grad_r_per(const CriticArgsPer& a, int lds_bytes, hipStream_t s);
 hipError_t mdp_launch_actor_grad_r(const ActorArgs& a, int lds_bytes, hipStream_t s);
-hipError_t mdp_launch_rollout(const RolloutArgs& a, int H, int lds_bytes, hipStream_t s);
+int mdp_rollout_spec_of(const Topo& T, const EnvDesc& env);
+hipError_t mdp_launch_rollout(const RolloutArgs& a, int H, int spec, int lds_bytes, hipStream_t s);
 hipError_t mdp_launch_eval(const EvalArgs& a, int H, int lds_bytes, hipStream_t s);
-hipError_t mdp_launch_eval_episodes(const EvalEpArgs& a, int H, int lds_bytes, hipStream_t s);
-hipError_t mdp_launch_eval_matchups(const EvalMuArgs& a, int H, int lds_bytes, hipStream_t s);
+hipError_t mdp_launch_eval_episodes(const EvalEpArgs& a, int H, int spec, int lds_bytes, hipStream_t s);
+hipError_t mdp_launch_eval_matchups(const EvalMuArgs& a, int H, int spec, int lds_bytes, hipStream_t s);
 hipError_t mdp_launch_eval_reset(const EnvDesc& env, uint64_t seed, uint32_t first, int count, float* pos, float* vel,
                                  int32_t* goal, hipStream_t s);
 hipError_t mdp_launch_apply(const ApplyArgs& a, hipStream_t s);
diff --git a/maddpg_amd/csrc/mdp_kernels.hip b/maddpg_amd/csrc/mdp_kernels.hip
--- a/maddpg_amd/csrc/mdp_kernels.hip
+++ b/maddpg_amd/csrc/mdp_kernels.hip
@@ -346,7 +346,8 @@
   return sqrtf(dx * dx + dy * dy);
 }
 
-__device__ inline void env_obs(const EnvDesc& E, const float* p, const float* v, int goal, int i, float* o) {
+template <class EV>
+__device__ inline void env_obs(const EV& E, const float* p, const float* v, int goal, int i, float* o) {
   const int n = E.n_agents, L = E.n_landmarks;
   int c = 0;
   switch (E.scenario) {
@@ -418,7 +419,8 @@
   }
 }
 
-__device__ inline void env_obs_comm(const EnvDesc& E, const float* p, const float* v, int goal, int i, float* o,
+template <class EV>
+__device__ inline void env_obs_comm(const EV& E, const float* p, const float* v, int goal, int i, float* o,
                                     const float* comm) {
   const int n = E.n_agents, L = E.n_landmarks;
   int c = 0;
@@ -436,7 +438,8 @@
   }
 }
 
-__device__ inline void env_reward(const EnvDesc& E, const float* p, int goal, float* rew) {
+template <class EV>
+__device__ inline void env_reward(const EV& E, const float* p, int goal, float* rew) {
   const int n = E.n_agents, L = E.n_landmarks;
   switch (E.scenario) {
     case MDP_SCN_SIMPLE: {
@@ -517,7 +520,8 @@
   }
 }
 
-__device__ inline void env_bench(const EnvDesc& E, const float* p, int goal, float* out) {
+template <class EV>
+__device__ inline void env_bench(const EV& E, const float* p, int goal, float* out) {
   const int n = E.n_agents, L = E.n_landmarks;
   for (int q = 0; q < n * MDP_BENCH_W; ++q) out[q] = 0.f;
   switch (E.scenario) {
@@ -573,7 +577,8 @@
   }
 }
 
-__device__ inline void env_physics_tile(const EnvDesc& E, float* sp, float* sv, const float* act, int ldr, float* f,
+template <class EV>
+__device__ inline void env_physics_tile(const EV& E, float* sp, float* sv, const float* act, int ldr, float* f,
                                         int nvalid) {
   const int n = E.n_agents, ne = E.n_agents + E.n_landmarks;
   const float k = 1e-3f;
@@ -612,6 +617,7 @@
     fr[2 * MDP_MAX_ENT + e] = has;
   }
   __syncthreads();
+  MDP_STAMP(50);
   for (int q = threadIdx.x; q < nvalid * ne; q += MDP_NT) {
     const int r = q / ne, e = q - r * ne;
     if (!E.movable[e]) continue;
@@ -638,9 +644,11 @@
     p[2 * e + 1] += vy * 0.1f;
   }
   __syncthreads();
-}
-
-__device__ inline void env_reset_one(const EnvDesc& E, uint64_t seed, uint32_t stream, uint32_t ctr, uint32_t env,
+  MDP_STAMP(51);
+}
+
+template <class EV>
+__device__ inline void env_reset_one(const EV& E, uint64_t seed, uint32_t stream, uint32_t ctr, uint32_t env,
                                      float* p, float* v, int32_t* goal) {
   const int n = E.n_agents, ne = E.n_agents + E.n_landmarks;
   const uint2 key = make_uint2((uint32_t)seed, (uint32_t)(seed >> 32));
@@ -720,12 +728,40 @@
   }
 }
 
-template <int H, bool MULTI>
+template <class EV>
+__device__ __forceinline__ int ag_field(const Topo& T, int j, int ADesc::*m) {
+  if constexpr (std::is_same<EV, EnvDesc>::value) {
+    return T.ag[j].*m;
+  } else {
+    int v = T.ag[0].*m;
+    asm volatile("" : "+s"(v));
+#pragma unroll
+    for (int k = 1; k < EV::n_agents; ++k) {
+      int c = T.ag[k].*m;
+      asm volatile("" : "+s"(c));
+      v = j == k ? c : v;
+    }
+    return v;
+  }
+}
+template <class EV>
+__device__ __forceinline__ decltype(auto) env_view(const EnvDesc& d) {
+  if constexpr (std::is_same<EV, EnvDesc>::value) return (d);
+  else return EV{d.max_ep_len};
+}
+struct ActorFrag {
+  f32x4 w1[16], w2[16], b1, b2;
+  float w3[16], b3;
+};
+
+template <int H, bool MULTI, class EV = EnvDesc>
 __global__ __launch_bounds__(MDP_NT) void k_rollout(RolloutArgs a) {
   extern __shared__ __attribute__((aligned(16))) float lds[];
   MDP_TL_ROLLOUT();
+  constexpr bool FIXED = !std::is_same<EV, EnvDesc>::value;
+  static_assert(!FIXED || H == 64, "the fixed tables are instantiated for the H = 64 path only");
   const Topo& T = a.topo;
-  const EnvDesc& E = a.env;
+  const auto& E = env_view<EV>(a.env);
   const int n = E.n_agents, ne = E.n_agents + E.n_landmarks;
   const int ldr = lds_ld(T.row_stride), ldh = H + 1;
   LdsCarve cv(lds);
@@ -775,8 +811,27 @@
       vv[u] = a.vel[(int64_t)(e0 + r) * 2 * ne + c];
     }
   }
+  ActorFrag fr;
+  if constexpr (FIXED) {
+    const int wv = min(__builtin_amdgcn_readfirstlane(tid >> 6), n - 1), r16 = tid & 15;
+    const ADesc& aw = T.ag[wv];
+    const NDesc& an = aw.actor;
+    const float* P = a.theta;
+    rf_load<16>(fr.w1, P + an.t[0].off, aw.obs_dim);
+    rf_load<16>(fr.w2, P + an.t[2].off, MDP_RH);
+    rh_load_raw(fr.w3, P + an.t[4].off, MDP_ACT_DIM);
+    fr.b1 = ld4(P + an.t[1].off + 4 * r16);
+    fr.b2 = ld4(P + an.t[3].off + 4 * r16);
+    fr.b3 = P[an.t[5].off + min(r16, MDP_ACT_DIM - 1)];
+  }
   const int64_t next_raw = gc->next, len_raw = gc->len;
-  const uint32_t step_raw = (uint32_t)gc->env_steps;
+  uint32_t step_raw;
+  if constexpr (FIXED) {
+    typedef __attribute__((address_space(1))) const uint32_t gU32;
+    step_raw = *(gU32*)&gc->env_steps;
+  } else {
+    step_raw = (uint32_t)gc->env_steps;
+  }
   const int64_t ep_base_raw = gc->episodes;
   if (tid < MDP_R * n) epr[er_r * MDP_MAX_AGENTS + er_j] = er;
 #pragma unroll
@@ -802,10 +857,12 @@
   if (tid < MDP_R * n) {
     const int r = tid / n, j = tid - r * n;
     if (__builtin_expect(a.comm != nullptr, 0))
-      env_obs_comm(E, sp + r * 2 * MDP_MAX_ENT, sv + r * 2 * MDP_MAX_ENT, sgoal[r], j, rowt + r * ldr + T.ag[j].obs_off,
+      env_obs_comm(E, sp + r * 2 * MDP_MAX_ENT, sv + r * 2 * MDP_MAX_ENT, sgoal[r], j,
+                   rowt + r * ldr + ag_field<EV>(T, j, &ADesc::obs_off),
                    r < nvalid ? a.comm + (int64_t)(e0 + r) * n * MDP_ACT_DIM : nullptr);
     else
-      env_obs(E, sp + r * 2 * MDP_MAX_ENT, sv + r * 2 * MDP_MAX_ENT, sgoal[r], j, rowt + r * ldr + T.ag[j].obs_off);
+      env_obs(E, sp + r * 2 * MDP_MAX_ENT, sv + r * 2 * MDP_MAX_ENT, sgoal[r], j,
+              rowt + r * ldr + ag_field<EV>(T, j, &ADesc::obs_off));
   }
   __syncthreads();
 
@@ -823,13 +880,17 @@
         const ADesc& aj = T.ag[j];
         const NDesc& an = aj.actor;
         const float* P = a.theta;
-        f32x4 w1[16], w2[16];
-        float w3[16];
-        rf_load<16>(w1, P + an.t[0].off, aj.obs_dim);
-        rf_load<16>(w2, P + an.t[2].off, MDP_RH);
-        rh_load(w3, P + an.t[4].off, MDP_ACT_DIM);
-        const f32x4 b1 = ld4(P + an.t[1].off + 4 * r), b2 = ld4(P + an.t[3].off + 4 * r);
-        const float b3 = P[an.t[5].off + min(r, MDP_ACT_DIM - 1)];
+        if constexpr (!FIXED) {
+          rf_load<16>(fr.w1, P + an.t[0].off, aj.obs_dim);
+          rf_load<16>(fr.w2, P + an.t[2].off, MDP_RH);
+          rh_load(fr.w3, P + an.t[4].off, MDP_ACT_DIM);
+          fr.b1 = ld4(P + an.t[1].off + 4 * r);
+          fr.b2 = ld4(P + an.t[3].off + 4 * r);
+          fr.b3 = P[an.t[5].off + min(r, MDP_ACT_DIM - 1)];
+        }
+        const f32x4(&w1)[16] = fr.w1, (&w2)[16] = fr.w2;
+        const f32x4 &b1 = fr.b1, &b2 = fr.b2;
+        const float& b3 = fr.b3;
         float u[MDP_ACT_DIM];
         if (lane < MDP_R) {
           if (a.u_in) {
@@ -857,6 +918,10 @@
         }
         wave_sync();
         {
+          float w3[16];
+#pragma unroll
+          for (int s = 0; s < 16; ++s) w3[s] = fr.w3[s];
+          if constexpr (FIXED) rh_mask(w3, MDP_ACT_DIM);
           const f32x4 acc = rh_acc(h2j, MDP_RLH, w3);
           if (r < MDP_ACT_DIM) {
 #pragma unroll
@@ -948,13 +1013,16 @@
   } else if (tid >= 64 && tid - 64 < nvalid * n) {
     const int q = tid - 64, r = q / n, j = q - r * n;
     if (__builtin_expect(a.comm != nullptr, 0))
-      env_obs_comm(E, sp + r * 2 * MDP_MAX_ENT, sv + r * 2 * MDP_MAX_ENT, sgoal[r], j, rowt + r * ldr + T.ag[j].nobs_off,
-                   rowt + r * ldr + T.ag[0].act_off);
+      env_obs_comm(E, sp + r * 2 * MDP_MAX_ENT, sv + r * 2 * MDP_MAX_ENT, sgoal[r], j,
+                   rowt + r * ldr + ag_field<EV>(T, j, &ADesc::nobs_off), rowt + r * ldr + T.ag[0].act_off);
     else
-      env_obs(E, sp + r * 2 * MDP_MAX_ENT, sv + r * 2 * MDP_MAX_ENT, sgoal[r], j, rowt + r * ldr + T.ag[j].nobs_off);
+      env_obs(E, sp + r * 2 * MDP_MAX_ENT, sv + r * 2 * MDP_MAX_ENT, sgoal[r], j,
+              rowt + r * ldr + ag_field<EV>(T, j, &ADesc::nobs_off));
   }
   static_assert(64 + MDP_R * MDP_MAX_AGENTS <= MDP_NT, "rollout obs': one pass on waves 1..");
+  if (tid == 0) MDP_STAMP(52);
   __syncthreads();
+  MDP_STAMP(53);
   if (MULTI) ep_done += s_nterm;
   if (term) {
     const int e = e0 + tid;
@@ -977,6 +1045,7 @@
     const int64_t dst = (next_s + e0 + r) % a.cap;
     *reinterpret_cast<float4*>(a.replay + dst * T.row_stride + c4 * 4) = make_float4(s[0], s[1], s[2], s[3]);
   }
+  MDP_STAMP(54);
   }
   for (int q = tid; q < nvalid * 2 * ne; q += MDP_NT) {
     const int r = q / (2 * ne), c = q - r * 2 * ne;
@@ -985,14 +1054,15 @@
   }
   MDP_STAMP(47);
   rollout_finish(a, next_raw, len_raw);
-}
-
-template <int H, class Args = EvalEpArgs>
+  MDP_STAMP(55);
+}
+
+template <int H, class Args = EvalEpArgs, class EV = EnvDesc>
 __global__ __launch_bounds__(MDP_NT) void k_eval_episodes(Args a) {
   constexpr bool MU = std::is_same<Args, EvalMuArgs>::value;
   extern __shared__ __attribute__((aligned(16))) float lds[];
   const Topo& T = a.topo;
-  const EnvDesc& E = a.env;
+  const auto& E = env_view<EV>(a.env);
   const int n = E.n_agents;
   const int ldr = lds_ld(T.row_stride), ldh = H + 1;
   LdsCarve cv(lds);
@@ -1082,10 +1152,12 @@
     if (tid < MDP_R * n) {
       const int r = tid / n, j = tid - r * n;
       if (comm)
-        env_obs_comm(E, sp + r * 2 * MDP_MAX_ENT, sv + r * 2 * MDP_MAX_ENT, sgoal[r], j, rowt + r * ldr + T.ag[j].obs_off,
+        env_obs_comm(E, sp + r * 2 * MDP_MAX_ENT, sv + r * 2 * MDP_MAX_ENT, sgoal[r], j,
+                     rowt + r * ldr + ag_field<EV>(T, j, &ADesc::obs_off),
                      t > 0 ? rowt + r * ldr + T.ag[0].act_off : nullptr);
       else
-        env_obs(E, sp + r * 2 * MDP_MAX_ENT, sv + r * 2 * MDP_MAX_ENT, sgoal[r], j, rowt + r * ldr + T.ag[j].obs_off);
+        env_obs(E, sp + r * 2 * MDP_MAX_ENT, sv + r * 2 * MDP_MAX_ENT, sgoal[r], j,
+                rowt + r * ldr + ag_field<EV>(T, j, &ADesc::obs_off));
     }
     __syncthreads();
     if (par) {
@@ -1224,9 +1296,44 @@
     if (e_ != hipSuccess) return e_;   \
   } while (0)
 
+#define MDP_ENV_SPECS(X)                  \
+  X(1, MDP_SCN_SIMPLE, 1, 1, 0)           \
+  X(2, MDP_SCN_SPREAD, 3, 3, 0)           \
+  X(3, MDP_SCN_ADVERSARY, 3, 2, 1)        \
+  X(4, MDP_SCN_TAG, 4, 2, 3)              \
+  X(5, MDP_SCN_SPEAKER_LISTENER, 2, 3, 0)
+
+int mdp_rollout_spec_of(const Topo& T, const EnvDesc& env) {
+  if (T.H != 64 || T.n > MDP_NW) return 0;
+  for (int j = 0; j < T.n; ++j)
+    if (T.ag[j].obs_dim > 64) return 0;
+#define X(id, scn, n, l, na) \
+  if (env_fixed_matches<scn, n, l, na>(env)) return id;
+  MDP_ENV_SPECS(X)
+#undef X
+  return 0;
+}
+
 template <int H>
-static hipError_t launch_rollout_t(const RolloutArgs& a, int lds_bytes, hipStream_t s) {
+static hipError_t launch_rollout_t(const RolloutArgs& a, int spec, int lds_bytes, hipStream_t s) {
   const int grid = (a.E + MDP_R - 1) / MDP_R + (a.pf_count > 0 ? 1 : 0);
+  if constexpr (H == 64) {
+    if (spec != 0 && a.nsteps <= 1) {
+      switch (spec) {
+#define X(id, scn, n, l, na)                                                                                         \
+  case id:                                                                                                           \
+    mdp_launch(k_rollout<64, false, EnvFixed<scn, n, l, na>>, dim3(grid), dim3(MDP_NT), lds_bytes, s, a); \
+    break;
+        MDP_ENV_SPECS(X)
+#undef X
+        default: return hipErrorInvalidValue;
+      }
+      MDP_CHECK_LAUNCH();
+      return hipSuccess;
+    }
+  } else if (spec != 0) {
+    return hipErrorInvalidValue;
+  }
   if (a.nsteps > 1)
     mdp_launch(k_rollout<H, true>, dim3(grid), dim3(MDP_NT), lds_bytes, s, a);
   else
@@ -1251,6 +1358,17 @@
   (void)hipFuncSetAttribute((const void*)k_eval_episodes<H>, hipFuncAttributeMaxDynamicSharedMemorySize, 128 * 1024);
   (void)hipFuncSetAttribute((const void*)k_eval_episodes<H, EvalMuArgs>, hipFuncAttributeMaxDynamicSharedMemorySize,
                             128 * 1024);
+  if constexpr (H == 64) {
+#define X(id, scn, n, l, na)                                                                                  \
+  {                                                                                                           \
+    using EV = EnvFixed<scn, n, l, na>;                                                                       \
+    const void* f[3] = {(const void*)k_rollout<64, false, EV>, (const void*)k_eval_episodes<64, EvalEpArgs, EV>, \
+                        (const void*)k_eval_episodes<64, EvalMuArgs, EV>};                                    \
+    for (const void* k : f) (void)hipFuncSetAttribute(k, hipFuncAttributeMaxDynamicSharedMemorySize, 128 * 1024); \
+  }
+    MDP_ENV_SPECS(X)
+#undef X
+  }
 }
 static void ensure_lds_limits() {
   if (!set_lds_limit_done) {
@@ -1262,12 +1380,12 @@
   }
 }
 
-hipError_t mdp_launch_rollout(const RolloutArgs& a, int H, int lds_bytes, hipStream_t s) {
+hipError_t mdp_launch_rollout(const RolloutArgs& a, int H, int spec, int lds_bytes, hipStream_t s) {
   ensure_lds_limits();
   switch (H) {
-    case 64: return launch_rollout_t<64>(a, lds_bytes, s);
-    case 128: return launch_rollout_t<128>(a, lds_bytes, s);
-    case 256: return launch_rollout_t<256>(a, lds_bytes, s);
+    case 64: return launch_rollout_t<64>(a, spec, lds_bytes, s);
+    case 128: return launch_rollout_t<128>(a, spec, lds_bytes, s);
+    case 256: return launch_rollout_t<256>(a, spec, lds_bytes, s);
     default: return hipErrorInvalidValue;
   }
 }
@@ -1280,14 +1398,31 @@
     default: return hipErrorInvalidValue;
   }
 }
+template <class Args>
+static hipError_t launch_eval_fixed(const Args& a, int spec, dim3 grid, int lds_bytes, hipStream_t s) {
+  switch (spec) {
+#define X(id, scn, n, l, na)                                                                                   \
+  case id:                                                                                                     \
+    mdp_launch(k_eval_episodes<64, Args, EnvFixed<scn, n, l, na>>, grid, dim3(MDP_NT), lds_bytes, s, a); \
+    break;
+    MDP_ENV_SPECS(X)
+#undef X
+    default: return hipErrorInvalidValue;
+  }
+  MDP_CHECK_LAUNCH();
+  return hipSuccess;
+}
 template <int H>
 static hipError_t launch_eval_episodes_t(const EvalEpArgs& a, int lds_bytes, hipStream_t s) {
   mdp_launch(k_eval_episodes<H>, dim3((a.episodes + MDP_R - 1) / MDP_R), dim3(MDP_NT), lds_bytes, s, a);
   MDP_CHECK_LAUNCH();
   return hipSuccess;
 }
-hipError_t mdp_launch_eval_episodes(const EvalEpArgs& a, int H, int lds_bytes, hipStream_t s) {
+hipError_t mdp_launch_eval_episodes(const EvalEpArgs& a, int H, int spec, int lds_bytes, hipStream_t s) {
   ensure_lds_limits();
+  if (spec != 0)
+    return H == 64 ? launch_eval_fixed(a, spec, dim3((a.episodes + MDP_R - 1) / MDP_R), lds_bytes, s)
+                   : hipErrorInvalidValue;
   switch (H) {
     case 64: return launch_eval_episodes_t<64>(a, lds_bytes, s);
     case 128: return launch_eval_episodes_t<128>(a, lds_bytes, s);
@@ -1302,8 +1437,11 @@
   MDP_CHECK_LAUNCH();
   return hipSuccess;
 }
-hipError_t mdp_launch_eval_matchups(const EvalMuArgs& a, int H, int lds_bytes, hipStream_t s) {
+hipError_t mdp_launch_eval_matchups(const EvalMuArgs& a, int H, int spec, int lds_bytes, hipStream_t s) {
   ensure_lds_limits();
+  if (spec != 0)
+    return H == 64 ? launch_eval_fixed(a, spec, dim3((a.episodes + MDP_R - 1) / MDP_R, a.matchups), lds_bytes, s)
+                   : hipErrorInvalidValue;
   switch (H) {
     case 64: return launch_eval_matchups_t<64>(a, lds_bytes, s);
     case 128: return launch_eval_matchups_t<128>(a, lds_bytes, s);
diff --git a/maddpg_amd/csrc/mdp_topo.h b/maddpg_amd/csrc/mdp_topo.h
--- a/maddpg_amd/csrc/mdp_topo.h
+++ b/maddpg_amd/csrc/mdp_topo.h
@@ -41,6 +41,64 @@
   int adversary[MDP_MAX_AGENTS];
 };
 #if defined(__HIPCC__)
+#define MDP_HD __host__ __device__
+#else
+#define MDP_HD
+#endif
+template <int SCN, int N, int L, int NA>
+struct EnvFixed {
+  static constexpr int scenario = SCN, n_agents = N, n_landmarks = L, n_adv = NA;
+  int max_ep_len;
+  struct Size {
+    MDP_HD constexpr float operator[](int e) const {
+      return SCN == MDP_SCN_SIMPLE ? 0.05f
+           : SCN == MDP_SCN_SPREAD ? (e < N ? 0.15f : 0.05f)
+           : SCN == MDP_SCN_ADVERSARY ? (e < N ? 0.15f : 0.08f)
+           : SCN == MDP_SCN_TAG ? (e < NA ? 0.075f : e < N ? 0.05f : 0.2f)
+           : (e < N ? 0.075f : 0.04f);
+    }
+  } size;
+  struct Accel {
+    MDP_HD constexpr float operator[](int e) const { return SCN == MDP_SCN_TAG ? (e < NA ? 3.0f : 4.0f) : 5.0f; }
+  } accel;
+  struct MaxSpeed {
+    MDP_HD constexpr float operator[](int e) const {
+      return SCN == MDP_SCN_TAG && e < N ? (e < NA ? 1.0f : 1.3f) : -1.f;
+    }
+  } max_speed;
+  struct Collide {
+    MDP_HD constexpr int operator[](int e) const {
+      return SCN == MDP_SCN_SPREAD ? e < N : SCN == MDP_SCN_TAG ? e < N + L : 0;
+    }
+  } collide;
+  struct Movable {
+    MDP_HD constexpr int operator[](int e) const {
+      return SCN == MDP_SCN_SPEAKER_LISTENER ? e == 1 : e < N;
+    }
+  } movable;
+  struct Adversary {
+    MDP_HD constexpr int operator[](int e) const {
+      return (SCN == MDP_SCN_ADVERSARY || SCN == MDP_SCN_TAG) && e < NA;
+    }
+  } adversary;
+};
+template <int SCN, int N, int L, int NA>
+inline bool env_fixed_matches(const EnvDesc& d) {
+  constexpr EnvFixed<SCN, N, L, NA> f{};
+  if (d.scenario != SCN || d.n_agents != N || d.n_landmarks != L || d.n_adv != NA) return false;
+  for (int e = 0; e < MDP_MAX_ENT; ++e) {
+    const bool in = e < N + L;
+    if (d.size[e] != (in ? f.size[e] : 0.f) || d.max_speed[e] != (in ? f.max_speed[e] : -1.f)) return false;
+    if (d.collide[e] != (in ? f.collide[e] : 0) || d.movable[e] != (in ? f.movable[e] : 0)) return false;
+  }
+  for (int i = 0; i < MDP_MAX_AGENTS; ++i) {
+    if (d.accel[i] != (i < N ? f.accel[i] : 5.0f)) return false;
+    if (d.adversary[i] != (i < N ? f.adversary[i] : 0)) return false;
+  }
+  return true;
+}
+
+#if defined(__HIPCC__)
 __host__ __device__
 #endif
 inline int env_dim_c(int scenario) { return scenario == MDP_SCN_SPEAKER_LISTENER ? 3 : 0; }
diff --git a/maddpg_amd/engine.py b/maddpg_amd/engine.py
--- a/maddpg_amd/engine.py
+++ b/maddpg_amd/engine.py
@@ -705,6 +705,20 @@
             self._keep = (a, uu)
             self.sync_out()
 
+    def rollout_kernel(self):
+        return int(self._c("mdp_rollout_kernel"))
+
+    def env_steps(self, nsteps, act_in=None, u=None, bench=None):
+        a = None if act_in is None else act_in.to(self.device, torch.float32).contiguous()
+        uu = None if u is None else u.to(self.device, torch.float32).contiguous()
+        self._sized("act_in", a, self.num_envs * self.n * _lib.ACT_DIM)
+        self._sized("u", uu, self.num_envs * self.n * _lib.ACT_DIM)
+        self._sized("bench", bench, self.num_envs * self.n * _lib.BENCH_W)
+        self.sync_in()
+        self._c("mdp_env_steps", int(nsteps), self._ptr(a), self._ptr(uu), self._ptr(bench))
+        self._keep = (a, uu, bench)
+        self.sync_out()
+
     def env_step_bench(self, out=None, u=None):
         if out is None:
             out = torch.empty((self.num_envs, self.n, _lib.BENCH_W), dtype=torch.float32, device=self.device)
```
